# megapose6d/megapose6d

Measured on AMD Instinct MI355X. Metric: pose-hypotheses/sec (render+coarse+refine), 640×480, megapose-1.0-RGB, higher is better.
Workload: dtype f32 (results of fp32 arithmetic; the convolutions' multiplications run on the bf16 MFMA as EXACT piece products of the fp32 operands, fp32 accumulate)

## Files before the change

### include/mp_engine.h

```cpp
#ifndef MP_ENGINE_H
#define MP_ENGINE_H

#include <stddef.h>
#include <stdint.h>

#ifdef __cplusplus
extern "C" {
#endif

typedef void* mp_stream;

#define MP_OK 0
#define MP_ERR_INVALID (-22)
#define MP_ERR_NOMEM (-12)
#define MP_ERR_HIP (-5)

int mp_version(void);
const char* mp_last_error(void);
int mp_profile_begin(void);
int mp_profile_end(void);
int mp_profile_active(void);
int mp_profile_query_ex(int idx, char* name, int name_len, int64_t* launches, double* total_ms, double* total_flops,
                        double* total_bytes, double* total_executed_flops, double* peak_tflops);



int mp_device_info(int* n_cus, int* lds_bytes, char* arch_name, int arch_name_len);

typedef struct mp_mesh_db mp_mesh_db;

typedef struct {
  const float* h_vertices;
  const float* h_normals;
  const float* h_colors;
  const int32_t* h_faces;
  int32_t n_vertices;
  int32_t n_faces;
} mp_mesh_desc;

int mp_mesh_db_create(const mp_mesh_desc* h_meshes, int n_meshes, mp_mesh_db** out);
#define MP_TEX_MAX_LEVELS 15
int mp_mesh_db_set_texture(mp_mesh_db* db, int mesh_id, const float* h_uvs, const uint32_t* h_texels, int tex_w, int tex_h,
                           int n_levels);
int mp_mesh_db_destroy(mp_mesh_db* db);
int mp_mesh_db_max_vertices(const mp_mesh_db* db);
float mp_mesh_db_radius(const mp_mesh_db* db, int mesh_id);

#define MP_RASTER_NORMALS 1u
#define MP_RASTER_DEPTH 2u
#define MP_RASTER_NORMALS_GL 4u
#define MP_RASTER_MSAA4 16u

#define MP_RASTER_F16 32u

#define MP_RASTER_XREC 64u

typedef struct {
  float ambient[3];
  int32_t n_point;
  float point_dir[8][3];
  float point_color[8][3];
  float point_offset[8][3];
} mp_lights;

size_t mp_raster_workspace_bytes(const mp_mesh_db* db, int n_views, int h, int w);

int mp_raster_render(const mp_mesh_db* db, const int32_t* d_mesh_ids, const float* d_TCO ,
                     const float* d_K , int n_views, int h, int w, uint32_t flags,
                     const mp_lights* h_lights, float* d_out, int64_t stride_v, int views_per_item,
                     int64_t stride_view, int64_t stride_y, int64_t stride_x, int c_rgb, int c_normals,
                     int c_depth, void* d_workspace, size_t workspace_bytes, mp_stream stream);

int mp_raster_render_crop(const mp_mesh_db* db, const int32_t* d_mesh_ids, const float* d_TCO, const float* d_K, int n_views,
                          int h, int w, uint32_t flags, const mp_lights* lights, float* d_out, int64_t stride_v,
                          int views_per_item, int64_t stride_view, int64_t stride_y, int64_t stride_x, int c_rgb,
                          int c_normals, int c_depth, void* d_workspace, size_t workspace_bytes,
                          const float* d_images , int images_nhwc4, int n_im,
                          int C, int H, int W, const int32_t* d_im_ids, const float* d_boxes, int c0_crop, mp_stream stream);
int mp_raster_render_xrec(const mp_mesh_db* db, const int32_t* d_mesh_ids, const float* d_TCO, const float* d_K, int n_views,
                          int h, int w, uint32_t flags, const mp_lights* lights, void* d_out_records, int64_t stride_v,
                          int views_per_item, int64_t stride_view, int64_t stride_y, int64_t stride_x, int c_rgb,
                          int c_normals, int c_depth, void* d_workspace, size_t workspace_bytes,
                          const float* d_images, int images_nhwc4, int n_im, int C, int H, int W, const int32_t* d_im_ids,
                          const float* d_boxes, uint32_t f32_mask, const float* d_tCR, int depth_mode, mp_stream stream);
const unsigned char* mp_raster_job_flags(const mp_mesh_db* db, const void* d_workspace, int n_views, int h, int w);
int mp_pack_observation_nhwc4(const float* d_images, int n_im, int C, int H, int W, float* d_out, mp_stream stream);

size_t mp_raster_scene_workspace_bytes(const mp_mesh_db* db, int n_objects, int h, int w);

int mp_raster_render_scene(const mp_mesh_db* db, int n_cams, const int32_t* h_obj_off, const int32_t* d_obj_off,
                           const int32_t* d_mesh_ids, const float* d_TCO, const float* d_K, const float* d_radius,
                           const mp_lights* d_lights, int h, int w, uint32_t flags, float* d_out, int64_t stride_v, int64_t stride_y,
                           int64_t stride_x, int c_rgb, int c_normals, int c_depth, int32_t* d_instance, void* d_workspace,
                           size_t workspace_bytes, mp_stream stream);

int mp_crop_roi_align(const float* d_images , int n_im, int C, int H, int W,
                      const int32_t* d_im_ids , const float* d_boxes , int b,
                      int out_h, int out_w, float* d_out, int64_t stride_b, int64_t stride_y,
                      int64_t stride_x, int c0, mp_stream stream);

int mp_normalize_depth(float* d_x, int b, int h, int w, int border, int C, const int32_t* h_channels,
                       int n_ch, const float* d_tCR , int mode, mp_stream stream);
int mp_normalize_depth_f16(void* d_x_half, int b, int h, int w, int border, int C, const int32_t* h_channels,
                           int n_ch, const float* d_tCR , int mode, mp_stream stream);

size_t mp_conv_packed_floats(int Cin_p, int Cout, int KH, int KW);
int mp_conv_pack_weights(const float* h_w_oihw, int Cout, int Cin, int KH, int KW, int Cin_p,
                         const float* h_scale , float* h_packed);

typedef struct {
  const float* d_x;
  int32_t N, H, W, C;
  int32_t in_border;
  const float* d_w;
  const float* d_bias;
  int32_t Cout, KH, KW, stride, pad;
  float* d_y;
  int32_t out_border;
  const float* d_residual;
  int32_t relu;
  float* d_y_act;
  const float* d_act_scale;
  const float* d_act_shift;
  int32_t c_real;
  float* d_splitk_ws;
  int64_t splitk_ws_floats;
  int32_t x_f16;
} mp_conv_desc;

int mp_conv2d_nhwc(const mp_conv_desc* desc, mp_stream stream);
int mp_conv2d_plan(const mp_conv_desc* desc, int n_cu, int32_t* out5);

const char* mp_conv2d_kernel_name(const mp_conv_desc* desc);

size_t mp_conv_bf16x9_packed_bytes(int Cin_p, int Cout, int KH, int KW);
int mp_conv_bf16x9_pack_weights(const float* h_w_oihw, int Cout, int Cin, int KH, int KW, int Cin_p, const float* h_scale ,
                                void* h_packed);
int mp_conv2d_bf16x9_nhwc(const mp_conv_desc* desc, const void* d_w_pieces, mp_stream stream);

size_t mp_conv_wino_packed_floats(int Cin_p, int Cout);
int mp_conv_wino_pack_weights(const float* h_w_oi33, int Cout, int Cin, int Cin_p, const float* h_scale , float* h_packed);
int mp_conv_wino_eligible(const mp_conv_desc* desc, int n_cu);
int mp_conv3x3_wino_nhwc(const mp_conv_desc* desc, const float* d_u, mp_stream stream);

size_t mp_conv_wino_bf16_packed_bytes(int Cin_p, int Cout);
int mp_conv_wino_bf16_pack_weights(const float* h_w_oi33, int Cout, int Cin, int Cin_p, const float* h_scale , void* h_packed);
int mp_conv3x3_wino_bf16_nhwc(const mp_conv_desc* desc, const void* d_u_pieces, mp_stream stream);

int mp_xrec_elements(int n_f32, int n_u8);
int mp_conv_stem_supported(int KS, int n_f32, int n_u8);
size_t mp_conv_stem_packed_bytes(int KS, int n_f32, int n_u8, int Cout);
int mp_conv_stem_pack_weights_mask(const float* h_w_oihw, int Cout, int Cin, int KS, uint32_t f32_mask,
                                   const float* h_scale , void* h_packed);
int mp_conv_stem_xrec(const mp_conv_desc* desc, const void* d_packed, int n_f32, mp_stream stream);
int mp_conv_stem_xrec_pool(const mp_conv_desc* desc, const void* d_packed, int n_f32, float* d_ypool, int pool_border, mp_stream stream);

int mp_conv_stem_sparse_chunks(int KS, int n_f32, int n_u8);
size_t mp_conv_stem_sparse_packed_bytes(int KS, int n_f32, int n_u8, int Cout);
int mp_conv_stem_pack_weights_sparse(const float* h_w_oihw, int Cout, int Cin, int KS, int n_f32, const float* h_scale, void* h_packed);
int mp_conv_stem_xrec_sparse(const mp_conv_desc* desc, const void* d_packed, const void* d_packed_sparse, int n_f32,
                             const unsigned char* d_tile_flags, float* d_ypool, int pool_border, mp_stream stream);

int mp_maxpool3x3s2(const float* d_x, int N, int H, int W, int C, int in_border, float* d_y,
                    int out_border, float* d_y_act, const float* d_act_scale, const float* d_act_shift,
                    mp_stream stream);

int mp_bn_relu_nhwc(const float* d_x, int N, int H, int W, int C, int border, float* d_y_act, const float* d_act_scale,
                    const float* d_act_shift, mp_stream stream);

int mp_pool_fc_heads(const float* d_x, int N, int H, int W, int C, int in_border, const float* d_fc_w,
                     const float* d_fc_b, int n_feat, const float* d_head_w, const float* d_head_b,
                     int n_out, float* d_feat , float* d_out ,
                     float* d_sigmoid , mp_stream stream);

typedef struct mp_backbone mp_backbone;
#define MP_BACKBONE_VANILLA_RESNET34 0
#define MP_BACKBONE_WIDE_RESNET34 1
#define MP_BACKBONE_WIDE_RESNET18 2

typedef struct {
  const char* name;
  const float* h_data;
  int64_t numel;
} mp_named_tensor;

int mp_backbone_create_wide(int kind, int width, int c_in, int head_kind, int n_head_out, const mp_named_tensor* state, int n_tensors,
                            mp_backbone** out);
int mp_backbone_destroy(mp_backbone* bb);
int mp_backbone_input_channels_padded(const mp_backbone* bb);
int mp_backbone_input_border(const mp_backbone* bb);
size_t mp_backbone_workspace_bytes(const mp_backbone* bb, int batch, int h, int w);
int mp_backbone_workspace_reset(mp_backbone* bb, const void* d_workspace);
int mp_backbone_forward(mp_backbone* bb, const float* d_x, int batch, int h, int w, float* d_out,
                        float* d_sigmoid, float* d_feat, void* d_workspace, size_t workspace_bytes,
                        mp_stream stream);
int mp_backbone_forward_f16(mp_backbone* bb, const void* d_x_half, int batch, int h, int w, float* d_out,
                            float* d_sigmoid, float* d_feat, void* d_workspace, size_t workspace_bytes,
                            mp_stream stream);
int mp_backbone_xrec_prepare(mp_backbone* bb, uint32_t f32_mask);
int mp_backbone_forward_xrec_mask(mp_backbone* bb, const void* d_xrec, uint32_t f32_mask, int batch, int h, int w, float* d_out,
                                  float* d_sigmoid, float* d_feat, void* d_workspace, size_t workspace_bytes,
                                  mp_stream stream);
int mp_backbone_forward_xrec_sparse(mp_backbone* bb, const void* d_xrec, uint32_t f32_mask, const unsigned char* d_tile_flags, int batch,
                                    int h, int w, float* d_out, float* d_sigmoid, float* d_feat, void* d_workspace,
                                    size_t workspace_bytes, mp_stream stream);
double mp_backbone_flops(const mp_backbone* bb, int batch, int h, int w);

int mp_normalize_T(const float* d_T, int b, float* d_T_out, mp_stream stream);

int mp_init_extents(const float* d_points , int n_mesh, int n_pts,
                    const float* d_R , int n_rot, float* d_ext, mp_stream stream);
int mp_init_poses_from_boxes(const float* d_boxes , const float* d_K ,
                             const int32_t* d_mesh_ids, const int32_t* d_rot_ids, const float* d_R,
                             int n_rot, const float* d_ext, int b, float* d_TCO ,
                             mp_stream stream);

#define MP_MV_REMOVE_TCO 256
#define MP_MV_INPLANE 512
int mp_pose_multiview_n_views(int multiview);
int mp_pose_prepare_ex(const float* d_TCO_in , const float* d_K ,
                       const int32_t* d_mesh_ids, const float* d_points ,
                       int n_pts_stride, int n_pts_main, int n_pts_views, int b, int V, int multiview,
                       int im_h, int im_w, int out_h, int out_w, float lamb,
                       float* d_TCO_n , float* d_tCR , float* d_TCV_O ,
                       float* d_KV_crop , float* d_boxes_rend ,
                       float* d_boxes_crop , float* d_K_main , mp_stream stream);

int mp_pose_update(const float* d_TCO , const float* d_K_crop ,
                   int k_stride_floats, const float* d_out9 , const float* d_tCR , int b,
                   float* d_TCO_out, mp_stream stream);

#define MP_POSE_ERROR_MEAN 0
#define MP_POSE_ERROR_MAX 1
size_t mp_pose_error_workspace_bytes(int b, int n_pts, int S_max);
int mp_pose_error_sym(const float* d_T_pred , const float* d_T_gt, const float* d_symmetries, const int32_t* d_n_sym, int S_max,
                      const float* d_points, int n_pts_stride, const int32_t* d_mesh_ids , const int32_t* d_n_points, int n_pts,
                      int b, int reduce, int split, float* d_err , float* d_err_alt, int32_t* d_idx , float* d_T_gt_sym,
                      float* d_errs, float* d_diffs, void* d_workspace, size_t workspace_bytes, mp_stream stream);
int mp_pose_error_nn(const float* d_T_pred , const float* d_T_gt , const float* d_points, int n_pts_stride,
                     const int32_t* d_mesh_ids, const int32_t* d_n_points, int n_pts, int b, int split, float* d_diffs, int32_t* d_assign,
                     float* d_mean , float* d_max , void* d_workspace, size_t workspace_bytes, mp_stream stream);
int mp_pose_error_rigid(const float* d_T_a , const float* d_T_b , int b, const float* d_K, const float* d_points,
                        int n_pts_stride, const int32_t* d_mesh_ids, const int32_t* d_n_points, int n_pts, float* d_trans_err ,
                        float* d_rot_err_deg , float* d_proj_err, mp_stream stream);

int mp_pose_error_mspd(const float* d_T_pred , const float* d_T_gt, const float* d_symmetries, const int32_t* d_n_sym, int S_max,
                       const float* d_points, int n_pts_stride, const int32_t* d_mesh_ids , const int32_t* d_n_points, int n_pts,
                       int b, int reduce, int split, const float* d_K , float* d_err , float* d_err_alt,
                       int32_t* d_idx , float* d_T_gt_sym, float* d_errs, void* d_workspace, size_t workspace_bytes, mp_stream stream);

size_t mp_vsd_workspace_bytes(int b, int n_tau);
int mp_vsd(const float* d_depth_est , const int32_t* d_est_ids ,
           const float* d_depth_gt , const int32_t* d_gt_ids, const float* d_depth_test ,
           const int32_t* d_im_ids, int n_est, int n_gt, int n_im, const float* d_K , const float* d_diameter ,
           int b, int h, int w, float delta, const float* h_taus, int n_tau , int normalized, int split,
           float* d_errs , int32_t* d_counts ,
           void* d_workspace, size_t workspace_bytes, mp_stream stream);

size_t mp_gt_info_workspace_bytes(int b);
int mp_gt_info(const float* d_depth_gt , const int32_t* d_gt_ids ,
               const float* d_depth_test , const int32_t* d_im_ids, int n_gt, int n_im, const float* d_K ,
               int b, int h, int w, int canvas , float delta, int split,
               int32_t* d_counts , int32_t* d_boxes ,
               float* d_visib_fract , uint8_t* d_mask , uint8_t* d_mask_visib ,
               void* d_workspace, size_t workspace_bytes, mp_stream stream);

int mp_bop_match_limits(int* max_errors, int* max_thetas, int* mask_bits, int* stage_floats);
size_t mp_bop_match_workspace_bytes(int n_taken_words, int E, int n_theta);
int mp_bop_match(const float* d_errs , const int32_t* d_cand_gt , const int32_t* d_cand_lgt ,
                 const int32_t* d_est_row , const int32_t* d_est_off ,
                 const int32_t* d_group_est_off , const int32_t* d_group_n_gt ,
                 const int32_t* d_group_taken_off , const int32_t* d_n_top ,
                 const double* d_thr , int P, int C, int n_est, int n_groups, int n_taken_words, int E,
                 int n_theta, int32_t* d_match , void* d_workspace, size_t workspace_bytes, mp_stream stream);

int mp_mask_pair_counts(const uint8_t* d_pred_masks , const uint8_t* d_gt_masks ,
                        const int32_t* d_cand_pred , const int32_t* d_cand_gt , int P, int G, int C, int H, int W, int split,
                        int32_t* d_counts , mp_stream stream);
size_t mp_det_match_workspace_bytes(int n_taken_words, int n_theta);
int mp_det_match(const double* d_iou , const int32_t* d_cand_gt , const int32_t* d_cand_lgt ,
                 const int32_t* d_est_row , const int32_t* d_est_off ,
                 const int32_t* d_group_est_off , const int32_t* d_group_n_gt ,
                 const int32_t* d_group_taken_off , const int32_t* d_n_top ,
                 const uint8_t* d_gt_ignore , const double* d_thr , int P, int C, int n_est, int n_groups,
                 int n_taken_words, int n_theta, int32_t* d_match , void* d_workspace, size_t workspace_bytes,
                 mp_stream stream);

size_t mp_model_info_scratch_bytes(int n_obj, const int32_t* h_n_points, int tile);
int mp_model_info(const float* d_points , int stride, const int32_t* d_n_points ,
                  const int32_t* h_n_points , int n_obj, int tile, void* d_scratch, float* d_d2 ,
                  int32_t* d_pair , float* d_bounds , mp_stream stream);

size_t mp_surface_sample_scratch_bytes(int n_obj, const int32_t* h_face_off, int count, int block);
int mp_surface_sample(const float* d_vertices , const int32_t* d_faces , const int32_t* d_vert_off ,
                      const int32_t* d_face_off , const int32_t* h_vert_off , const int32_t* h_face_off ,
                      int n_obj, const float* d_u , int count, int block, void* d_workspace,
                      float* d_points , int32_t* d_face , mp_stream stream);

int mp_overlay(const uint8_t* d_images , const uint8_t* d_render , const int32_t* d_labels ,
               const uint8_t* d_colors , int n_colors, int n, int h, int w, int dilate_iterations,
               uint8_t* d_contour , uint8_t* d_canny , uint8_t* d_mask ,
               uint8_t* d_mesh , mp_stream stream);
int mp_draw_boxes(const uint8_t* d_images , const float* d_boxes , const int32_t* d_image_ids ,
                  int n_boxes, const uint8_t* d_colors , int n_colors, int n, int h, int w, int thickness,
                  uint8_t* d_out , mp_stream stream);

size_t mp_icp_workspace_bytes(int n_images, int n_rows, int H, int W);
int mp_icp_refine(const float* d_depth_meas, int n_images, const int32_t* d_im_ids, const float* d_depth_rend,
                  const float* d_K_images, const float* d_K_rows, const float* d_TCO, int n_rows, int H, int W,
                  int n_iterations, int n_levels, float tolerance, int n_min_points, int user_masks, float* d_TCO_out,
                  int32_t* d_retval, float* d_residual, void* d_workspace, size_t workspace_bytes, mp_stream stream);

int mp_icp_nn_max_points(void);
size_t mp_icp_nn_workspace_bytes(int n_images, int n_rows, int H, int W);
int mp_icp_refine_nn(const float* d_depth_meas, int n_images, const int32_t* d_im_ids, const float* d_depth_rend, const float* d_K_images,
                     const float* d_K_rows, const float* d_TCO, int n_rows, int H, int W, int n_iterations, int n_levels, float tolerance,
                     int n_min_points, const unsigned char* d_masks, float* d_TCO_out, int32_t* d_retval, float* d_residual, int32_t* d_iters,
                     void* d_ws, size_t ws_bytes, mp_stream stream);

size_t mp_fps_workspace_bytes(int n_rows, int stride);
int mp_fps(const float* d_points, const int32_t* d_counts, int n_rows, int stride, int n_points, int use_fps, int32_t* d_idx, int32_t* d_m,
           void* d_workspace, size_t workspace_bytes, mp_stream stream);
size_t mp_teaser_workspace_bytes(int n_rows, int H, int W);
int mp_teaser_solve(const float* d_src, const float* d_dst, const int32_t* d_counts, int n_rows, int stride, float noise_bound,
                    int inlier_selection, int tim_graph, int min_num_inliers, double* d_Rt, int32_t* d_retval, int32_t* d_degree,
                    int32_t* d_core, int32_t* d_selected, int32_t* d_info, void* d_workspace, size_t workspace_bytes, mp_stream stream);
int mp_teaser_refine(const float* d_depth_meas, int n_images, const int32_t* d_im_ids, const float* d_depth_rend, const float* d_K_rows,
                     const float* d_TCO, int n_rows, int H, int W, int mask_type, float depth_delta_thresh, int n_min_points, int n_points,
                     float noise_bound, int min_num_inliers, int use_fps, int inlier_selection, int tim_graph, float* d_TCO_out,
                     int32_t* d_retval, double* d_Rt, int32_t* d_sample_idx, int32_t* d_degree, int32_t* d_core, int32_t* d_selected,
                     int32_t* d_info, void* d_workspace, size_t workspace_bytes, mp_stream stream);
int mp_max_clique_default_steps(void);
size_t mp_max_clique_workspace_bytes(int n_rows, int stride);
int mp_max_clique(const uint8_t* d_adjacency, const int32_t* d_counts, int n_rows, int stride, int max_steps, int32_t* d_members, int32_t* d_info,
                  void* d_workspace, size_t workspace_bytes, mp_stream stream);
size_t mp_teaser_workspace_bytes_ex(int n_rows, int H, int W, int stride, int inlier_selection);
int mp_teaser_solve_ex(const float* d_src, const float* d_dst, const int32_t* d_counts, int n_rows, int stride, float noise_bound,
                       int inlier_selection, int tim_graph, int min_num_inliers, double* d_Rt, int32_t* d_retval, int32_t* d_degree,
                       int32_t* d_core, int32_t* d_selected, int32_t* d_info, int max_clique_steps, int32_t* d_clique_info, void* d_workspace,
                       size_t workspace_bytes, mp_stream stream);
int mp_teaser_refine_ex(const float* d_depth_meas, int n_images, const int32_t* d_im_ids, const float* d_depth_rend, const float* d_K_rows,
                        const float* d_TCO, int n_rows, int H, int W, int mask_type, float depth_delta_thresh, int n_min_points, int n_points,
                        float noise_bound, int min_num_inliers, int use_fps, int inlier_selection, int tim_graph, float* d_TCO_out,
                        int32_t* d_retval, double* d_Rt, int32_t* d_sample_idx, int32_t* d_degree, int32_t* d_core, int32_t* d_selected,
                        int32_t* d_info, int max_clique_steps, int32_t* d_clique_info, void* d_workspace, size_t workspace_bytes, mp_stream stream);

typedef struct mp_detector mp_detector;

typedef struct {
  int32_t n_classes;
  int32_t min_size, max_size;
  float image_mean[3], image_std[3];
  int32_t anchor_sizes[5];
  float aspect_ratios[3];
  int32_t rpn_pre_nms_top_n, rpn_post_nms_top_n;
  float rpn_nms_thresh, rpn_score_thresh, rpn_min_size;
  float box_score_thresh, box_nms_thresh, box_min_size;
  int32_t box_detections_per_img;
} mp_detector_config;

int mp_detector_default_config(mp_detector_config* cfg, int n_classes, int min_size, int max_size);
int mp_detector_state_spec(int n_classes, int idx, char* name, int name_len, int64_t* shape4, int32_t* n_dims);
int mp_detector_create(const mp_detector_config* cfg, const mp_named_tensor* h_state, int n_tensors, mp_detector** out);
int mp_detector_destroy(mp_detector* det);
size_t mp_detector_workspace_bytes(const mp_detector* det, int n_images, int H, int W);
int mp_detector_forward(mp_detector* det, const float* d_images, int n_images, int H, int W, float* d_boxes, float* d_scores,
                        int32_t* d_labels, int32_t* d_counts, float* d_masks, void* d_workspace, size_t workspace_bytes,
                        mp_stream stream);
int mp_detector_debug_tensor(const mp_detector* det, const char* what, const void** d_ptr, int64_t* shape4, int32_t* border,
                             int64_t* row_stride, int64_t* n_elements );

#ifdef __cplusplus
}
#endif
#endif
```

### megapose6d_amd/_lib.py

```python
from __future__ import annotations

import ctypes as C
import os
from pathlib import Path

_HERE = Path(__file__).resolve().parent
LIB_PATH = _HERE / "libmp_engine.so"


class EngineError(RuntimeError):
    pass


class MeshDesc(C.Structure):
    _fields_ = [
        ("h_vertices", C.c_void_p),
        ("h_normals", C.c_void_p),
        ("h_colors", C.c_void_p),
        ("h_faces", C.c_void_p),
        ("n_vertices", C.c_int32),
        ("n_faces", C.c_int32),
    ]


class Lights(C.Structure):
    _fields_ = [
        ("ambient", C.c_float * 3),
        ("n_point", C.c_int32),
        ("point_dir", (C.c_float * 3) * 8),
        ("point_color", (C.c_float * 3) * 8),
        ("point_offset", (C.c_float * 3) * 8),
    ]


class ConvDesc(C.Structure):
    _fields_ = [
        ("d_x", C.c_void_p),
        ("N", C.c_int32), ("H", C.c_int32), ("W", C.c_int32), ("C", C.c_int32),
        ("in_border", C.c_int32),
        ("d_w", C.c_void_p),
        ("d_bias", C.c_void_p),
        ("Cout", C.c_int32), ("KH", C.c_int32), ("KW", C.c_int32), ("stride", C.c_int32), ("pad", C.c_int32),
        ("d_y", C.c_void_p),
        ("out_border", C.c_int32),
        ("d_residual", C.c_void_p),
        ("relu", C.c_int32),
        ("d_y_act", C.c_void_p),
        ("d_act_scale", C.c_void_p),
        ("d_act_shift", C.c_void_p),
        ("c_real", C.c_int32),
        ("d_splitk_ws", C.c_void_p),
        ("splitk_ws_floats", C.c_int64),
        ("x_f16", C.c_int32),
    ]


class DetectorConfig(C.Structure):
    _fields_ = [
        ("n_classes", C.c_int32),
        ("min_size", C.c_int32), ("max_size", C.c_int32),
        ("image_mean", C.c_float * 3), ("image_std", C.c_float * 3),
        ("anchor_sizes", C.c_int32 * 5),
        ("aspect_ratios", C.c_float * 3),
        ("rpn_pre_nms_top_n", C.c_int32), ("rpn_post_nms_top_n", C.c_int32),
        ("rpn_nms_thresh", C.c_float), ("rpn_score_thresh", C.c_float), ("rpn_min_size", C.c_float),
        ("box_score_thresh", C.c_float), ("box_nms_thresh", C.c_float), ("box_min_size", C.c_float),
        ("box_detections_per_img", C.c_int32),
    ]


class NamedTensor(C.Structure):
    _fields_ = [("name", C.c_char_p), ("h_data", C.c_void_p), ("numel", C.c_int64)]


_vp, _i, _i64, _f, _sz, _u32 = C.c_void_p, C.c_int, C.c_int64, C.c_float, C.c_size_t, C.c_uint32

SIGNATURES = {
    "mp_version": (_i, []),
    "mp_last_error": (C.c_char_p, []),
    "mp_conv_clock_read": (_i, [C.POINTER(C.c_double), _i]),
    "mp_clock_probe": (_i, [C.c_double, C.POINTER(C.c_double), C.POINTER(C.c_double), _vp]),
    "mp_profile_begin": (_i, []),
    "mp_profile_end": (_i, []),
    "mp_profile_active": (_i, []),
    "mp_profile_query_ex": (_i, [_i, C.c_char_p, _i, C.POINTER(_i64), C.POINTER(C.c_double), C.POINTER(C.c_double), C.POINTER(C.c_double),
                                 C.POINTER(C.c_double), C.POINTER(C.c_double)]),
    "mp_device_info": (_i, [C.POINTER(_i), C.POINTER(_i), C.c_char_p, _i]),
    "mp_mesh_db_create": (_i, [C.POINTER(MeshDesc), _i, C.POINTER(_vp)]),
    "mp_mesh_db_set_texture": (_i, [_vp, _i, _vp, _vp, _i, _i, _i]),
    "mp_mesh_db_destroy": (_i, [_vp]),
    "mp_mesh_db_max_vertices": (_i, [_vp]),
    "mp_mesh_db_radius": (_f, [_vp, _i]),
    "mp_raster_workspace_bytes": (_sz, [_vp, _i, _i, _i]),
    "mp_raster_render": (_i, [_vp, _vp, _vp, _vp, _i, _i, _i, _u32, C.POINTER(Lights), _vp, _i64, _i, _i64, _i64, _i64, _i, _i, _i,
                              _vp, _sz, _vp]),
    "mp_raster_render_crop": (_i, [_vp, _vp, _vp, _vp, _i, _i, _i, _u32, C.POINTER(Lights), _vp, _i64, _i, _i64, _i64, _i64, _i, _i, _i,
                                   _vp, _sz, _vp, _i, _i, _i, _i, _i, _vp, _vp, _i, _vp]),
    "mp_raster_render_xrec": (_i, [_vp, _vp, _vp, _vp, _i, _i, _i, _u32, C.POINTER(Lights), _vp, _i64, _i, _i64, _i64, _i64, _i, _i, _i,
                                   _vp, _sz, _vp, _i, _i, _i, _i, _i, _vp, _vp, _u32, _vp, _i, _vp]),
    "mp_raster_job_flags": (_vp, [_vp, _vp, _i, _i, _i]),
    "mp_pack_observation_nhwc4": (_i, [_vp, _i, _i, _i, _i, _vp, _vp]),
    "mp_raster_scene_workspace_bytes": (_sz, [_vp, _i, _i, _i]),
    "mp_raster_render_scene": (_i, [_vp, _i, C.POINTER(C.c_int32), _vp, _vp, _vp, _vp, _vp, _vp, _i, _i, _u32, _vp, _i64, _i64, _i64, _i, _i,
                                    _i, _vp, _vp, _sz, _vp]),
    "mp_crop_roi_align": (_i, [_vp, _i, _i, _i, _i, _vp, _vp, _i, _i, _i, _vp, _i64, _i64, _i64, _i, _vp]),
    "mp_normalize_depth": (_i, [_vp, _i, _i, _i, _i, _i, C.POINTER(C.c_int32), _i, _vp, _i, _vp]),
    "mp_normalize_depth_f16": (_i, [_vp, _i, _i, _i, _i, _i, C.POINTER(C.c_int32), _i, _vp, _i, _vp]),
    "mp_conv_packed_floats": (_sz, [_i, _i, _i, _i]),
    "mp_conv_pack_weights": (_i, [_vp, _i, _i, _i, _i, _i, _vp, _vp]),
    "mp_conv2d_nhwc": (_i, [C.POINTER(ConvDesc), _vp]),
    "mp_conv2d_plan": (_i, [C.POINTER(ConvDesc), _i, C.POINTER(C.c_int32)]),
    "mp_conv_bf16x9_packed_bytes": (_sz, [_i, _i, _i, _i]),
    "mp_conv_bf16x9_pack_weights": (_i, [_vp, _i, _i, _i, _i, _i, _vp, _vp]),
    "mp_conv2d_bf16x9_nhwc": (_i, [C.POINTER(ConvDesc), _vp, _vp]),
    "mp_conv2d_kernel_name": (C.c_char_p, [C.POINTER(ConvDesc)]),
    "mp_conv_wino_packed_floats": (_sz, [_i, _i]),
    "mp_conv_wino_pack_weights": (_i, [_vp, _i, _i, _i, _vp, _vp]),
    "mp_conv_wino_eligible": (_i, [C.POINTER(ConvDesc), _i]),
    "mp_conv3x3_wino_nhwc": (_i, [C.POINTER(ConvDesc), _vp, _vp]),
    "mp_conv_wino_stats": (_i, [C.POINTER(C.c_double), C.POINTER(C.c_double), _i]),
    "mp_conv_wino_bf16_packed_bytes": (_sz, [_i, _i]),
    "mp_conv_wino_bf16_pack_weights": (_i, [_vp, _i, _i, _i, _vp, _vp]),
    "mp_conv3x3_wino_bf16_nhwc": (_i, [C.POINTER(ConvDesc), _vp, _vp]),
    "mp_conv_wino_bf16_stats": (_i, [C.POINTER(C.c_double), C.POINTER(C.c_double), _i]),
    "mp_conv_wino_bf16_clock": (_i, [C.POINTER(C.c_double), C.POINTER(C.c_double), _i]),
    "mp_conv_wino_bf16_phases": (_i, [C.POINTER(C.c_double), C.POINTER(C.c_double)]),
    "mp_conv_wino_bf16_telemetry": (_i, [_i]),
    "mp_xrec_elements": (_i, [_i, _i]),
    "mp_conv_stem_supported": (_i, [_i, _i, _i]),
    "mp_conv_stem_packed_bytes": (_sz, [_i, _i, _i, _i]),
    "mp_conv_stem_pack_weights_mask": (_i, [_vp, _i, _i, _i, _u32, _vp, _vp]),
    "mp_conv_stem_sparse_chunks": (_i, [_i, _i, _i]),
    "mp_conv_stem_sparse_packed_bytes": (_sz, [_i, _i, _i, _i]),
    "mp_conv_stem_pack_weights_sparse": (_i, [_vp, _i, _i, _i, _i, _vp, _vp]),
    "mp_conv_stem_xrec_sparse": (_i, [C.POINTER(ConvDesc), _vp, _vp, _i, _vp, _vp, _i, _vp]),
    "mp_conv_stem_bg_stats": (_i, [C.POINTER(C.c_double), C.POINTER(C.c_double), _i]),
    "mp_conv_stem_xrec": (_i, [C.POINTER(ConvDesc), _vp, _i, _vp]),
    "mp_conv_stem_xrec_pool": (_i, [C.POINTER(ConvDesc), _vp, _i, _vp, _i, _vp]),
    "mp_maxpool3x3s2": (_i, [_vp, _i, _i, _i, _i, _i, _vp, _i, _vp, _vp, _vp, _vp]),
    "mp_bn_relu_nhwc": (_i, [_vp, _i, _i, _i, _i, _i, _vp, _vp, _vp, _vp]),
    "mp_pool_fc_heads": (_i, [_vp, _i, _i, _i, _i, _i, _vp, _vp, _i, _vp, _vp, _i, _vp, _vp, _vp, _vp]),
    "mp_backbone_create_wide": (_i, [_i, _i, _i, _i, _i, C.POINTER(NamedTensor), _i, C.POINTER(_vp)]),
    "mp_backbone_destroy": (_i, [_vp]),
    "mp_backbone_input_channels_padded": (_i, [_vp]),
    "mp_backbone_input_border": (_i, [_vp]),
    "mp_backbone_workspace_bytes": (_sz, [_vp, _i, _i, _i]),
    "mp_backbone_workspace_reset": (_i, [_vp, _vp]),
    "mp_backbone_forward": (_i, [_vp, _vp, _i, _i, _i, _vp, _vp, _vp, _vp, _sz, _vp]),
    "mp_backbone_forward_f16": (_i, [_vp, _vp, _i, _i, _i, _vp, _vp, _vp, _vp, _sz, _vp]),
    "mp_backbone_xrec_prepare": (_i, [_vp, _u32]),
    "mp_backbone_forward_xrec_mask": (_i, [_vp, _vp, _u32, _i, _i, _i, _vp, _vp, _vp, _vp, _sz, _vp]),
    "mp_backbone_forward_xrec_sparse": (_i, [_vp, _vp, _u32, _vp, _i, _i, _i, _vp, _vp, _vp, _vp, _sz, _vp]),
    "mp_backbone_flops": (C.c_double, [_vp, _i, _i, _i]),
    "mp_normalize_T": (_i, [_vp, _i, _vp, _vp]),
    "mp_init_extents": (_i, [_vp, _i, _i, _vp, _i, _vp, _vp]),
    "mp_init_poses_from_boxes": (_i, [_vp, _vp, _vp, _vp, _vp, _i, _vp, _i, _vp, _vp]),
    "mp_pose_multiview_n_views": (_i, [_i]),
    "mp_pose_prepare_ex": (_i, [_vp, _vp, _vp, _vp, _i, _i, _i, _i, _i, _i, _i, _i, _i, _i, _f, _vp, _vp, _vp, _vp, _vp, _vp, _vp, _vp]),
    "mp_pose_error_workspace_bytes": (_sz, [_i, _i, _i]),
    "mp_pose_error_sym": (_i, [_vp, _vp, _vp, _vp, _i, _vp, _i, _vp, _vp, _i, _i, _i, _i, _vp, _vp, _vp, _vp, _vp, _vp, _vp, _sz, _vp]),
    "mp_pose_error_nn": (_i, [_vp, _vp, _vp, _i, _vp, _vp, _i, _i, _i, _vp, _vp, _vp, _vp, _vp, _sz, _vp]),
    "mp_pose_error_rigid": (_i, [_vp, _vp, _i, _vp, _vp, _i, _vp, _vp, _i, _vp, _vp, _vp, _vp]),
    "mp_pose_error_mspd": (_i, [_vp, _vp, _vp, _vp, _i, _vp, _i, _vp, _vp, _i, _i, _i, _i, _vp, _vp, _vp, _vp, _vp, _vp, _vp, _sz, _vp]),
    "mp_vsd_workspace_bytes": (_sz, [_i, _i]),
    "mp_vsd": (_i, [_vp, _vp, _vp, _vp, _vp, _vp, _i, _i, _i, _vp, _vp, _i, _i, _i, _f, _vp, _i, _i, _i, _vp, _vp, _vp, _sz, _vp]),
    "mp_gt_info_workspace_bytes": (_sz, [_i]),
    "mp_gt_info": (_i, [_vp, _vp, _vp, _vp, _i, _i, _vp, _i, _i, _i, _i, _f, _i, _vp, _vp, _vp, _vp, _vp, _vp, _sz, _vp]),
    "mp_bop_match_limits": (_i, [C.POINTER(_i), C.POINTER(_i), C.POINTER(_i), C.POINTER(_i)]),
    "mp_bop_match_workspace_bytes": (_sz, [_i, _i, _i]),
    "mp_bop_match": (_i, [_vp, _vp, _vp, _vp, _vp, _vp, _vp, _vp, _vp, _vp, _i, _i, _i, _i, _i, _i, _i, _vp, _vp, _sz, _vp]),
    "mp_mask_pair_counts": (_i, [_vp, _vp, _vp, _vp, _i, _i, _i, _i, _i, _i, _vp, _vp]),
    "mp_det_match_workspace_bytes": (_sz, [_i, _i]),
    "mp_det_match": (_i, [_vp, _vp, _vp, _vp, _vp, _vp, _vp, _vp, _vp, _vp, _vp, _i, _i, _i, _i, _i, _i, _vp, _vp, _sz, _vp]),
    "mp_model_info_scratch_bytes": (_sz, [_i, _vp, _i]),
    "mp_model_info": (_i, [_vp, _i, _vp, _vp, _i, _i, _vp, _vp, _vp, _vp, _vp]),
    "mp_overlay": (_i, [_vp, _vp, _vp, _vp, _i, _i, _i, _i, _i, _vp, _vp, _vp, _vp, _vp]),
    "mp_draw_boxes": (_i, [_vp, _vp, _vp, _i, _vp, _i, _i, _i, _i, _i, _vp, _vp]),
    "mp_surface_sample_scratch_bytes": (_sz, [_i, _vp, _i, _i]),
    "mp_surface_sample": (_i, [_vp, _vp, _vp, _vp, _vp, _vp, _i, _vp, _i, _i, _vp, _vp, _vp, _vp]),
    "mp_fps_workspace_bytes": (_sz, [_i, _i]),
    "mp_fps": (_i, [_vp, _vp, _i, _i, _i, _i, _vp, _vp, _vp, _sz, _vp]),
    "mp_teaser_workspace_bytes": (_sz, [_i, _i, _i]),
    "mp_teaser_solve": (_i, [_vp, _vp, _vp, _i, _i, _f, _i, _i, _i, _vp, _vp, _vp, _vp, _vp, _vp, _vp, _sz, _vp]),
    "mp_teaser_refine": (_i, [_vp, _i, _vp, _vp, _vp, _vp, _i, _i, _i, _i, _f, _i, _i, _f, _i, _i, _i, _i, _vp, _vp, _vp, _vp, _vp, _vp, _vp, _vp,
                              _vp, _sz, _vp]),
    "mp_max_clique_default_steps": (_i, []),
    "mp_max_clique_workspace_bytes": (_sz, [_i, _i]),
    "mp_max_clique": (_i, [_vp, _vp, _i, _i, _i, _vp, _vp, _vp, _sz, _vp]),
    "mp_teaser_workspace_bytes_ex": (_sz, [_i, _i, _i, _i, _i]),
    "mp_teaser_solve_ex": (_i, [_vp, _vp, _vp, _i, _i, _f, _i, _i, _i, _vp, _vp, _vp, _vp, _vp, _vp, _i, _vp, _vp, _sz, _vp]),
    "mp_teaser_refine_ex": (_i, [_vp, _i, _vp, _vp, _vp, _vp, _i, _i, _i, _i, _f, _i, _i, _f, _i, _i, _i, _i, _vp, _vp, _vp, _vp, _vp, _vp, _vp, _vp,
                                 _i, _vp, _vp, _sz, _vp]),
    "mp_icp_workspace_bytes": (_sz, [_i, _i, _i, _i]),
    "mp_icp_refine": (_i, [_vp, _i, _vp, _vp, _vp, _vp, _vp, _i, _i, _i, _i, _i, _f, _i, _i, _vp, _vp, _vp, _vp, _sz, _vp]),
    "mp_icp_nn_max_points": (_i, []),
    "mp_icp_nn_workspace_bytes": (_sz, [_i, _i, _i, _i]),
    "mp_icp_refine_nn": (_i, [_vp, _i, _vp, _vp, _vp, _vp, _vp, _i, _i, _i, _i, _i, _f, _i, _vp, _vp, _vp, _vp, _vp, _vp, _sz, _vp]),
    "mp_pose_update": (_i, [_vp, _vp, _i, _vp, _vp, _i, _vp, _vp]),
    "mp_detector_default_config": (_i, [C.POINTER(DetectorConfig), _i, _i, _i]),
    "mp_detector_state_spec": (_i, [_i, _i, C.c_char_p, _i, C.POINTER(_i64), C.POINTER(C.c_int32)]),
    "mp_detector_create": (_i, [C.POINTER(DetectorConfig), C.POINTER(NamedTensor), _i, C.POINTER(_vp)]),
    "mp_detector_destroy": (_i, [_vp]),
    "mp_detector_workspace_bytes": (_sz, [_vp, _i, _i, _i]),
    "mp_detector_forward": (_i, [_vp, _vp, _i, _i, _i, _vp, _vp, _vp, _vp, _vp, _vp, _sz, _vp]),
    "mp_detector_debug_tensor": (_i, [_vp, C.c_char_p, C.POINTER(_vp), C.POINTER(_i64), C.POINTER(C.c_int32), C.POINTER(_i64), C.POINTER(_i64)]),
}

_lib = None


def load() -> C.CDLL:
    global _lib
    if _lib is not None:
        return _lib
    path = Path(os.environ.get("MP_ENGINE_LIB", LIB_PATH))
    if not path.is_file():
        raise EngineError(
            f"{path} not found: the HIP engine is not built. Run `python __graft_entry__.py` "
            "(hipcc --offload-arch=gfx950). There is no CPU/PyTorch fallback."
        )
    try:
        lib = C.CDLL(str(path))
    except OSError as e:
        raise EngineError(f"cannot load {path}: {e}") from e
    for name, (res, args) in SIGNATURES.items():
        try:
            fn = getattr(lib, name)
        except AttributeError as e:
            raise EngineError(f"{path} does not export {name}") from e
        fn.restype = res
        fn.argtypes = args
    _lib = lib
    return lib


def check(rc: int) -> None:
    if rc != 0:
        msg = load().mp_last_error().decode("utf-8", "replace")
        raise EngineError(f"mp_engine error {rc}: {msg}")
```

### megapose6d_amd/csrc/backbone.hip

```cpp
#include <cmath>
#include <cstdlib>
#include <map>
#include <mutex>
#include <string>
#include <vector>

#include "conv_layer.h"

namespace mp {

struct BnAct {
  float* d_scale = nullptr;
  float* d_shift = nullptr;
};

struct Block {
  ConvLayer conv1, conv2, down;
  bool has_down = false;
  BnAct pre;
};

}

using namespace mp;

struct mp_backbone {
  int kind, c_in, c_in_p, in_border, head_kind, n_out, n_feat;
  int width = 1;
  int stageC[4] = {64, 128, 256, 512};
  bool wide;
  bool direct_bf16 = true;
  ConvLayer stem;
  std::vector<Block> blocks;
  std::vector<int> stage_of_block;
  float *d_fc_w = nullptr, *d_fc_b = nullptr, *d_head_w = nullptr, *d_head_b = nullptr;
  std::vector<void*> allocs;
  std::vector<float> stem_w_host, stem_scale_host;
  std::mutex blob_mu;
  std::map<uint32_t, void*> stem_blobs;
  std::map<uint32_t, void*> stem_blobs_sparse;
  struct WsKey { void* ptr; int batch, h, w; };
  std::vector<WsKey> ws_known;
};

namespace {

const char* const WHO = "mp_backbone_create";

int make_conv(mp_backbone* bb, const StateMap& sm, const std::string& wkey, const std::string& bnkey , int Cin,
              int Cin_p, int Cout, int K, int stride, int pad, ConvLayer* L) {
  const float* w = find(sm, wkey, (int64_t)Cout * Cin * K * K, WHO);
  if (!w) return MP_ERR_INVALID;
  static const int wino_mode = getenv("MP_CONV_WINO") ? atoi(getenv("MP_CONV_WINO")) : 2;
  unsigned forms = wino_mode == 0 ? 0u : wino_mode == 1 ? CONV_FORM_WINO_F32 : CONV_FORM_WINO_BF16;
  if (L == &bb->stem) {
    bb->stem_w_host.assign(w, w + (size_t)Cout * Cin * K * K);
    std::vector<float> shift;
    if (!bnkey.empty() && bn_affine(sm, bnkey, Cout, WHO, bb->stem_scale_host, shift)) return MP_ERR_INVALID;
  } else if (bb->direct_bf16) {
    forms |= CONV_FORM_DIRECT_BF16;
  }
  return make_conv_layer(bb->allocs, sm, WHO, w, bnkey, nullptr, 0, Cin, Cin_p, Cout, K, stride, pad, forms, L);
}

int make_bnact(mp_backbone* bb, const StateMap& sm, const std::string& bnkey, int C, BnAct* a) {
  std::vector<float> scale, shift;
  int rc = bn_affine(sm, bnkey, C, WHO, scale, shift);
  if (rc) return rc;
  rc = upload(bb->allocs, scale, &a->d_scale);
  if (rc) return rc;
  return upload(bb->allocs, shift, &a->d_shift);
}

constexpr size_t SPLITK_WS_FLOATS = 12u << 20;

inline size_t align_up(size_t v, size_t a) { return (v + a - 1) / a * a; }
inline size_t buf_floats(int N, int H, int W, int C) { return (size_t)N * (H + 2) * (W + 2) * C + (size_t)(W + 3) * C + 64; }

struct Geometry {
  int h1, w1;
  int hs[4], ws[4];
};

Geometry geometry(const mp_backbone* bb, int h, int w) {
  Geometry g;
  g.h1 = (h + 2 * bb->stem.pad - bb->stem.K) / 2 + 1;
  g.w1 = (w + 2 * bb->stem.pad - bb->stem.K) / 2 + 1;
  g.hs[0] = (g.h1 + 2 - 3) / 2 + 1;
  g.ws[0] = (g.w1 + 2 - 3) / 2 + 1;
  for (int s = 1; s < 4; ++s) {
    g.hs[s] = (g.hs[s - 1] + 2 - 3) / 2 + 1;
    g.ws[s] = (g.ws[s - 1] + 2 - 3) / 2 + 1;
  }
  return g;
}


}

extern "C" int mp_backbone_create_wide(int kind, int width, int c_in, int head_kind, int n_head_out, const mp_named_tensor* st, int n_tensors,
                                       mp_backbone** out) {
  MP_REQUIRE(out && st && n_tensors > 0, "mp_backbone_create: bad arguments");
  MP_REQUIRE(kind >= 0 && kind <= 2, "mp_backbone_create: unknown backbone kind %d", kind);
  MP_REQUIRE(width >= 1 && width <= 8 && (width == 1 || kind != MP_BACKBONE_VANILLA_RESNET34),
             "mp_backbone_create: width multiplier %d (1..8, WideResNets only: training/pose_models_cfg.py:114-116)", width);
  MP_REQUIRE(c_in >= 1 && c_in <= 512, "mp_backbone_create: bad c_in %d", c_in);
  StateMap sm;
  for (int i = 0; i < n_tensors; ++i) sm[st[i].name] = std::make_pair(st[i].h_data, st[i].numel);
  mp_backbone* bb = new mp_backbone();
  bb->kind = kind;
  bb->wide = kind != MP_BACKBONE_VANILLA_RESNET34;
  bb->direct_bf16 = !(getenv("MP_CONV_DIRECT_BF16") && atoi(getenv("MP_CONV_DIRECT_BF16")) == 0);
  bb->c_in = c_in;
  bb->c_in_p = (c_in + 3) / 4 * 4;
  bb->head_kind = head_kind;
  bb->n_out = n_head_out;
  bb->width = width;
  for (int k = 0; k < 4; ++k) bb->stageC[k] = bb->stageC[k] * width;
  const int C0 = bb->stageC[0], NF = bb->stageC[3];
  bb->n_feat = NF;
  int rc;
#define MP_TRY(e) do { rc = (e); if (rc) { mp_backbone_destroy(bb); return rc; } } while (0)
  const std::string B = "backbone.";
  if (!bb->wide) {
    bb->in_border = 3;
    MP_TRY(make_conv(bb, sm, B + "conv1.weight", B + "bn1", c_in, bb->c_in_p, C0, 7, 2, 3, &bb->stem));
  } else {
    bb->in_border = 2;
    MP_TRY(make_conv(bb, sm, B + "conv1.weight", B + "bn1", c_in, bb->c_in_p, C0, 5, 2, 2, &bb->stem));
  }
  static const int n34[4] = {3, 4, 6, 3}, n18[4] = {2, 2, 2, 2};
  const int* nblocks = (kind == MP_BACKBONE_WIDE_RESNET18) ? n18 : n34;
  int inplanes = C0;
  for (int s = 0; s < 4; ++s) {
    const int planes = bb->stageC[s];
    for (int i = 0; i < nblocks[s]; ++i) {
      Block blk;
      const int stride = (i == 0 && s > 0) ? 2 : 1;
      const std::string P = B + "layer" + std::to_string(s + 1) + "." + std::to_string(i) + ".";
      blk.has_down = (i == 0) && (stride != 1 || inplanes != planes);
      if (!bb->wide) {
        MP_TRY(make_conv(bb, sm, P + "conv1.weight", P + "bn1", inplanes, inplanes, planes, 3, stride, 1, &blk.conv1));
        MP_TRY(make_conv(bb, sm, P + "conv2.weight", P + "bn2", planes, planes, planes, 3, 1, 1, &blk.conv2));
        if (blk.has_down)
          MP_TRY(make_conv(bb, sm, P + "downsample.0.weight", P + "downsample.1", inplanes, inplanes, planes, 1, stride, 0, &blk.down));
      } else {
        MP_TRY(make_bnact(bb, sm, P + "bn1", inplanes, &blk.pre));
        MP_TRY(make_conv(bb, sm, P + "conv1.weight", P + "bn2", inplanes, inplanes, planes, 3, stride, 1, &blk.conv1));
        MP_TRY(make_conv(bb, sm, P + "conv2.weight", "", planes, planes, planes, 3, 1, 1, &blk.conv2));
        if (blk.has_down) MP_TRY(make_conv(bb, sm, P + "downsample.weight", "", inplanes, inplanes, planes, 1, stride, 0, &blk.down));
      }
      bb->blocks.push_back(blk);
      bb->stage_of_block.push_back(s);
      inplanes = planes;
    }
  }
  if (!bb->wide) {
    const float* fw = find(sm, B + "fc.weight", 512 * 512, WHO);
    const float* fb = find(sm, B + "fc.bias", 512, WHO);
    if (!fw || !fb) { mp_backbone_destroy(bb); return MP_ERR_INVALID; }
    MP_TRY(upload(bb->allocs, std::vector<float>(fw, fw + 512 * 512), &bb->d_fc_w));
    MP_TRY(upload(bb->allocs, std::vector<float>(fb, fb + 512), &bb->d_fc_b));
  }
  const std::string H = head_kind == 0 ? "pose_fc" : "views_logits_head";
  const float* hw = find(sm, H + ".weight", (int64_t)n_head_out * NF, WHO);
  const float* hb = find(sm, H + ".bias", n_head_out, WHO);
  if (!hw || !hb) { mp_backbone_destroy(bb); return MP_ERR_INVALID; }
  MP_TRY(upload(bb->allocs, std::vector<float>(hw, hw + (size_t)n_head_out * NF), &bb->d_head_w));
  MP_TRY(upload(bb->allocs, std::vector<float>(hb, hb + n_head_out), &bb->d_head_b));
#undef MP_TRY
  *out = bb;
  return MP_OK;
}

extern "C" int mp_backbone_destroy(mp_backbone* bb) {
  if (!bb) return MP_OK;
  for (void* p : bb->allocs) (void)hipFree(p);
  delete bb;
  return MP_OK;
}

extern "C" int mp_backbone_input_channels_padded(const mp_backbone* bb) { return bb ? bb->c_in_p : 0; }
extern "C" int mp_backbone_input_border(const mp_backbone* bb) { return bb ? bb->in_border : 0; }

extern "C" size_t mp_backbone_workspace_bytes(const mp_backbone* bb, int batch, int h, int w) {
  if (!bb || batch <= 0) return 0;
  const Geometry g = geometry(bb, h, w);
  size_t fl = align_up(buf_floats(batch, g.h1, g.w1, bb->stageC[0]), 64);
  const int per_stage = bb->wide ? 4 : 3;
  for (int s = 0; s < 4; ++s) fl += per_stage * align_up(buf_floats(batch, g.hs[s], g.ws[s], bb->stageC[s]), 64);
  fl += SPLITK_WS_FLOATS;
  return fl * sizeof(float);
}

extern "C" int mp_backbone_workspace_reset(mp_backbone* bb, const void* d_ws) {
  MP_REQUIRE(bb, "mp_backbone_workspace_reset: null handle");
  for (size_t i = 0; i < bb->ws_known.size();)
    if (bb->ws_known[i].ptr == d_ws) bb->ws_known.erase(bb->ws_known.begin() + i); else ++i;
  return MP_OK;
}

extern "C" int mp_backbone_xrec_prepare(mp_backbone* bb, uint32_t f32_mask) {
  if (!bb || bb->stem_w_host.empty() || bb->c_in > 32) return 0;
  if (bb->c_in < 32 && (f32_mask >> bb->c_in) != 0u) return 0;
  const int n_f32 = __builtin_popcount(f32_mask), n_u8 = bb->c_in - n_f32;
  if (!mp_conv_stem_supported(bb->stem.K, n_f32, n_u8) || bb->stem.Cout % 64 != 0) return 0;
  std::lock_guard<std::mutex> blob_lock(bb->blob_mu);
  if (!bb->stem_blobs.count(f32_mask)) {
    std::vector<unsigned char> blob(mp_conv_stem_packed_bytes(bb->stem.K, n_f32, n_u8, bb->stem.Cout));
    if (mp_conv_stem_pack_weights_mask(bb->stem_w_host.data(), bb->stem.Cout, bb->c_in, bb->stem.K, f32_mask,
                                       bb->stem_scale_host.empty() ? nullptr : bb->stem_scale_host.data(), blob.data()) != MP_OK)
      return 0;
    void* d = nullptr;
    if (hipMalloc(&d, blob.size()) != hipSuccess) return 0;
    if (hipMemcpy(d, blob.data(), blob.size(), hipMemcpyHostToDevice) != hipSuccess) { (void)hipFree(d); return 0; }
    bb->allocs.push_back(d);
    bb->stem_blobs[f32_mask] = d;
    if (f32_mask == (n_f32 >= 32 ? 0xFFFFFFFFu : (1u << n_f32) - 1u) && mp_conv_stem_sparse_chunks(bb->stem.K, n_f32, n_u8) > 0) {
      std::vector<unsigned char> sb(mp_conv_stem_sparse_packed_bytes(bb->stem.K, n_f32, n_u8, bb->stem.Cout));
      void* ds = nullptr;
      if (mp_conv_stem_pack_weights_sparse(bb->stem_w_host.data(), bb->stem.Cout, bb->c_in, bb->stem.K, n_f32,
                                           bb->stem_scale_host.empty() ? nullptr : bb->stem_scale_host.data(), sb.data()) == MP_OK &&
          hipMalloc(&ds, sb.size()) == hipSuccess) {
        if (hipMemcpy(ds, sb.data(), sb.size(), hipMemcpyHostToDevice) == hipSuccess) {
          bb->allocs.push_back(ds);
          bb->stem_blobs_sparse[f32_mask] = ds;
        } else {
          (void)hipFree(ds);
        }
      }
    }
  }
  return mp_xrec_elements(n_f32, n_u8);
}

static int backbone_forward_impl(mp_backbone* bb, const float* d_x, int x_mode, uint32_t f32_mask, int batch, int h, int w, float* d_out, float* d_sigmoid,
                                 float* d_feat, void* d_ws, size_t ws_bytes, mp_stream stream, const unsigned char* d_tile_flags = nullptr) {
  const bool x_f16 = x_mode == 1;
  MP_REQUIRE(bb && d_x && d_out && d_ws, "mp_backbone_forward: null pointer");
  if (batch == 0) return MP_OK;
  const size_t need = mp_backbone_workspace_bytes(bb, batch, h, w);
  MP_REQUIRE(ws_bytes >= need, "mp_backbone_forward: workspace %zu < %zu bytes", ws_bytes, need);
  hipStream_t s = (hipStream_t)stream;
  const Geometry g = geometry(bb, h, w);
  bool known = false;
  for (const auto& k : bb->ws_known) known = known || (k.ptr == d_ws && k.batch == batch && k.h == h && k.w == w);
  if (!known) {
    MP_CHECK_HIP(hipMemsetAsync(d_ws, 0, need, s));
    for (size_t i = 0; i < bb->ws_known.size();)
      if (bb->ws_known[i].ptr == d_ws) bb->ws_known.erase(bb->ws_known.begin() + i); else ++i;
    if (bb->ws_known.size() >= 8) bb->ws_known.erase(bb->ws_known.begin());
    bb->ws_known.push_back({d_ws, batch, h, w});
  }
  float* p = (float*)d_ws;
  float* S = p; p += align_up(buf_floats(batch, g.h1, g.w1, bb->stageC[0]), 64);
  float *A[4], *Aact[4], *Bf[4], *Cf[4];
  for (int st = 0; st < 4; ++st) {
    const size_t n = align_up(buf_floats(batch, g.hs[st], g.ws[st], bb->stageC[st]), 64);
    A[st] = p; p += n;
    Aact[st] = nullptr;
    if (bb->wide) { Aact[st] = p; p += n; }
    Bf[st] = p; p += n;
    Cf[st] = p; p += n;
  }
  float* SK = p;
  int rc;
  bool stem_pooled = false;
  if (x_mode == 2) {
    const void* d_stem_pieces = nullptr;
    const void* d_sparse_blob = nullptr;
    {
      std::lock_guard<std::mutex> blob_lock(bb->blob_mu);
      const auto blob_it = bb->stem_blobs.find(f32_mask);
      if (blob_it != bb->stem_blobs.end()) d_stem_pieces = blob_it->second;
      const auto sp_it = bb->stem_blobs_sparse.find(f32_mask);
      if (sp_it != bb->stem_blobs_sparse.end()) d_sparse_blob = sp_it->second;
    }
    MP_REQUIRE(d_stem_pieces != nullptr, "mp_backbone_forward_xrec: no piece blob for the fp32-kind channel mask 0x%x of this %d-channel stem: "
               "call mp_backbone_xrec_prepare first (it returns 0 if the stem has no exact-piece form)", f32_mask, bb->c_in);
    const int n_f32 = __builtin_popcount(f32_mask);
    mp_conv_desc d;
    memset(&d, 0, sizeof(d));
    d.d_x = d_x; d.N = batch; d.H = h; d.W = w; d.C = bb->stem.Cin_p; d.c_real = bb->c_in; d.in_border = bb->in_border;
    d.d_bias = bb->stem.d_b; d.Cout = bb->stem.Cout; d.KH = bb->stem.K; d.KW = bb->stem.K; d.stride = 2; d.pad = bb->stem.pad;
    d.d_y = S; d.out_border = 1; d.relu = 1;
    static const bool fuse_pool = !(getenv("MP_STEM_POOL") && atoi(getenv("MP_STEM_POOL")) == 0);
    const void* d_sparse = d_tile_flags ? d_sparse_blob : nullptr;
    if (fuse_pool) {
      d.d_y = nullptr;
      rc = d_sparse ? mp_conv_stem_xrec_sparse(&d, d_stem_pieces, d_sparse, n_f32, d_tile_flags, A[0], 1, s)
                    : mp_conv_stem_xrec_pool(&d, d_stem_pieces, n_f32, A[0], 1, s);
      if (!rc && bb->wide) rc = mp_bn_relu_nhwc(A[0], batch, g.hs[0], g.ws[0], bb->stageC[0], 1, Aact[0], bb->blocks[0].pre.d_scale, bb->blocks[0].pre.d_shift, s);
      stem_pooled = true;
    } else {
      rc = d_sparse ? mp_conv_stem_xrec_sparse(&d, d_stem_pieces, d_sparse, n_f32, d_tile_flags, nullptr, 0, s)
                    : mp_conv_stem_xrec(&d, d_stem_pieces, n_f32, s);
    }
  } else {
    rc = run_conv_layer(bb->stem, d_x, batch, h, w, bb->in_border, S, 1, nullptr, 1, s, SK, SPLITK_WS_FLOATS, nullptr, nullptr, nullptr, x_f16);
  }
  if (rc) return rc;
  const Block& b0 = bb->blocks[0];
  if (!stem_pooled) {
    rc = mp_maxpool3x3s2(S, batch, g.h1, g.w1, bb->stageC[0], 1, A[0], 1, bb->wide ? Aact[0] : nullptr, bb->wide ? b0.pre.d_scale : nullptr,
                         bb->wide ? b0.pre.d_shift : nullptr, s);
    if (rc) return rc;
  }
  const int nb = (int)bb->blocks.size();
  for (int i = 0; i < nb; ++i) {
    const Block& blk = bb->blocks[i];
    const int so = bb->stage_of_block[i];
    const int si = (blk.has_down && so > 0) ? so - 1 : so;
    const int Hi = g.hs[si], Wi = g.ws[si];
    const bool last = (i + 1 == nb);
    if (!bb->wide) {
      rc = run_conv_layer(blk.conv1, A[si], batch, Hi, Wi, 1, Bf[so], 1, nullptr, 1, s, SK, SPLITK_WS_FLOATS);
      if (rc) return rc;
      const float* idn = A[si];
      if (blk.has_down) {
        rc = run_conv_layer(blk.down, A[si], batch, Hi, Wi, 1, Cf[so], 1, nullptr, 0, s, SK, SPLITK_WS_FLOATS);
        if (rc) return rc;
        idn = Cf[so];
      }
      rc = run_conv_layer(blk.conv2, Bf[so], batch, g.hs[so], g.ws[so], 1, A[so], 1, idn, 1, s, SK, SPLITK_WS_FLOATS);
      if (rc) return rc;
    } else {
      rc = run_conv_layer(blk.conv1, Aact[si], batch, Hi, Wi, 1, Bf[so], 1, nullptr, 1, s, SK, SPLITK_WS_FLOATS);
      if (rc) return rc;
      const float* idn = A[si];
      if (blk.has_down) {
        rc = run_conv_layer(blk.down, Aact[si], batch, Hi, Wi, 1, Cf[so], 1, nullptr, 0, s, SK, SPLITK_WS_FLOATS);
        if (rc) return rc;
        idn = Cf[so];
      }
      const BnAct next_pre = last ? BnAct() : bb->blocks[i + 1].pre;
      rc = run_conv_layer(blk.conv2, Bf[so], batch, g.hs[so], g.ws[so], 1, A[so], 1, idn, 0, s, SK, SPLITK_WS_FLOATS, last ? nullptr : Aact[so],
                          next_pre.d_scale, next_pre.d_shift);
      if (rc) return rc;
    }
  }
  return mp_pool_fc_heads(A[3], batch, g.hs[3], g.ws[3], bb->stageC[3], 1, bb->d_fc_w, bb->d_fc_b, bb->n_feat, bb->d_head_w, bb->d_head_b, bb->n_out,
                          d_feat, d_out, d_sigmoid, s);
}

extern "C" int mp_backbone_forward(mp_backbone* bb, const float* d_x, int batch, int h, int w, float* d_out, float* d_sigmoid,
                                   float* d_feat, void* d_ws, size_t ws_bytes, mp_stream stream) {
  return backbone_forward_impl(bb, d_x, 0, 0, batch, h, w, d_out, d_sigmoid, d_feat, d_ws, ws_bytes, stream);
}

extern "C" int mp_backbone_forward_xrec_mask(mp_backbone* bb, const void* d_xrec, uint32_t f32_mask, int batch, int h, int w, float* d_out,
                                             float* d_sigmoid, float* d_feat, void* d_ws, size_t ws_bytes, mp_stream stream) {
  return backbone_forward_impl(bb, (const float*)d_xrec, 2, f32_mask, batch, h, w, d_out, d_sigmoid, d_feat, d_ws, ws_bytes, stream);
}

extern "C" int mp_backbone_forward_xrec_sparse(mp_backbone* bb, const void* d_xrec, uint32_t f32_mask, const unsigned char* d_tile_flags, int batch,
                                               int h, int w, float* d_out, float* d_sigmoid, float* d_feat, void* d_ws, size_t ws_bytes,
                                               mp_stream stream) {
  return backbone_forward_impl(bb, (const float*)d_xrec, 2, f32_mask, batch, h, w, d_out, d_sigmoid, d_feat, d_ws, ws_bytes, stream, d_tile_flags);
}

extern "C" int mp_backbone_forward_f16(mp_backbone* bb, const void* d_x_half, int batch, int h, int w, float* d_out, float* d_sigmoid,
                                       float* d_feat, void* d_ws, size_t ws_bytes, mp_stream stream) {
  return backbone_forward_impl(bb, (const float*)d_x_half, 1, 0, batch, h, w, d_out, d_sigmoid, d_feat, d_ws, ws_bytes, stream);
}

extern "C" double mp_backbone_flops(const mp_backbone* bb, int batch, int h, int w) {
  if (!bb) return 0.0;
  const Geometry g = geometry(bb, h, w);
  auto conv_flops = [](const ConvLayer& L, int Ho, int Wo) { return 2.0 * L.Cout * L.Cin * L.K * L.K * (double)Ho * Wo; };
  double f = conv_flops(bb->stem, g.h1, g.w1);
  for (size_t i = 0; i < bb->blocks.size(); ++i) {
    const Block& blk = bb->blocks[i];
    const int so = bb->stage_of_block[i];
    f += conv_flops(blk.conv1, g.hs[so], g.ws[so]) + conv_flops(blk.conv2, g.hs[so], g.ws[so]);
    if (blk.has_down) f += conv_flops(blk.down, g.hs[so], g.ws[so]);
  }
  if (!bb->wide) f += 2.0 * 512 * 512;
  f += 2.0 * bb->n_feat * bb->n_out;
  return f * batch;
}
```

### megapose6d_amd/csrc/conv_stem.hip

```cpp
#include <cstdlib>
#include <vector>

#include "bf16x9_split.h"
#include "common.h"

namespace mp {
namespace stem {

typedef float f32x4 __attribute__((ext_vector_type(4)));
typedef __bf16 bf16x8 __attribute__((ext_vector_type(8)));
typedef unsigned u32x4 __attribute__((ext_vector_type(4)));

constexpr int TH = 8, TW = 16;
constexpr int NCO = 64;

struct Params {
  const unsigned char* __restrict__ x;
  const unsigned char* __restrict__ w;
  const float* __restrict__ bias;
  float* __restrict__ y;
  int N, Ho, Wo;
  int Hp, Wp;
  int in_off;
  int Cout, Hop, Wop, out_border;
  int tiles_x, tiles_y, n_cb;
  int n_steps;
  int relu;
  unsigned img_bytes;
  unsigned out_bytes;
  float* __restrict__ ypool;
  int Hq, Wq, pool_border;
  const unsigned char* __restrict__ tile_flags;
  const unsigned char* __restrict__ w_sparse;
  int fl_tx, fl_ty, q_use, n_steps_sparse;
  int H, W, pad;
  int count_bg;
};

__device__ unsigned long long g_stem_bg[2];

constexpr size_t LDS_PER_WG = 80 * 1024;

template <int KS, int Q>
struct Geo {
  static constexpr int PH = 2 * (TH - 1) + KS, PW = 2 * (TW - 1) + KS;
  static constexpr int QP = (Q % 2 == 0 && (size_t)(PH + 1) * ((PW * (Q + 1)) | 1) * 16 <= LDS_PER_WG) ? Q + 1 : Q;
  static constexpr int ROW16 = PW * QP;
  static constexpr int PITCH16 = ROW16 | 1;
  static constexpr int PITCH = PITCH16 * 16;
  static constexpr int KWQ = KS * Q;
  static constexpr int S = KS * KWQ;
  static constexpr int T = ((S + 3) / 4 + 1) / 2 * 2;
  static constexpr size_t PATCH = (size_t)(PH + 1) * PITCH;
  static constexpr size_t OUT_TILE = (size_t)TH * TW * NCO * 4;
  static constexpr size_t LDS = PATCH > OUT_TILE ? PATCH : OUT_TILE;
  static_assert(4 * T + 4 - S <= KWQ, "padding slices (and the look-ahead read past the last step) must stay inside the extra row");
  static_assert(LDS <= LDS_PER_WG, "the patch must leave room for a second workgroup on the CU");
};

template <int KS, int Q, bool POOL, bool SP = false>
__global__ __launch_bounds__(256) __attribute__((amdgpu_waves_per_eu(2, 2))) void conv_stem_bf16x3(Params p) {
  using G = Geo<KS, Q>;
  extern __shared__ __attribute__((aligned(16))) unsigned char lds[];
  const int tid = threadIdx.x, lane = tid & 63;
  const int wave = __builtin_amdgcn_readfirstlane(tid >> 6);
  int wg = xcd_remap(blockIdx.x, gridDim.x);
  const int cb = wg % p.n_cb; wg /= p.n_cb;
  const int tx = wg % p.tiles_x; wg /= p.tiles_x;
  const int ty = wg % p.tiles_y;
  const int n = wg / p.tiles_y;
  bool sparse = false;
  if constexpr (SP) {
    const int r0 = max(2 * ty * TH - p.pad, 0) >> 3, r1 = min(2 * ty * TH - p.pad + G::PH - 1, p.H - 1) >> 3;
    const int c0 = max(2 * tx * TW - p.pad, 0) >> 3, c1 = min(2 * tx * TW - p.pad + G::PW - 1, p.W - 1) >> 3;
    const int nc = c1 - c0 + 1, cnt = (r1 - r0 + 1) * nc;
    unsigned char f = 0;
    if (lane < cnt) f = p.tile_flags[((size_t)n * p.fl_ty + r0 + lane / nc) * p.fl_tx + c0 + lane % nc];
    sparse = cnt <= 64 && __ballot(f != 0) == 0ull;
  }
  if constexpr (SP) {
    if (p.count_bg && tid == 0) {
      if (sparse) atomicAdd(&g_stem_bg[0], 1ull);
      if (blockIdx.x == 0) atomicAdd(&g_stem_bg[1], (unsigned long long)gridDim.x);
    }
  }
  const int QU = SP && sparse ? p.q_use : Q;
  const int n_steps = SP && sparse ? p.n_steps_sparse : p.n_steps;

  {
    const unsigned char* img = p.x + (size_t)n * p.img_bytes;
    const __amdgpu_buffer_rsrc_t r_x = __builtin_amdgcn_make_buffer_rsrc((void*)img, 0, p.img_bytes, 0x00020000);
    const int row_bytes = p.Wp * (16 * Q);
    const int org = (2 * ty * TH + p.in_off) * row_bytes + (2 * tx * TW + p.in_off) * (16 * Q);
    constexpr int SRC16 = G::PW * Q;
    constexpr int N_CH = G::PH * SRC16, PER = (N_CH + 255) / 256;
    constexpr int HALF = (PER + 1) / 2;
    u32x4 v[HALF];
#pragma unroll
    for (int h = 0; h < 2; ++h) {
#pragma unroll
      for (int k = 0; k < HALF; ++k) {
        const int c = tid + 256 * (h * HALF + k);
        const int row = c / SRC16, col = c - row * SRC16;
        const bool want = c < N_CH && (!SP || col % Q < QU);
        v[k] = want ? __builtin_amdgcn_raw_buffer_load_b128(r_x, org + row * row_bytes + col * 16, 0, 0) : u32x4{0, 0, 0, 0};
      }
#pragma unroll
      for (int k = 0; k < HALF; ++k) {
        const int c = tid + 256 * (h * HALF + k);
        const int row = c / SRC16, col = c - row * SRC16;
        const int lcol = G::QP == Q ? col : col + (col / Q) * (G::QP - Q);
        if (c < N_CH && (!SP || col % Q < QU)) *reinterpret_cast<u32x4*>(lds + row * G::PITCH + lcol * 16) = v[k];
      }
    }
    for (int c = tid; c < G::PITCH16; c += 256) *reinterpret_cast<u32x4*>(lds + G::PH * G::PITCH + c * 16) = u32x4{0, 0, 0, 0};
  }

  const size_t w_wave = ((size_t)cb * 4 + wave) * n_steps * 3072;
  const __amdgpu_buffer_rsrc_t r_w = __builtin_amdgcn_make_buffer_rsrc((void*)((SP && sparse ? p.w_sparse : p.w) + w_wave), 0, (unsigned)n_steps * 3072u, 0x00020000);
  const int w_voff = lane * 16;
  u32x4 b0[3], b1[3];
#pragma unroll
  for (int q = 0; q < 3; ++q) {
    b0[q] = __builtin_amdgcn_raw_buffer_load_b128(r_w, w_voff, q * 1024, 0);
    b1[q] = __builtin_amdgcn_raw_buffer_load_b128(r_w, w_voff, 3072 + q * 1024, 0);
  }

  const int i = lane & 15, g = lane >> 4;
  int s_r = g;
  int a_row = (2 * i) * (16 * G::QP);
  const int kwq = SP ? KS * QU : G::KWQ;
  const int qu_m = 1024 / QU + 1;
  auto slice_off = [&](int sr) {
    if constexpr (SP) {
      const int kw = (sr * qu_m) >> 10;
      return (kw * G::QP + (sr - kw * QU)) * 16;
    } else {
      return G::QP == Q ? sr * 16 : (sr + (sr / Q) * (G::QP - Q)) * 16;
    }
  };
  int a_off = a_row + slice_off(s_r);
  auto advance = [&]() {
    s_r += 4;
    if (s_r >= kwq) { s_r -= kwq; a_row += G::PITCH; }
    a_off = a_row + slice_off(s_r);
  };
  f32x4 acc[TH];
#pragma unroll
  for (int j = 0; j < TH; ++j) acc[j] = f32x4{0.f, 0.f, 0.f, 0.f};
  u32x4 a0[TH], a1[TH];

  __syncthreads();
#pragma unroll
  for (int j = 0; j < TH; ++j) a0[j] = *reinterpret_cast<const u32x4*>(lds + a_off + j * 2 * G::PITCH);
  advance();

  const int n_pairs = n_steps >> 1;
  for (int tp = 0; tp < n_pairs; ++tp) {
    const int w_next = (2 * tp + 2) * 3072;
#pragma unroll
    for (int j = 0; j < TH; ++j) a1[j] = *reinterpret_cast<const u32x4*>(lds + a_off + j * 2 * G::PITCH);
    advance();
#pragma unroll
    for (int q = 0; q < 3; ++q) {
      const bf16x8 bq = __builtin_bit_cast(bf16x8, b0[q]);
#pragma unroll
      for (int j = 0; j < TH; ++j) acc[j] = __builtin_amdgcn_mfma_f32_16x16x32_bf16(__builtin_bit_cast(bf16x8, a0[j]), bq, acc[j], 0, 0, 0);
    }
#pragma unroll
    for (int q = 0; q < 3; ++q) b0[q] = __builtin_amdgcn_raw_buffer_load_b128(r_w, w_voff, w_next + q * 1024, 0);
#pragma unroll
    for (int j = 0; j < TH; ++j) a0[j] = *reinterpret_cast<const u32x4*>(lds + a_off + j * 2 * G::PITCH);
    advance();
#pragma unroll
    for (int q = 0; q < 3; ++q) {
      const bf16x8 bq = __builtin_bit_cast(bf16x8, b1[q]);
#pragma unroll
      for (int j = 0; j < TH; ++j) acc[j] = __builtin_amdgcn_mfma_f32_16x16x32_bf16(__builtin_bit_cast(bf16x8, a1[j]), bq, acc[j], 0, 0, 0);
    }
#pragma unroll
    for (int q = 0; q < 3; ++q) b1[q] = __builtin_amdgcn_raw_buffer_load_b128(r_w, w_voff, w_next + 3072 + q * 1024, 0);
  }

  __syncthreads();
  {
    const int co = cb * NCO + wave * 16 + i;
    const float bias = p.bias ? p.bias[co] : 0.f;
    float* tile = reinterpret_cast<float*>(lds);
#pragma unroll
    for (int j = 0; j < TH; ++j)
#pragma unroll
      for (int r = 0; r < 4; ++r) {
        float v = acc[j][r] + bias;
        if (p.relu) v = fmaxf(v, 0.f);
        tile[(j * TW + 4 * g + r) * NCO + wave * 16 + i] = v;
      }
  }
  __syncthreads();
  if constexpr (POOL) {
    const int oy0 = ty * TH, ox0 = tx * TW;
    const int Hqp = p.Hq + 2 * p.pool_border, Wqp = p.Wq + 2 * p.pool_border;
    const float4* tile4 = reinterpret_cast<const float4*>(lds);
    for (int item = tid; item < (TH / 2 + 1) * (TW / 2 + 1) * 16; item += 256) {
      const int part = item & 15, pp = item >> 4;
      const int ppy = pp / (TW / 2 + 1), ppx = pp - ppy * (TW / 2 + 1);
      const int PY = ty * (TH / 2) + ppy, PX = tx * (TW / 2) + ppx;
      if (PY >= p.Hq || PX >= p.Wq) continue;
      const int wr0 = max(2 * PY - 1, 0), wr1 = min(2 * PY + 1, p.Ho - 1), wc0 = max(2 * PX - 1, 0), wc1 = min(2 * PX + 1, p.Wo - 1);
      const int r0 = max(wr0, oy0), r1 = min(wr1, oy0 + TH - 1), c0 = max(wc0, ox0), c1 = min(wc1, ox0 + TW - 1);
      if (r0 > r1 || c0 > c1) continue;
      float4 m = make_float4(0.f, 0.f, 0.f, 0.f);
      for (int r = r0; r <= r1; ++r)
        for (int c = c0; c <= c1; ++c) {
          const float4 v = tile4[((r - oy0) * TW + (c - ox0)) * 16 + part];
          m.x = fmaxf(m.x, v.x); m.y = fmaxf(m.y, v.y); m.z = fmaxf(m.z, v.z); m.w = fmaxf(m.w, v.w);
        }
      float* dst = p.ypool + ((((size_t)n * Hqp + PY + p.pool_border) * Wqp + PX + p.pool_border) * p.Cout + cb * NCO + part * 4);
      if (r0 == wr0 && r1 == wr1 && c0 == wc0 && c1 == wc1) {
        *reinterpret_cast<float4*>(dst) = m;
      } else {
        unsigned* du = reinterpret_cast<unsigned*>(dst);
        atomicMax(du, __float_as_uint(m.x) & 0x7FFFFFFFu); atomicMax(du + 1, __float_as_uint(m.y) & 0x7FFFFFFFu);
        atomicMax(du + 2, __float_as_uint(m.z) & 0x7FFFFFFFu); atomicMax(du + 3, __float_as_uint(m.w) & 0x7FFFFFFFu);
      }
    }
  }
  if (!POOL || p.y != nullptr) {
    const __amdgpu_buffer_rsrc_t r_y = __builtin_amdgcn_make_buffer_rsrc((void*)(p.y + (size_t)n * (p.out_bytes / 4)), 0, p.out_bytes, 0x00020000);
    const int oy0 = ty * TH, ox0 = tx * TW;
#pragma unroll
    for (int k = 0; k < (TH * TW * NCO / 4) / 256; ++k) {
      const int c = tid + 256 * k;
      const int pix = c >> 4, part = c & 15;
      const int oy = oy0 + (pix >> 4), ox = ox0 + (pix & 15);
      const u32x4 v = *reinterpret_cast<const u32x4*>(lds + c * 16);
      const int off = ((oy + p.out_border) * p.Wop + ox + p.out_border) * p.Cout + cb * NCO + part * 4;
      const unsigned voff = (oy < p.Ho && ox < p.Wo) ? (unsigned)off * 4u : 0xFFFFFFF0u;
      __builtin_amdgcn_raw_buffer_store_b128(v, r_y, (int)voff, 0, 0);
    }
  }
}

__host__ __device__ inline int pool_zero_positions(int Hq, int Wq) {
  const int rows4 = (Hq + TH / 2 - 1) / (TH / 2), cols8 = (Wq + TW / 2 - 1) / (TW / 2);
  return rows4 * Wq + (Hq - rows4) * cols8;
}
__global__ __launch_bounds__(256) void pool_zero_kernel(float* __restrict__ y, int N, int Hq, int Wq, int C, int border) {
  const int c4n = C / 4;
  const int P = pool_zero_positions(Hq, Wq);
  const long idx = (long)blockIdx.x * blockDim.x + threadIdx.x;
  if (idx >= (long)N * P * c4n) return;
  const int c4 = (int)(idx % c4n);
  long t = idx / c4n;
  const int pos = (int)(t % P), n = (int)(t / P);
  const int rows4 = (Hq + TH / 2 - 1) / (TH / 2), cols8 = (Wq + TW / 2 - 1) / (TW / 2);
  int py, px;
  if (pos < rows4 * Wq) {
    py = (pos / Wq) * (TH / 2);
    px = pos % Wq;
  } else {
    const int q = pos - rows4 * Wq, k = q / cols8;
    py = k + k / (TH / 2 - 1) + 1;
    px = (q % cols8) * (TW / 2);
  }
  *reinterpret_cast<float4*>(y + ((((size_t)n * (Hq + 2 * border) + py + border) * (Wq + 2 * border) + px + border) * C + c4 * 4)) =
      make_float4(0.f, 0.f, 0.f, 0.f);
}

template <int KS, int Q, bool POOL = false, bool SP = false>
int launch(const Params& p, hipStream_t s, double flops, double bytes, const char* name) {
  const double executed = 2.0 * (double)p.N * p.tiles_y * p.tiles_x * (TH * TW) * p.Cout * (double)p.n_steps * 32.0 * 3.0;
  using G = Geo<KS, Q>;
  static int attr_dev = -1;
  int dev = 0;
  MP_CHECK_HIP(hipGetDevice(&dev));
  if (attr_dev != dev) {
    MP_CHECK_HIP(hipFuncSetAttribute((const void*)conv_stem_bf16x3<KS, Q, POOL, SP>, hipFuncAttributeMaxDynamicSharedMemorySize, (int)G::LDS));
    attr_dev = dev;
  }
  if (POOL) {
    ProfScope prof0("pool_zero", 0.0, 16.0 * p.N * (p.Hq / 4 + 1) * p.Wq * p.Cout, s);
    const long total = (long)p.N * pool_zero_positions(p.Hq, p.Wq) * (p.Cout / 4);
    hipLaunchKernelGGL(pool_zero_kernel, dim3((unsigned)((total + 255) / 256)), dim3(256), 0, s, p.ypool, p.N, p.Hq, p.Wq, p.Cout, p.pool_border);
  }
  ProfScope prof(name, flops, bytes, s, executed, 2500.0);
  hipLaunchKernelGGL((conv_stem_bf16x3<KS, Q, POOL, SP>), dim3((unsigned)((long)p.N * p.tiles_y * p.tiles_x * p.n_cb)), dim3(256), G::LDS, s, p);
  MP_CHECK_HIP(hipGetLastError());
  return MP_OK;
}

inline int n_steps(int KS, int Q) { return ((KS * KS * Q + 3) / 4 + 1) / 2 * 2; }

}
}

using namespace mp;

extern "C" int mp_xrec_elements(int n_f32, int n_u8) {
  if (n_f32 < 0 || n_u8 < 0 || n_f32 + n_u8 <= 0) return 0;
  return (3 * n_f32 + n_u8 + 7) / 8 * 8;
}

extern "C" int mp_conv_stem_supported(int KS, int n_f32, int n_u8) {
  const int R = mp_xrec_elements(n_f32, n_u8);
  return (KS == 7 || KS == 5) && R >= 16 && R <= 48 ? 1 : 0;
}

extern "C" size_t mp_conv_stem_packed_bytes(int KS, int n_f32, int n_u8, int Cout) {
  const int Q = mp_xrec_elements(n_f32, n_u8) / 8;
  return (size_t)(Cout / stem::NCO) * 4 * stem::n_steps(KS, Q) * 3072;
}

static int pack_weights_walk(const float* w, int Cout, int Cin, int KS, uint32_t f32_mask, const float* scale, void* packed, int q_walk);

extern "C" int mp_conv_stem_pack_weights_mask(const float* w, int Cout, int Cin, int KS, uint32_t f32_mask, const float* scale, void* packed) {
  return pack_weights_walk(w, Cout, Cin, KS, f32_mask, scale, packed, 0);
}

extern "C" int mp_conv_stem_sparse_chunks(int KS, int n_f32, int n_u8) {
  if (!mp_conv_stem_supported(KS, n_f32, n_u8) || n_f32 <= 0) return 0;
  const int Q = mp_xrec_elements(n_f32, n_u8) / 8, q_use = (3 * n_f32 + 7) / 8;
  if (q_use >= Q) return 0;
  const int pad = 4 * stem::n_steps(KS, q_use) + 4 - KS * KS * q_use;
  return pad <= KS * q_use ? q_use : 0;
}
extern "C" size_t mp_conv_stem_sparse_packed_bytes(int KS, int n_f32, int n_u8, int Cout) {
  const int q_use = mp_conv_stem_sparse_chunks(KS, n_f32, n_u8);
  return q_use ? (size_t)(Cout / stem::NCO) * 4 * stem::n_steps(KS, q_use) * 3072 : 0;
}
extern "C" int mp_conv_stem_pack_weights_sparse(const float* w, int Cout, int Cin, int KS, int n_f32, const float* scale, void* packed) {
  const int q_use = mp_conv_stem_sparse_chunks(KS, n_f32, Cin - n_f32);
  MP_REQUIRE(q_use > 0, "mp_conv_stem_pack_weights_sparse: this record has no background-tile form");
  return pack_weights_walk(w, Cout, Cin, KS, n_f32 >= 32 ? 0xFFFFFFFFu : (1u << n_f32) - 1u, scale, packed, q_use);
}

static int pack_weights_walk(const float* w, int Cout, int Cin, int KS, uint32_t f32_mask, const float* scale, void* packed, int q_walk) {
  MP_REQUIRE(Cin >= 1 && Cin <= 32 && (Cin == 32 || (f32_mask >> Cin) == 0u), "mp_conv_stem_pack_weights_mask: mask names channels >= Cin (<= 32 input channels)");
  const int n_f32 = __builtin_popcount(f32_mask), n_u8 = Cin - n_f32;
  MP_REQUIRE(w && packed && n_u8 >= 0 && Cout % stem::NCO == 0 && mp_conv_stem_supported(KS, n_f32, n_u8),
             "mp_conv_stem_pack_weights: bad arguments (Cout %% 64, KS 5 | 7, 16 <= record <= 48 elements)");
  int ch_of_f32[32], ch_of_u8[32];
  for (int c = 0, a = 0, b = 0; c < Cin; ++c) {
    if ((f32_mask >> c) & 1u) ch_of_f32[a++] = c; else ch_of_u8[b++] = c;
  }
  const int Q = q_walk > 0 ? q_walk : mp_xrec_elements(n_f32, n_u8) / 8;
  const int T = stem::n_steps(KS, Q), S = KS * KS * Q;
  unsigned short* out = (unsigned short*)packed;
  memset(out, 0, (size_t)(Cout / stem::NCO) * 4 * T * 3072);
  for (int co = 0; co < Cout; ++co) {
    const int cb = co / stem::NCO, wave = (co % stem::NCO) / 16, i = co % 16;
    const double sc = scale ? (double)scale[co] : 1.0;
    for (int s = 0; s < S; ++s) {
      const int t = s / 4, g = s % 4;
      const int kh = s / (KS * Q), rr = s % (KS * Q), kw = rr / Q, q = rr % Q;
      for (int e = 0; e < 8; ++e) {
        const int slot = 8 * q + e;
        int ch;
        double f;
        if (slot < 3 * n_f32) { ch = ch_of_f32[slot / 3]; f = sc; }
        else if (slot < 3 * n_f32 + n_u8) { ch = ch_of_u8[slot - 3 * n_f32]; f = sc / 255.0; }
        else continue;
        const float v = (float)((double)w[(((size_t)co * Cin + ch) * KS + kh) * KS + kw] * f);
        unsigned short pc[3];
        bf16x9_split3(v, pc);
        for (int piece = 0; piece < 3; ++piece)
          out[((((size_t)(cb * 4 + wave) * T + t) * 3 + piece) * 64 + (g * 16 + i)) * 8 + e] = pc[piece];
      }
    }
  }
  return MP_OK;
}

static int stem_xrec_impl(const mp_conv_desc* d, const void* d_packed, int n_f32, float* d_ypool, int pool_border, mp_stream stream,
                          const void* d_packed_sparse = nullptr, const unsigned char* d_tile_flags = nullptr) {
  MP_REQUIRE(d && d->d_x && d_packed && (d->d_y || d_ypool), "mp_conv_stem_xrec: null pointer");
  MP_REQUIRE(!d_ypool || (d->relu && pool_border >= 0), "mp_conv_stem_xrec_pool: the fused max pool needs the ReLU (its atomicMax orders non-negative floats)");
  const int n_u8 = d->c_real - n_f32;
  MP_REQUIRE(d->KH == d->KW && d->stride == 2 && d->Cout % stem::NCO == 0 && !d->d_residual && !d->d_y_act && d->in_border >= d->pad &&
                 mp_conv_stem_supported(d->KH, n_f32, n_u8),
             "mp_conv_stem_xrec: unsupported layer (square 5x5 / 7x7, stride 2, Cout %% 64, c_real = real channels, 16 <= record <= 48 elements)");
  const int R = mp_xrec_elements(n_f32, n_u8), Q = R / 8;
  stem::Params p;
  p.x = (const unsigned char*)d->d_x; p.w = (const unsigned char*)d_packed; p.bias = d->d_bias; p.y = d->d_y;
  p.N = d->N;
  p.Ho = (d->H + 2 * d->pad - d->KH) / 2 + 1; p.Wo = (d->W + 2 * d->pad - d->KW) / 2 + 1;
  p.Hp = d->H + 2 * d->in_border; p.Wp = d->W + 2 * d->in_border; p.in_off = d->in_border - d->pad;
  p.Cout = d->Cout; p.Hop = p.Ho + 2 * d->out_border; p.Wop = p.Wo + 2 * d->out_border; p.out_border = d->out_border;
  p.tiles_x = ceil_div(p.Wo, stem::TW); p.tiles_y = ceil_div(p.Ho, stem::TH); p.n_cb = d->Cout / stem::NCO;
  p.n_steps = stem::n_steps(d->KH, Q);
  p.relu = d->relu;
  const long img = (long)p.Hp * p.Wp * 16 * Q, outb = (long)p.Hop * p.Wop * d->Cout * 4;
  MP_REQUIRE(img < (1L << 31) && outb < (1L << 31) && (long)d->N * p.tiles_y * p.tiles_x * p.n_cb < (1L << 31), "mp_conv_stem_xrec: image too large for 32-bit offsets");
  p.img_bytes = (unsigned)img; p.out_bytes = (unsigned)outb;
  p.ypool = d_ypool; p.pool_border = pool_border;
  p.Hq = (p.Ho + 2 - 3) / 2 + 1; p.Wq = (p.Wo + 2 - 3) / 2 + 1;
  p.H = d->H; p.W = d->W; p.pad = d->pad;
  p.tile_flags = nullptr; p.w_sparse = nullptr; p.fl_tx = p.fl_ty = 0; p.q_use = Q; p.n_steps_sparse = p.n_steps;
  const int q_use = mp_conv_stem_sparse_chunks(d->KH, n_f32, n_u8);
  const bool sp = d_packed_sparse && d_tile_flags && q_use > 0;
  p.count_bg = 0;
  if (sp) {
    p.count_bg = mp_profile_active();
    p.tile_flags = d_tile_flags; p.w_sparse = (const unsigned char*)d_packed_sparse;
    p.fl_tx = ceil_div(d->W, 8); p.fl_ty = ceil_div(d->H, 8); p.q_use = q_use; p.n_steps_sparse = stem::n_steps(d->KH, q_use);
  }
  const double M = (double)d->N * p.Ho * p.Wo;
  const double flops = 2.0 * M * d->Cout * d->KH * d->KW * d->c_real;
  const double bytes = (double)d->N * img + (d->d_y ? 4.0 * M * d->Cout : 0.0) + (d_ypool ? 4.0 * (double)d->N * p.Hq * p.Wq * d->Cout : 0.0) +
                       (double)mp_conv_stem_packed_bytes(d->KH, n_f32, n_u8, d->Cout);
  hipStream_t s = (hipStream_t)stream;
#define MP_STEM_GO(KSV, QV)                                                                                                          \
  if (d->KH == KSV && Q == QV) {                                                                                                   \
    if (sp)                                                                                                                        \
      return d_ypool ? stem::launch<KSV, QV, true, true>(p, s, flops, bytes, "conv_stem_bf16x3+maxpool<" #KSV "x" #KSV ",Q" #QV ">")   \
                     : stem::launch<KSV, QV, false, true>(p, s, flops, bytes, "conv_stem_bf16x3<" #KSV "x" #KSV ",Q" #QV ">");       \
    return d_ypool ? stem::launch<KSV, QV, true>(p, s, flops, bytes, "conv_stem_bf16x3+maxpool<" #KSV "x" #KSV ",Q" #QV ">")         \
                   : stem::launch<KSV, QV, false>(p, s, flops, bytes, "conv_stem_bf16x3<" #KSV "x" #KSV ",Q" #QV ">");               \
  }
  MP_STEM_GO(7, 2) MP_STEM_GO(7, 3) MP_STEM_GO(7, 4) MP_STEM_GO(7, 5) MP_STEM_GO(7, 6)
  MP_STEM_GO(5, 2) MP_STEM_GO(5, 3) MP_STEM_GO(5, 4) MP_STEM_GO(5, 5) MP_STEM_GO(5, 6)
#undef MP_STEM_GO
  set_error("mp_conv_stem_xrec: no instance for %dx%d, record of %d elements", d->KH, d->KW, R);
  return MP_ERR_INVALID;
}

extern "C" int mp_conv_stem_xrec(const mp_conv_desc* d, const void* d_packed, int n_f32, mp_stream stream) {
  MP_REQUIRE(d && d->d_y, "mp_conv_stem_xrec: null output");
  return stem_xrec_impl(d, d_packed, n_f32, nullptr, 0, stream);
}

extern "C" int mp_conv_stem_xrec_pool(const mp_conv_desc* d, const void* d_packed, int n_f32, float* d_ypool, int pool_border, mp_stream stream) {
  MP_REQUIRE(d_ypool, "mp_conv_stem_xrec_pool: null pooled output");
  return stem_xrec_impl(d, d_packed, n_f32, d_ypool, pool_border, stream);
}

extern "C" int mp_conv_stem_xrec_sparse(const mp_conv_desc* d, const void* d_packed, const void* d_packed_sparse, int n_f32,
                                        const unsigned char* d_tile_flags, float* d_ypool, int pool_border, mp_stream stream) {
  MP_REQUIRE(d && (d->d_y || d_ypool), "mp_conv_stem_xrec_sparse: null output");
  return stem_xrec_impl(d, d_packed, n_f32, d_ypool, pool_border, stream, d_packed_sparse, d_tile_flags);
}

extern "C" int mp_conv_stem_bg_stats(double* background_wgs, double* total_wgs, int reset) {
  unsigned long long h[2] = {0, 0};
  MP_CHECK_HIP(hipDeviceSynchronize());
  MP_CHECK_HIP(hipMemcpyFromSymbol(h, HIP_SYMBOL(stem::g_stem_bg), sizeof(h)));
  if (background_wgs) *background_wgs = (double)h[0];
  if (total_wgs) *total_wgs = (double)h[1];
  if (reset) {
    const unsigned long long z[2] = {0, 0};
    MP_CHECK_HIP(hipMemcpyToSymbol(HIP_SYMBOL(stem::g_stem_bg), z, sizeof(z)));
  }
  return MP_OK;
}
```

### megapose6d_amd/engine.py

```python
from __future__ import annotations

import ctypes as C
from typing import Dict, List, Optional, Sequence, Tuple

import numpy as np
import torch

from . import _lib
from ._lib import ConvDesc, EngineError, Lights, MeshDesc, NamedTensor, check

RASTER_NORMALS = 1
RASTER_DEPTH = 2
RASTER_NORMALS_GL = 4
RASTER_MSAA4 = 16
RASTER_F16 = 32
RASTER_XREC = 64

BACKBONE_KINDS = {"vanilla_resnet34": 0, "resnet34": 1, "resnet18": 2}


def _stream() -> int:
    return torch.cuda.current_stream().cuda_stream


def _ptr(t: Optional[torch.Tensor]) -> Optional[int]:
    return None if t is None else t.data_ptr()


def _dev(t: torch.Tensor, dtype: torch.dtype) -> torch.Tensor:
    if not t.is_cuda:
        raise EngineError("engine tensors must live on the GPU")
    if t.dtype != dtype or not t.is_contiguous():
        t = t.to(dtype).contiguous()
    return t


def _dev_f32(t: torch.Tensor) -> torch.Tensor:
    return _dev(t, torch.float32)


def _dev_i32(t: torch.Tensor) -> torch.Tensor:
    return _dev(t, torch.int32)


def _workspace(n_bytes: int, device) -> torch.Tensor:
    return torch.empty(max(int(n_bytes), 256), dtype=torch.uint8, device=device)


class _Handle:
    _destroy = ""
    handle = None

    def close(self):
        if self.handle:
            getattr(_lib.load(), self._destroy)(self.handle)
            self.handle = None

    def __del__(self):
        try:
            self.close()
        except Exception:
            pass


def _named_tensors(state_dict: Dict[str, torch.Tensor]):
    items = [(k.encode(), np.ascontiguousarray(v.detach().cpu().numpy(), dtype=np.float32)) for k, v in state_dict.items()
             if torch.is_tensor(v) and v.dtype.is_floating_point]
    arr = (NamedTensor * len(items))()
    for i, (k, a) in enumerate(items):
        arr[i] = NamedTensor(k, a.ctypes.data, a.size)
    return arr, items


def clock_probe(ms_target: float = 20.0) -> Dict[str, float]:
    mhz, tf = C.c_double(0), C.c_double(0)
    check(_lib.load().mp_clock_probe(float(ms_target), C.byref(mhz), C.byref(tf), _stream()))
    return {"shader_mhz": mhz.value, "mfma_tflops": tf.value}


def conv_clock(reset: bool = True) -> float:
    mhz = C.c_double(0)
    check(_lib.load().mp_conv_clock_read(C.byref(mhz), 1 if reset else 0))
    return mhz.value


def conv_wino_stats(reset: bool = True) -> Tuple[float, float]:
    a, b = C.c_double(0), C.c_double(0)
    check(_lib.load().mp_conv_wino_stats(C.byref(a), C.byref(b), 1 if reset else 0))
    return a.value, b.value


_PROFILING = False


def profiling() -> bool:
    return _PROFILING


def profile_begin() -> None:
    global _PROFILING
    check(_lib.load().mp_profile_begin())
    _PROFILING = True


def profile_end() -> Dict[str, Dict[str, float]]:
    global _PROFILING
    lib = _lib.load()
    check(lib.mp_profile_end())
    _PROFILING = False
    out: Dict[str, Dict[str, float]] = {}
    i = 0
    while True:
        name = C.create_string_buffer(128)
        n, ms, fl, by, ex, pk = C.c_int64(0), C.c_double(0), C.c_double(0), C.c_double(0), C.c_double(0), C.c_double(0)
        rc = lib.mp_profile_query_ex(i, name, 128, C.byref(n), C.byref(ms), C.byref(fl), C.byref(by), C.byref(ex), C.byref(pk))
        if rc == 1:
            break
        check(rc)
        out[name.value.decode()] = {"launches": n.value, "ms": ms.value, "flops": fl.value, "bytes": by.value, "executed": ex.value,
                                    "peak_tflops": pk.value}
        i += 1
    return out


def device_info() -> Tuple[int, int, str]:
    lib = _lib.load()
    n_cu, lds = C.c_int(0), C.c_int(0)
    name = C.create_string_buffer(64)
    check(lib.mp_device_info(C.byref(n_cu), C.byref(lds), name, 64))
    return n_cu.value, lds.value, name.value.decode()


class MeshDB(_Handle):
    _destroy = "mp_mesh_db_destroy"

    def __init__(self, meshes: Sequence[Dict[str, np.ndarray]]):
        lib = _lib.load()
        self._keep = []
        descs = (MeshDesc * len(meshes))()
        for i, m in enumerate(meshes):
            v = np.ascontiguousarray(m["vertices"], dtype=np.float32)
            n = np.ascontiguousarray(m["normals"], dtype=np.float32)
            c = np.ascontiguousarray(m["colors"], dtype=np.float32)
            f = np.ascontiguousarray(m["faces"], dtype=np.int32)
            assert v.shape == n.shape == c.shape and v.shape[1] == 3 and f.shape[1] == 3
            self._keep += [v, n, c, f]
            descs[i] = MeshDesc(v.ctypes.data, n.ctypes.data, c.ctypes.data, f.ctypes.data, v.shape[0], f.shape[0])
        h = C.c_void_p()
        check(lib.mp_mesh_db_create(descs, len(meshes), C.byref(h)))
        self.handle = h
        self.n = len(meshes)
        self.max_vertices = lib.mp_mesh_db_max_vertices(h)
        for i, m in enumerate(meshes):
            if m.get("uvs") is not None and m.get("texture_mips") is not None:
                uv = np.ascontiguousarray(m["uvs"], dtype=np.float32)
                mips = m["texture_mips"]
                assert uv.shape == (np.asarray(m["faces"]).shape[0], 3, 2)
                th, tw = mips[0].shape[:2]
                flat = np.ascontiguousarray(np.concatenate([lv.reshape(-1) for lv in mips]).astype(np.uint32))
                check(lib.mp_mesh_db_set_texture(h, i, uv.ctypes.data, flat.ctypes.data, tw, th, len(mips)))
        self._keep = []
        self._ws: Dict[int, torch.Tensor] = {}

    def radius(self, i: int) -> float:
        return _lib.load().mp_mesh_db_radius(self.handle, i)

    def workspace(self, n_views: int, h: int, w: int, device, slot: int = 0) -> torch.Tensor:
        need = _lib.load().mp_raster_workspace_bytes(self.handle, n_views, h, w)
        ws = self._ws.get(slot)
        if ws is None or ws.numel() < need or ws.device != torch.device(device):
            self._ws[slot] = ws = torch.empty(max(need, 1), dtype=torch.uint8, device=device)
        return ws


def make_lights(ambient=(1.0, 1.0, 1.0), point_dirs=(), point_colors=(), point_offsets=None) -> Lights:
    L = Lights()
    L.ambient[:] = ambient
    L.n_point = len(point_dirs)
    for i, (d, c) in enumerate(zip(point_dirs, point_colors)):
        L.point_dir[i][:] = d
        L.point_color[i][:] = c
        L.point_offset[i][:] = point_offsets[i] if point_offsets is not None else (0.0, 0.0, 0.0)
    return L


class PackedObservation:

    def __init__(self, images: torch.Tensor):
        images = _dev_f32(images)
        self.n_im, self.C, self.H, self.W = (int(v) for v in images.shape)
        self.data = torch.empty(self.n_im, self.H, self.W, 4, dtype=torch.float32, device=images.device)
        check(_lib.load().mp_pack_observation_nhwc4(images.data_ptr(), self.n_im, self.C, self.H, self.W, self.data.data_ptr(), _stream()))


def raster_render(db: MeshDB, mesh_ids: torch.Tensor, TCO: torch.Tensor, K: torch.Tensor, h: int, w: int, flags: int,
                  lights: Lights, out: torch.Tensor, stride_v: int, stride_y: int, stride_x: int, c_rgb: int, c_normals: int,
                  c_depth: int, out_offset_floats: int = 0, views_per_item: int = 1, stride_view: int = 0, slot: int = 0,
                  crop=None, xrec=None) -> None:
    lib = _lib.load()
    n = int(TCO.shape[0])
    mesh_ids = _dev_i32(mesh_ids)
    TCO = _dev_f32(TCO)
    K = _dev_f32(K)
    assert out.dtype in (torch.float32, torch.float16, torch.bfloat16) and out.is_cuda
    es = out.element_size()
    flags = (flags | RASTER_F16) if out.dtype == torch.float16 else (flags & ~RASTER_F16)
    flags = (flags | RASTER_XREC) if out.dtype == torch.bfloat16 else (flags & ~RASTER_XREC)
    ws = db.workspace(n, h, w, out.device, slot)
    args = [db.handle, mesh_ids.data_ptr(), TCO.data_ptr(), K.data_ptr(), n, h, w, flags, C.byref(lights),
            out.data_ptr() + es * out_offset_floats, stride_v, views_per_item, stride_view, stride_y, stride_x, c_rgb, c_normals, c_depth,
            ws.data_ptr(), ws.numel()]
    if crop is not None:
        images, im_ids, boxes, c0 = crop
        if isinstance(images, PackedObservation):
            nhwc4, n_im, Cc, H, W, images = 1, images.n_im, images.C, images.H, images.W, images.data
        else:
            images = _dev_f32(images)
            nhwc4 = 0
            n_im, Cc, H, W = images.shape
        im_ids, boxes = _dev_i32(im_ids), _dev_f32(boxes)
        assert boxes.shape[0] * views_per_item == n and im_ids.shape[0] == boxes.shape[0]
        args += [images.data_ptr(), nhwc4, n_im, Cc, H, W, im_ids.data_ptr(), boxes.data_ptr()]
        if xrec is not None:
            assert out.dtype == torch.bfloat16 and c0 == 0
            f32_mask, tCR, depth_mode = xrec
            tCR = _dev_f32(tCR) if tCR is not None else None
            args[7] = flags & ~RASTER_XREC
            check(lib.mp_raster_render_xrec(*args, int(f32_mask) & 0xFFFFFFFF, _ptr(tCR), int(depth_mode), _stream()))
            return
        check(lib.mp_raster_render_crop(*args, c0, _stream()))
        return
    check(lib.mp_raster_render(*args, _stream()))


def lights_array(rigs: Sequence[Lights], device) -> torch.Tensor:
    arr = (Lights * max(len(rigs), 1))(*rigs)
    return torch.frombuffer(bytearray(arr), dtype=torch.uint8).to(device)


def raster_render_scene(db: MeshDB, obj_off: Sequence[int], mesh_ids: torch.Tensor, TCO: torch.Tensor, K: torch.Tensor, radius: torch.Tensor,
                        lights: torch.Tensor, h: int, w: int, flags: int, out: Optional[torch.Tensor], stride_v: int, stride_y: int,
                        stride_x: int, c_rgb: int, c_normals: int, c_depth: int, instance: Optional[torch.Tensor] = None) -> None:
    lib = _lib.load()
    n_cams = len(obj_off) - 1
    off = (C.c_int32 * len(obj_off))(*[int(v) for v in obj_off])
    dev = K.device
    d_off = torch.tensor([int(v) for v in obj_off], dtype=torch.int32, device=dev)
    mesh_ids, TCO, K, radius = _dev_i32(mesh_ids), _dev_f32(TCO), _dev_f32(K), _dev_f32(radius)
    assert out is None or (out.dtype == torch.float32 and out.is_cuda)
    assert instance is None or (instance.dtype == torch.int32 and instance.is_cuda and instance.is_contiguous() and instance.numel() >= n_cams * h * w)
    n_obj = int(obj_off[-1])
    need = lib.mp_raster_scene_workspace_bytes(db.handle, n_obj, h, w)
    ws = torch.empty(max(need, 1), dtype=torch.uint8, device=dev)
    check(lib.mp_raster_render_scene(db.handle, n_cams, off, d_off.data_ptr(), mesh_ids.data_ptr(), TCO.data_ptr(), K.data_ptr(),
                                     radius.data_ptr(), lights.data_ptr(), h, w, flags, _ptr(out), stride_v, stride_y, stride_x, c_rgb,
                                     c_normals, c_depth, _ptr(instance), ws.data_ptr(), ws.numel(), _stream()))


def raster_job_flags(db: MeshDB, n_views: int, h: int, w: int, device, slot: int = 0) -> int:
    ws = db.workspace(n_views, h, w, device, slot)
    return int(_lib.load().mp_raster_job_flags(db.handle, ws.data_ptr(), n_views, h, w) or 0)


def crop_roi_align(images: torch.Tensor, im_ids: torch.Tensor, boxes: torch.Tensor, out_h: int, out_w: int, out: torch.Tensor,
                   stride_b: int, stride_y: int, stride_x: int, c0: int, out_offset_floats: int = 0) -> None:
    lib = _lib.load()
    images = _dev_f32(images)
    n_im, Cc, H, W = images.shape
    check(lib.mp_crop_roi_align(images.data_ptr(), n_im, Cc, H, W, _dev_i32(im_ids).data_ptr(), _dev_f32(boxes).data_ptr(),
                                int(boxes.shape[0]), out_h, out_w, out.data_ptr() + 4 * out_offset_floats, stride_b, stride_y,
                                stride_x, c0, _stream()))


def normalize_depth(x: torch.Tensor, b: int, h: int, w: int, border: int, Cp: int, channels: Sequence[int], tCR: torch.Tensor,
                    mode: int) -> None:
    lib = _lib.load()
    ch = (C.c_int32 * len(channels))(*channels)
    fn = lib.mp_normalize_depth_f16 if x.dtype == torch.float16 else lib.mp_normalize_depth
    check(fn(x.data_ptr(), b, h, w, border, Cp, ch, len(channels), _dev_f32(tCR).data_ptr(), mode, _stream()))


DEPTH_NORM_MODES = {None: 0, "none": 0, "tCR_scale": 1, "tCR_scale_clamp_center": 2, "tCR_center_clamp": 3}


def padded_nhwc(n: int, h: int, w: int, c: int, border: int, device, slack: Optional[int] = None,
                dtype: torch.dtype = torch.float32) -> torch.Tensor:
    if slack is None:
        slack = (w + 2 * border) * c + 64
    return torch.zeros(n * (h + 2 * border) * (w + 2 * border) * c + slack, dtype=dtype, device=device)


def padded_view(buf: torch.Tensor, n: int, h: int, w: int, c: int, border: int) -> torch.Tensor:
    full = buf[: n * (h + 2 * border) * (w + 2 * border) * c].view(n, h + 2 * border, w + 2 * border, c)
    return full[:, border : border + h, border : border + w, :]


def _pack_weights(entry, w_oihw: np.ndarray, scale: Optional[np.ndarray], n_out: int, dtype, *dims) -> np.ndarray:
    w = np.ascontiguousarray(w_oihw, dtype=np.float32)
    sc = None if scale is None else np.ascontiguousarray(scale, dtype=np.float32)
    out = np.empty(n_out, dtype=dtype)
    check(entry(w.ctypes.data, *dims, None if sc is None else sc.ctypes.data, out.ctypes.data))
    return out


def _conv_desc(x: Optional[int], N: int, H: int, W: int, Cp: int, in_border: int, Cout: int, K: int, stride: int, pad: int,
               y: Optional[int] = None, out_border: int = 0, bias=None, residual=None, relu: bool = False, y_act=None, act_scale=None,
               act_shift=None) -> ConvDesc:
    d = ConvDesc()
    d.d_x, d.N, d.H, d.W, d.C, d.in_border = x, N, H, W, Cp, in_border
    d.d_bias = _ptr(bias)
    d.Cout, d.KH, d.KW, d.stride, d.pad = Cout, K, K, stride, pad
    d.d_y, d.out_border, d.d_residual, d.relu = y, out_border, _ptr(residual), int(relu)
    d.d_y_act, d.d_act_scale, d.d_act_shift = _ptr(y_act), _ptr(act_scale), _ptr(act_shift)
    return d


def conv_pack_weights(w_oihw: np.ndarray, cin_p: int, scale: Optional[np.ndarray] = None) -> np.ndarray:
    lib = _lib.load()
    Cout, Cin, KH, KW = np.shape(w_oihw)
    return _pack_weights(lib.mp_conv_pack_weights, w_oihw, scale, lib.mp_conv_packed_floats(cin_p, Cout, KH, KW), np.float32,
                         Cout, Cin, KH, KW, cin_p)


def conv2d_nhwc(x: torch.Tensor, N: int, H: int, W: int, Cp: int, in_border: int, w_packed: torch.Tensor,
                bias: Optional[torch.Tensor], Cout: int, K: int, stride: int, pad: int, y: Optional[torch.Tensor], out_border: int,
                residual: Optional[torch.Tensor] = None, relu: bool = False, y_act: Optional[torch.Tensor] = None,
                act_scale: Optional[torch.Tensor] = None, act_shift: Optional[torch.Tensor] = None,
                splitk_ws: Optional[torch.Tensor] = None) -> None:
    assert x.dtype in (torch.float32, torch.float16)
    d = _conv_desc(x.data_ptr(), N, H, W, Cp, in_border, Cout, K, stride, pad, _ptr(y), out_border, bias, residual, relu, y_act, act_scale,
                   act_shift)
    d.d_w, d.x_f16 = w_packed.data_ptr(), int(x.dtype == torch.float16)
    if splitk_ws is not None:
        d.d_splitk_ws, d.splitk_ws_floats = splitk_ws.data_ptr(), splitk_ws.numel()
    check(_lib.load().mp_conv2d_nhwc(C.byref(d), _stream()))


def conv_bf16x9_pack_weights(w_oihw: np.ndarray, cin_p: int, scale: Optional[np.ndarray] = None) -> np.ndarray:
    lib = _lib.load()
    Cout, Cin, KH, KW = np.shape(w_oihw)
    return _pack_weights(lib.mp_conv_bf16x9_pack_weights, w_oihw, scale, lib.mp_conv_bf16x9_packed_bytes(cin_p, Cout, KH, KW), np.uint8,
                         Cout, Cin, KH, KW, cin_p)


def conv2d_bf16x9_nhwc(x: torch.Tensor, N: int, H: int, W: int, Cp: int, in_border: int, w_pieces: torch.Tensor,
                       bias: Optional[torch.Tensor], Cout: int, K: int, stride: int, pad: int, y: Optional[torch.Tensor], out_border: int,
                       residual: Optional[torch.Tensor] = None, relu: bool = False, y_act: Optional[torch.Tensor] = None,
                       act_scale: Optional[torch.Tensor] = None, act_shift: Optional[torch.Tensor] = None) -> None:
    d = _conv_desc(x.data_ptr(), N, H, W, Cp, in_border, Cout, K, stride, pad, _ptr(y), out_border, bias, residual, relu, y_act, act_scale,
                   act_shift)
    d.d_w = w_pieces.data_ptr()
    check(_lib.load().mp_conv2d_bf16x9_nhwc(C.byref(d), w_pieces.data_ptr(), _stream()))


def conv_wino_pack_weights(w_oihw: np.ndarray, cin_p: int, scale: Optional[np.ndarray] = None) -> np.ndarray:
    lib = _lib.load()
    Cout, Cin, KH, KW = np.shape(w_oihw)
    assert KH == 3 and KW == 3
    return _pack_weights(lib.mp_conv_wino_pack_weights, w_oihw, scale, lib.mp_conv_wino_packed_floats(cin_p, Cout), np.float32,
                         Cout, Cin, cin_p)


def conv3x3_wino_nhwc(x: torch.Tensor, N: int, H: int, W: int, Cp: int, in_border: int, u_packed: torch.Tensor,
                      bias: Optional[torch.Tensor], Cout: int, y: Optional[torch.Tensor], out_border: int,
                      residual: Optional[torch.Tensor] = None, relu: bool = False, y_act: Optional[torch.Tensor] = None,
                      act_scale: Optional[torch.Tensor] = None, act_shift: Optional[torch.Tensor] = None) -> None:
    d = _conv_desc(x.data_ptr(), N, H, W, Cp, in_border, Cout, 3, 1, 1, _ptr(y), out_border, bias, residual, relu, y_act, act_scale,
                   act_shift)
    if u_packed.dtype == torch.uint8:
        check(_lib.load().mp_conv3x3_wino_bf16_nhwc(C.byref(d), u_packed.data_ptr(), _stream()))
        return
    check(_lib.load().mp_conv3x3_wino_nhwc(C.byref(d), u_packed.data_ptr(), _stream()))


def conv_wino_eligible(N: int, H: int, W: int, Cp: int, in_border: int, Cout: int, out_border: int, n_cu: int) -> bool:
    d = _conv_desc(None, N, H, W, Cp, in_border, Cout, 3, 1, 1, None, out_border)
    return bool(_lib.load().mp_conv_wino_eligible(C.byref(d), n_cu))


def conv_wino_bf16_pack_weights(w_oihw: np.ndarray, cin_p: int, scale: Optional[np.ndarray] = None) -> np.ndarray:
    lib = _lib.load()
    Cout, Cin, KH, KW = np.shape(w_oihw)
    assert KH == 3 and KW == 3
    return _pack_weights(lib.mp_conv_wino_bf16_pack_weights, w_oihw, scale, lib.mp_conv_wino_bf16_packed_bytes(cin_p, Cout), np.uint8,
                         Cout, Cin, cin_p)


def conv_wino_bf16_telemetry(on: bool) -> bool:
    return bool(_lib.load().mp_conv_wino_bf16_telemetry(int(bool(on))))


def conv_wino_bf16_stats(reset: bool = True) -> Tuple[float, float]:
    a, b = C.c_double(0), C.c_double(0)
    check(_lib.load().mp_conv_wino_bf16_stats(C.byref(a), C.byref(b), 1 if reset else 0))
    return a.value, b.value


def conv_wino_bf16_clock(reset: bool = True) -> Tuple[float, float]:
    a, b = C.c_double(0), C.c_double(0)
    check(_lib.load().mp_conv_wino_bf16_clock(C.byref(a), C.byref(b), 1 if reset else 0))
    return a.value, b.value


def leading_mask(n_f32: int) -> int:
    return (1 << int(n_f32)) - 1


def conv_stem_pack_weights(w_oihw: np.ndarray, n_f32: int, scale: Optional[np.ndarray] = None, f32_mask: Optional[int] = None) -> np.ndarray:
    lib = _lib.load()
    Cout, Cin, KH, KW = np.shape(w_oihw)
    assert KH == KW
    mask = leading_mask(n_f32) if f32_mask is None else int(f32_mask)
    nf = bin(mask).count("1")
    return _pack_weights(lib.mp_conv_stem_pack_weights_mask, w_oihw, scale, lib.mp_conv_stem_packed_bytes(KH, nf, Cin - nf, Cout), np.uint8,
                         Cout, Cin, KH, mask)


def xrec_elements(n_f32: int, n_u8: int) -> int:
    return int(_lib.load().mp_xrec_elements(n_f32, n_u8))


def conv_stem_pack_weights_sparse(w_oihw: np.ndarray, n_f32: int, scale: Optional[np.ndarray] = None) -> Optional[np.ndarray]:
    lib = _lib.load()
    Cout, Cin, KH, KW = np.shape(w_oihw)
    n = lib.mp_conv_stem_sparse_packed_bytes(KH, n_f32, Cin - n_f32, Cout)
    if n == 0:
        return None
    return _pack_weights(lib.mp_conv_stem_pack_weights_sparse, w_oihw, scale, n, np.uint8, Cout, Cin, KH, n_f32)


def conv_stem_bg_stats(reset: bool = True) -> Tuple[float, float]:
    a, b = C.c_double(), C.c_double()
    check(_lib.load().mp_conv_stem_bg_stats(C.byref(a), C.byref(b), int(reset)))
    return a.value, b.value


def conv_stem_xrec(xrec: torch.Tensor, N: int, H: int, W: int, c_real: int, n_f32: int, in_border: int, w_pieces: torch.Tensor,
                   bias: Optional[torch.Tensor], Cout: int, K: int, pad: int, y: Optional[torch.Tensor], out_border: int, relu: bool = False,
                   y_pool: Optional[torch.Tensor] = None, pool_border: int = 1, w_sparse: Optional[torch.Tensor] = None,
                   tile_flags: Optional[torch.Tensor] = None) -> None:
    assert xrec.dtype == torch.bfloat16 and w_pieces.dtype == torch.uint8
    d = _conv_desc(xrec.data_ptr(), N, H, W, (c_real + 3) // 4 * 4, in_border, Cout, K, 2, pad, _ptr(y), out_border, bias, relu=relu)
    d.c_real = c_real
    if w_sparse is not None and tile_flags is not None:
        assert tile_flags.dtype == torch.uint8 and tile_flags.is_cuda and w_sparse.dtype == torch.uint8
        check(_lib.load().mp_conv_stem_xrec_sparse(C.byref(d), w_pieces.data_ptr(), w_sparse.data_ptr(), n_f32, tile_flags.data_ptr(),
                                                   _ptr(y_pool), pool_border, _stream()))
        return
    if y_pool is not None:
        check(_lib.load().mp_conv_stem_xrec_pool(C.byref(d), w_pieces.data_ptr(), n_f32, y_pool.data_ptr(), pool_border, _stream()))
        return
    check(_lib.load().mp_conv_stem_xrec(C.byref(d), w_pieces.data_ptr(), n_f32, _stream()))


def conv2d_plan(N: int, H: int, W: int, Cp: int, in_border: int, Cout: int, K: int, stride: int, pad: int, n_cu: int,
                ws_floats: int = 0, x_f16: bool = False) -> Dict[str, int]:
    dummy = 0x1000
    d = _conv_desc(dummy, N, H, W, Cp, in_border, Cout, K, stride, pad, dummy, 1)
    d.d_w, d.x_f16 = dummy, int(x_f16)
    if ws_floats:
        d.d_splitk_ws, d.splitk_ws_floats = dummy, ws_floats
    out = (C.c_int32 * 5)()
    check(_lib.load().mp_conv2d_plan(C.byref(d), n_cu, out))
    return dict(zip(("mode", "k_split", "chunks_per_split", "n_main", "m_begin"), out))


def maxpool3x3s2(x, N, H, W, Cc, in_border, y, out_border, y_act=None, sc=None, sh=None) -> None:
    check(_lib.load().mp_maxpool3x3s2(x.data_ptr(), N, H, W, Cc, in_border, _ptr(y), out_border, _ptr(y_act), _ptr(sc), _ptr(sh),
                                      _stream()))


def bn_relu_nhwc(x, N, H, W, Cc, border, y_act, sc, sh) -> None:
    check(_lib.load().mp_bn_relu_nhwc(x.data_ptr(), N, H, W, Cc, border, y_act.data_ptr(), sc.data_ptr(), sh.data_ptr(), _stream()))


def pool_fc_heads(x, N, H, W, Cc, in_border, fc_w, fc_b, n_feat, head_w, head_b, n_out, feat, out, sigmoid) -> None:
    check(_lib.load().mp_pool_fc_heads(x.data_ptr(), N, H, W, Cc, in_border, _ptr(fc_w), _ptr(fc_b), n_feat, head_w.data_ptr(),
                                       head_b.data_ptr(), n_out, _ptr(feat), out.data_ptr(), _ptr(sigmoid), _stream()))


class Backbone(_Handle):
    _destroy = "mp_backbone_destroy"

    def __init__(self, kind: str, c_in: int, head: str, n_out: int, state_dict: Dict[str, torch.Tensor]):
        lib = _lib.load()
        width = 1
        if kind.startswith("resnet34_width="):
            width, kind = int(kind.split("resnet34_width=")[1]), "resnet34"
        if kind not in BACKBONE_KINDS:
            raise EngineError(f"unknown backbone '{kind}' (pose_models_cfg.py:106-118 supports {list(BACKBONE_KINDS)} and resnet34_width=N)")
        self.width = width
        arr, items = _named_tensors(state_dict)
        h = C.c_void_p()
        check(lib.mp_backbone_create_wide(BACKBONE_KINDS[kind], width, c_in, 0 if head == "pose" else 1, n_out, arr, len(items), C.byref(h)))
        self.handle = h
        self.kind, self.c_in, self.n_out = kind, c_in, n_out
        self.c_in_p = lib.mp_backbone_input_channels_padded(h)
        self.in_border = lib.mp_backbone_input_border(h)
        self._ws: Dict[int, torch.Tensor] = {}
        self._xrec_len: Dict[int, int] = {}

    def workspace(self, batch: int, h: int, w: int, device, slot: int = 0) -> torch.Tensor:
        need = _lib.load().mp_backbone_workspace_bytes(self.handle, batch, h, w)
        ws = self._ws.get(slot)
        if ws is None or ws.numel() < need or ws.device != torch.device(device):
            self._ws.pop(slot, None)
            self._ws[slot] = ws = torch.empty(need, dtype=torch.uint8, device=device)
            check(_lib.load().mp_backbone_workspace_reset(self.handle, ws.data_ptr()))
        return ws

    def flops(self, batch: int, h: int, w: int) -> float:
        return _lib.load().mp_backbone_flops(self.handle, batch, h, w)

    def xrec_elements(self, n_f32: int = 3, f32_mask: Optional[int] = None) -> int:
        mask = leading_mask(n_f32) if f32_mask is None else int(f32_mask)
        if mask >> 32 or (self.c_in < 32 and mask >> self.c_in):
            return 0
        hit = self._xrec_len.get(mask)
        if hit is None:
            hit = self._xrec_len[mask] = int(_lib.load().mp_backbone_xrec_prepare(self.handle, mask))
        return hit

    def forward(self, x: torch.Tensor, batch: int, h: int, w: int, out: torch.Tensor, sigmoid: Optional[torch.Tensor] = None,
                feat: Optional[torch.Tensor] = None, slot: int = 0, n_f32: int = 3, f32_mask: Optional[int] = None,
                tile_flags: int = 0) -> None:
        ws = self.workspace(batch, h, w, x.device, slot)
        assert x.dtype in (torch.float32, torch.float16, torch.bfloat16)
        lib = _lib.load()
        if x.dtype == torch.bfloat16:
            mask = leading_mask(n_f32) if f32_mask is None else int(f32_mask)
            self.xrec_elements(f32_mask=mask)
            if tile_flags:
                check(lib.mp_backbone_forward_xrec_sparse(self.handle, x.data_ptr(), mask & 0xFFFFFFFF, tile_flags, batch, h, w, out.data_ptr(),
                                                          _ptr(sigmoid), _ptr(feat), ws.data_ptr(), ws.numel(), _stream()))
                return
            check(lib.mp_backbone_forward_xrec_mask(self.handle, x.data_ptr(), mask & 0xFFFFFFFF, batch, h, w, out.data_ptr(), _ptr(sigmoid),
                                                    _ptr(feat), ws.data_ptr(), ws.numel(), _stream()))
            return
        fn = lib.mp_backbone_forward_f16 if x.dtype == torch.float16 else lib.mp_backbone_forward
        check(fn(self.handle, x.data_ptr(), batch, h, w, out.data_ptr(), _ptr(sigmoid), _ptr(feat), ws.data_ptr(), ws.numel(), _stream()))


def normalize_T(T: torch.Tensor) -> torch.Tensor:
    T = _dev_f32(T)
    out = torch.empty_like(T)
    check(_lib.load().mp_normalize_T(T.data_ptr(), T.shape[0], out.data_ptr(), _stream()))
    return out


def init_extents(points: torch.Tensor, R: torch.Tensor) -> torch.Tensor:
    points, R = _dev_f32(points), _dev_f32(R)
    n_mesh, n_pts, _ = points.shape
    ext = torch.empty(n_mesh, R.shape[0], 2, dtype=torch.float32, device=points.device)
    check(_lib.load().mp_init_extents(points.data_ptr(), n_mesh, n_pts, R.data_ptr(), R.shape[0], ext.data_ptr(), _stream()))
    return ext


def init_poses_from_boxes(boxes, K, mesh_ids, rot_ids, R, ext) -> torch.Tensor:
    boxes, K, R, ext = _dev_f32(boxes), _dev_f32(K), _dev_f32(R), _dev_f32(ext)
    b = boxes.shape[0]
    TCO = torch.empty(b, 4, 4, dtype=torch.float32, device=boxes.device)
    check(_lib.load().mp_init_poses_from_boxes(boxes.data_ptr(), K.data_ptr(), _dev_i32(mesh_ids).data_ptr(),
                                               _dev_i32(rot_ids).data_ptr(), R.data_ptr(), R.shape[0], ext.data_ptr(), b,
                                               TCO.data_ptr(), _stream()))
    return TCO


MV_MODES = {"TCO": 0, "1view_TCO": 0, "TCO+front_3views": 1, "TCO+front_1view": 2, "sphere_26views": 3}
MV_REMOVE_TCO, MV_INPLANE = 256, 512


def multiview_n_views(multiview: int) -> int:
    return int(_lib.load().mp_pose_multiview_n_views(int(multiview)))


def pose_prepare(TCO_in, K, mesh_ids, points, n_pts_main: int, n_pts_views: int, V: int, multiview: int, im_hw, out_hw,
                 lamb: float = 1.4, with_K_main: bool = False):
    TCO_in, K, points = _dev_f32(TCO_in), _dev_f32(K), _dev_f32(points)
    b = TCO_in.shape[0]
    dev = TCO_in.device
    f = dict(dtype=torch.float32, device=dev)
    TCO_n = torch.empty(b, 4, 4, **f)
    tCR = torch.empty(b, 3, **f)
    TCV_O = torch.empty(b, V, 4, 4, **f)
    KV = torch.empty(b, V, 3, 3, **f)
    boxes_rend = torch.empty(b, 4, **f)
    boxes_crop = torch.empty(b, 4, **f)
    K_main = torch.empty(b, 3, 3, **f) if with_K_main else None
    check(_lib.load().mp_pose_prepare_ex(TCO_in.data_ptr(), K.data_ptr(), _dev_i32(mesh_ids).data_ptr(), points.data_ptr(),
                                         points.shape[1], n_pts_main, n_pts_views, b, V, multiview, im_hw[0], im_hw[1], out_hw[0],
                                         out_hw[1], lamb, TCO_n.data_ptr(), tCR.data_ptr(), TCV_O.data_ptr(), KV.data_ptr(),
                                         boxes_rend.data_ptr(), boxes_crop.data_ptr(), _ptr(K_main), _stream()))
    if with_K_main:
        return TCO_n, tCR, TCV_O, KV, boxes_rend, boxes_crop, K_main
    return TCO_n, tCR, TCV_O, KV, boxes_rend, boxes_crop


def pose_update(TCO, K_crop, out9, tCR, k_stride_floats: int = 9) -> torch.Tensor:
    TCO, out9, tCR = _dev_f32(TCO), _dev_f32(out9), _dev_f32(tCR)
    assert K_crop.dtype == torch.float32 and K_crop.is_cuda
    out = torch.empty_like(TCO)
    check(_lib.load().mp_pose_update(TCO.data_ptr(), K_crop.data_ptr(), k_stride_floats, out9.data_ptr(), tCR.data_ptr(),
                                     TCO.shape[0], out.data_ptr(), _stream()))
    return out


POSE_ERROR_MEAN, POSE_ERROR_MAX = 0, 1


def _pose_error_points(points: torch.Tensor, mesh_ids, n_points, b: int):
    points = _dev_f32(points)
    if points.dim() != 3 or points.shape[-1] != 3 or points.shape[1] < 1:
        raise EngineError(f"points must be [n_mesh, n_pts >= 1, 3], got {tuple(points.shape)}")
    if mesh_ids is None:
        if points.shape[0] != b:
            raise EngineError("without mesh ids the points are per row: [b, n_pts, 3]")
        mesh_ids = torch.arange(b, dtype=torch.int32, device=points.device)
    return points, _dev_i32(mesh_ids), (None if n_points is None else _dev_i32(n_points))


def pose_error_workspace(b: int, n_pts: int, S_max: int, device) -> torch.Tensor:
    return _workspace(_lib.load().mp_pose_error_workspace_bytes(b, n_pts, S_max), device)


def _pose_error_sym_set(entry, T_pred, T_gt, symmetries, n_sym, points, mesh_ids, n_points, reduce, split, with_errs, with_alt,
                        K=None, with_diffs=None) -> Dict[str, torch.Tensor]:
    T_pred, T_gt = _dev_f32(T_pred), _dev_f32(T_gt)
    b = T_pred.shape[0]
    if K is not None:
        K = _dev_f32(K)
        if K.shape != (b, 3, 3):
            raise EngineError(f"K must be [b,3,3], got {tuple(K.shape)}")
    points, mesh_ids, n_points = _pose_error_points(points, mesh_ids, n_points, b)
    if symmetries is not None:
        symmetries = _dev_f32(symmetries)
        S = symmetries.shape[1]
        if T_gt.shape != (b, 4, 4):
            raise EngineError(f"T_gt must be [b,4,4], got {tuple(T_gt.shape)}")
    else:
        if T_gt.dim() != 4 or T_gt.shape[0] != b:
            raise EngineError(f"candidate poses must be [b,S,4,4], got {tuple(T_gt.shape)}")
        S = T_gt.shape[1]
    n_sym = None if symmetries is None or n_sym is None else _dev_i32(n_sym)
    n_pts = points.shape[1]
    dev = T_pred.device
    f = dict(dtype=torch.float32, device=dev)
    out = dict(err=torch.empty(b, **f), idx=torch.empty(b, dtype=torch.int32, device=dev), T_gt_sym=torch.empty(b, 4, 4, **f))
    if with_errs:
        out["errs"] = torch.empty(b, S, **f)
    if with_diffs:
        out["diffs"] = torch.empty(b, n_pts, 3, **f)
    if with_alt:
        out["err_alt"] = torch.empty(b, **f)
    ws = pose_error_workspace(b, n_pts, S, dev)
    check(entry(T_pred.data_ptr(), T_gt.data_ptr(), _ptr(symmetries), _ptr(n_sym), S, points.data_ptr(), n_pts, mesh_ids.data_ptr(),
                _ptr(n_points), n_pts, b, int(reduce), int(split), *([] if K is None else [K.data_ptr()]), out["err"].data_ptr(),
                _ptr(out.get("err_alt")), out["idx"].data_ptr(), out["T_gt_sym"].data_ptr(), _ptr(out.get("errs")),
                *([] if with_diffs is None else [_ptr(out.get("diffs"))]), ws.data_ptr(), ws.numel(), _stream()))
    return out


def pose_error_sym(T_pred: torch.Tensor, T_gt: torch.Tensor, symmetries: Optional[torch.Tensor], n_sym: Optional[torch.Tensor],
                   points: torch.Tensor, mesh_ids: Optional[torch.Tensor] = None, n_points: Optional[torch.Tensor] = None,
                   reduce: int = POSE_ERROR_MEAN, split: int = 0, with_errs: bool = True, with_diffs: bool = False,
                   with_alt: bool = False) -> Dict[str, torch.Tensor]:
    return _pose_error_sym_set(_lib.load().mp_pose_error_sym, T_pred, T_gt, symmetries, n_sym, points, mesh_ids, n_points, reduce, split,
                               with_errs, with_alt, with_diffs=bool(with_diffs))


def pose_error_nn(T_pred: torch.Tensor, T_gt: torch.Tensor, points: torch.Tensor, mesh_ids: Optional[torch.Tensor] = None,
                  n_points: Optional[torch.Tensor] = None, split: int = 0, with_diffs: bool = True,
                  with_assign: bool = True) -> Dict[str, torch.Tensor]:
    T_pred, T_gt = _dev_f32(T_pred), _dev_f32(T_gt)
    b = T_pred.shape[0]
    points, mesh_ids, n_points = _pose_error_points(points, mesh_ids, n_points, b)
    n_pts = points.shape[1]
    dev = T_pred.device
    f = dict(dtype=torch.float32, device=dev)
    out = dict(mean=torch.empty(b, **f), max=torch.empty(b, **f))
    if with_diffs:
        out["diffs"] = torch.empty(b, n_pts, 3, **f)
    if with_assign:
        out["assign"] = torch.empty(b, n_pts, dtype=torch.int32, device=dev)
    ws = pose_error_workspace(b, n_pts, 1, dev)
    check(_lib.load().mp_pose_error_nn(T_pred.data_ptr(), T_gt.data_ptr(), points.data_ptr(), n_pts, mesh_ids.data_ptr(), _ptr(n_points),
                                       n_pts, b, int(split), _ptr(out.get("diffs")), _ptr(out.get("assign")), out["mean"].data_ptr(),
                                       out["max"].data_ptr(), ws.data_ptr(), ws.numel(), _stream()))
    return out


def pose_error_rigid(T_a: torch.Tensor, T_b: torch.Tensor, K: Optional[torch.Tensor] = None, points: Optional[torch.Tensor] = None,
                     mesh_ids: Optional[torch.Tensor] = None, n_points: Optional[torch.Tensor] = None) -> Dict[str, torch.Tensor]:
    T_a, T_b = _dev_f32(T_a), _dev_f32(T_b)
    b = T_a.shape[0]
    f = dict(dtype=torch.float32, device=T_a.device)
    out = dict(trans_err=torch.empty(b, **f), rot_err_deg=torch.empty(b, **f))
    n_pts = 0
    if K is not None:
        K = _dev_f32(K)
        points, mesh_ids, n_points = _pose_error_points(points, mesh_ids, n_points, b)
        n_pts = points.shape[1]
        out["proj_error"] = torch.empty(b, **f)
    check(_lib.load().mp_pose_error_rigid(T_a.data_ptr(), T_b.data_ptr(), b, _ptr(K), _ptr(points) if K is not None else None,
                                          n_pts, _ptr(mesh_ids) if K is not None else None, _ptr(n_points) if K is not None else None, n_pts,
                                          out["trans_err"].data_ptr(), out["rot_err_deg"].data_ptr(), _ptr(out.get("proj_error")), _stream()))
    return out


def pose_error_mspd(T_pred: torch.Tensor, T_gt: torch.Tensor, symmetries: Optional[torch.Tensor], n_sym: Optional[torch.Tensor],
                    points: torch.Tensor, K: torch.Tensor, mesh_ids: Optional[torch.Tensor] = None, n_points: Optional[torch.Tensor] = None,
                    reduce: int = POSE_ERROR_MAX, split: int = 0, with_errs: bool = True, with_alt: bool = False) -> Dict[str, torch.Tensor]:
    return _pose_error_sym_set(_lib.load().mp_pose_error_mspd, T_pred, T_gt, symmetries, n_sym, points, mesh_ids, n_points, reduce, split,
                               with_errs, with_alt, K=K)


def _row_ids(name: str, ids: Optional[torch.Tensor], maps: torch.Tensor, b: int) -> Optional[torch.Tensor]:
    if ids is None:
        if maps.shape[0] < b:
            raise EngineError(f"without {name} the maps are per row: need {b}, got {maps.shape[0]}")
        return None
    ids = _dev_i32(ids)
    if ids.shape != (b,):
        raise EngineError(f"{name} must be [b], got {tuple(ids.shape)}")
    return ids


VSD_TAUS = tuple(0.05 * k for k in range(1, 11))


def vsd(depth_est: torch.Tensor, depth_gt: torch.Tensor, depth_test: torch.Tensor, K: torch.Tensor, diameter: torch.Tensor,
        delta: float = 0.015, taus=None, normalized_by_diameter: bool = True, est_ids: Optional[torch.Tensor] = None,
        gt_ids: Optional[torch.Tensor] = None, im_ids: Optional[torch.Tensor] = None, split: int = 0,
        with_counts: bool = True) -> Dict[str, torch.Tensor]:
    depth_est, depth_gt, depth_test = _dev_f32(depth_est), _dev_f32(depth_gt), _dev_f32(depth_test)
    K, diameter = _dev_f32(K), _dev_f32(diameter)
    if depth_est.dim() != 3 or depth_gt.dim() != 3 or depth_test.dim() != 3 or depth_gt.shape[1:] != depth_est.shape[1:] \
            or depth_test.shape[1:] != depth_est.shape[1:]:
        raise EngineError(f"depth maps must be [n,h,w] of one size, got {tuple(depth_est.shape)}, {tuple(depth_gt.shape)}, {tuple(depth_test.shape)}")
    b = K.shape[0]
    if K.shape != (b, 3, 3) or diameter.shape != (b,):
        raise EngineError(f"K must be [b,3,3] and diameter [b], got {tuple(K.shape)}, {tuple(diameter.shape)}")
    h, w = depth_est.shape[1:]
    ids = [_row_ids("est_ids", est_ids, depth_est, b), _row_ids("gt_ids", gt_ids, depth_gt, b), _row_ids("im_ids", im_ids, depth_test, b)]
    taus = [float(t) for t in (VSD_TAUS if taus is None else taus)]
    n_tau = len(taus)
    h_taus = (C.c_float * max(n_tau, 1))(*taus)
    dev = K.device
    out = dict(errs=torch.empty(b, n_tau, dtype=torch.float32, device=dev))
    if with_counts:
        out["counts"] = torch.empty(b, 2 + n_tau, dtype=torch.int32, device=dev)
    lib = _lib.load()
    ws = _workspace(lib.mp_vsd_workspace_bytes(b, n_tau), dev)
    check(lib.mp_vsd(depth_est.data_ptr(), _ptr(ids[0]), depth_gt.data_ptr(), _ptr(ids[1]), depth_test.data_ptr(), _ptr(ids[2]),
                     depth_est.shape[0], depth_gt.shape[0], depth_test.shape[0], K.data_ptr(), diameter.data_ptr(), b, h, w, float(delta),
                     C.cast(h_taus, C.c_void_p), n_tau, int(bool(normalized_by_diameter)), int(split), out["errs"].data_ptr(),
                     _ptr(out.get("counts")), ws.data_ptr(), ws.numel(), _stream()))
    return out


def gt_info(depth_gt: torch.Tensor, depth_test: torch.Tensor, K: torch.Tensor, canvas: int = 3, delta: float = 0.015,
            gt_ids: Optional[torch.Tensor] = None, im_ids: Optional[torch.Tensor] = None, with_masks: bool = False,
            split: int = 0) -> Dict[str, torch.Tensor]:
    depth_gt, depth_test, K = _dev_f32(depth_gt), _dev_f32(depth_test), _dev_f32(K)
    if depth_gt.dim() == 3 and canvas == 1:
        depth_gt = depth_gt.unsqueeze(1)
    if depth_gt.dim() != 4 or depth_test.dim() != 3 or depth_gt.shape[1] != canvas * canvas or depth_gt.shape[2:] != depth_test.shape[1:]:
        raise EngineError(f"depth_gt must be [n_gt,{canvas * canvas},h,w] and depth_test [n_im,h,w], got {tuple(depth_gt.shape)}, {tuple(depth_test.shape)}")
    b = K.shape[0]
    if K.shape != (b, 3, 3):
        raise EngineError(f"K must be [b,3,3], got {tuple(K.shape)}")
    h, w = depth_test.shape[1:]
    ids = [_row_ids("gt_ids", gt_ids, depth_gt, b), _row_ids("im_ids", im_ids, depth_test, b)]
    dev = K.device
    out = dict(counts=torch.empty(b, 4, dtype=torch.int32, device=dev), boxes=torch.empty(b, 8, dtype=torch.int32, device=dev),
               visib_fract=torch.empty(b, dtype=torch.float32, device=dev))
    if with_masks:
        out["mask"] = torch.empty(b, h, w, dtype=torch.uint8, device=dev)
        out["mask_visib"] = torch.empty(b, h, w, dtype=torch.uint8, device=dev)
    lib = _lib.load()
    ws = _workspace(lib.mp_gt_info_workspace_bytes(b), dev)
    check(lib.mp_gt_info(depth_gt.data_ptr(), _ptr(ids[0]), depth_test.data_ptr(), _ptr(ids[1]), depth_gt.shape[0], depth_test.shape[0],
                         K.data_ptr(), b, h, w, int(canvas), float(delta), int(split), out["counts"].data_ptr(), out["boxes"].data_ptr(),
                         out["visib_fract"].data_ptr(), _ptr(out.get("mask")), _ptr(out.get("mask_visib")), ws.data_ptr(), ws.numel(),
                         _stream()))
    return out


BOP_MATCH_MAX_ERRORS = 16
BOP_MATCH_MAX_THETAS = 16
BOP_MATCH_MASK_BITS = 64
BOP_MATCH_STAGE_FLOATS = 4096
BOP_MATCH_INDEX = ("cand_gt", "cand_lgt", "est_row", "est_off", "group_est_off", "group_n_gt", "group_taken_off")


def bop_match_limits() -> Dict[str, int]:
    v = [C.c_int(0) for _ in range(4)]
    check(_lib.load().mp_bop_match_limits(*[C.byref(x) for x in v]))
    return dict(zip(("max_errors", "max_thetas", "mask_bits", "stage_floats"), (int(x.value) for x in v)))


def _match_index(index: Dict[str, torch.Tensor], c: int, n_groups: Optional[int], checked: Sequence[str], misfit: str,
                 n_top: Optional[torch.Tensor]):
    ix = {k: _dev_i32(index[k]) for k in BOP_MATCH_INDEX}
    n_est = ix["est_row"].shape[0]
    if n_groups is None:
        n_groups = ix["group_n_gt"].shape[0]
    shape = dict(cand_gt=(c,), cand_lgt=(c,), est_off=(n_est + 1,), group_est_off=(n_groups + 1,), group_n_gt=(n_groups,),
                 group_taken_off=(n_groups + 1,))
    if any(ix[k].shape != shape[k] for k in checked):
        raise EngineError(misfit)
    if n_top is not None:
        n_top = _dev_i32(n_top)
        if n_top.shape != (n_groups,):
            raise EngineError(f"n_top must be [n_groups], got {tuple(n_top.shape)}")
    n_words = int(index["n_taken_words"])
    return ix, [ix[k].data_ptr() for k in BOP_MATCH_INDEX], n_top, n_est, n_groups, n_words


def bop_match(errs: torch.Tensor, index: Dict[str, torch.Tensor], thr: torch.Tensor, n_pred: int,
              n_top: Optional[torch.Tensor] = None) -> torch.Tensor:
    errs = _dev_f32(errs)
    if errs.dim() != 2:
        raise EngineError(f"errs must be [C,E], got {tuple(errs.shape)}")
    dev = errs.device
    c, e = errs.shape
    thr = thr.to(device=dev, dtype=torch.float64).contiguous()
    if thr.dim() != 3 or thr.shape[1] != e:
        raise EngineError(f"thr must be [n_groups,{e},n_theta], got {tuple(thr.shape)}")
    n_groups, _, n_theta = thr.shape
    ix, ix_ptrs, n_top, n_est, n_groups, n_words = _match_index(
        index, c, n_groups, BOP_MATCH_INDEX[:2] + BOP_MATCH_INDEX[3:], "the index does not fit errs [C,E] and thr [n_groups,E,n_theta]", n_top)
    match = torch.empty(int(n_pred), e, n_theta, dtype=torch.int32, device=dev)
    lib = _lib.load()
    ws = _workspace(lib.mp_bop_match_workspace_bytes(n_words, e, n_theta), dev)
    check(lib.mp_bop_match(errs.data_ptr(), *ix_ptrs, _ptr(n_top), thr.data_ptr(), int(n_pred), c, n_est, n_groups, n_words, e, n_theta,
                           match.data_ptr(), ws.data_ptr(), ws.numel(), _stream()))
    return match


DET_MATCH_MAX_THETAS = 16
MASK_PAIR_MAX_PAIRS = 1 << 23


def _dev_bytes(name: str, t: torch.Tensor) -> torch.Tensor:
    t = _dev(t, t.dtype)
    if t.dtype == torch.bool:
        t = t.view(torch.uint8)
    if t.dtype != torch.uint8:
        raise EngineError(f"{name} must be uint8 or bool, got {t.dtype}")
    return t


def mask_pair_counts(pred_masks: torch.Tensor, gt_masks: torch.Tensor, cand_pred: torch.Tensor, cand_gt: torch.Tensor,
                     split: int = 0) -> torch.Tensor:
    pred_masks, gt_masks = _dev_bytes("pred_masks", pred_masks), _dev_bytes("gt_masks", gt_masks)
    if pred_masks.dim() != 3 or gt_masks.dim() != 3 or pred_masks.shape[1:] != gt_masks.shape[1:]:
        raise EngineError(f"masks must be [P,H,W] and [G,H,W], got {tuple(pred_masks.shape)}, {tuple(gt_masks.shape)}")
    cand_pred, cand_gt = _dev_i32(cand_pred), _dev_i32(cand_gt)
    if cand_pred.dim() != 1 or cand_pred.shape != cand_gt.shape:
        raise EngineError(f"cand_pred and cand_gt must be [C], got {tuple(cand_pred.shape)}, {tuple(cand_gt.shape)}")
    c = cand_pred.shape[0]
    h, w = pred_masks.shape[1:]
    counts = torch.empty(c, 3, dtype=torch.int32, device=pred_masks.device)
    lib = _lib.load()
    for c0 in range(0, max(c, 1), MASK_PAIR_MAX_PAIRS):
        n = min(c, c0 + MASK_PAIR_MAX_PAIRS) - c0
        check(lib.mp_mask_pair_counts(pred_masks.data_ptr(), gt_masks.data_ptr(), cand_pred[c0:].data_ptr(), cand_gt[c0:].data_ptr(),
                                      pred_masks.shape[0], gt_masks.shape[0], n, h, w, int(split), counts[c0:].data_ptr(), _stream()))
    return counts


def det_match(iou: torch.Tensor, index: Dict[str, torch.Tensor], gt_ignore: torch.Tensor, thr: torch.Tensor, n_pred: int,
              n_top: Optional[torch.Tensor] = None) -> torch.Tensor:
    iou = _dev(iou, torch.float64)
    dev = iou.device
    thr = thr.to(device=dev, dtype=torch.float64).contiguous()
    if iou.dim() != 1 or thr.dim() != 1:
        raise EngineError(f"iou must be [C] and thr [n_theta], got {tuple(iou.shape)}, {tuple(thr.shape)}")
    c, n_theta = iou.shape[0], thr.shape[0]
    gt_ignore = _dev_bytes("gt_ignore", gt_ignore)
    misfit = "the index does not fit iou [C]"
    if gt_ignore.dim() != 1:
        raise EngineError(misfit)
    ix, ix_ptrs, n_top, n_est, n_groups, n_words = _match_index(
        index, c, None, ("cand_gt", "cand_lgt", "est_off", "group_est_off", "group_taken_off"), misfit, n_top)
    match = torch.empty(int(n_pred), n_theta, dtype=torch.int32, device=dev)
    lib = _lib.load()
    ws = _workspace(lib.mp_det_match_workspace_bytes(n_words, n_theta), dev)
    check(lib.mp_det_match(iou.data_ptr(), *ix_ptrs, _ptr(n_top), gt_ignore.data_ptr(), thr.data_ptr(), int(n_pred), c, n_est, n_groups,
                           n_words, n_theta, match.data_ptr(), ws.data_ptr(), ws.numel(), _stream()))
    return match


MODEL_INFO_TILE_STEP = 64
MODEL_INFO_MAX_TILE = 1024


def model_info(points: torch.Tensor, n_points, tile: int = 0) -> Tuple[torch.Tensor, torch.Tensor, torch.Tensor]:
    points = _dev_f32(points)
    if points.dim() != 3 or points.shape[2] != 3:
        raise EngineError(f"points must be [n_obj,stride,3], got {tuple(points.shape)}")
    n_obj, stride = int(points.shape[0]), int(points.shape[1])
    h_n = np.ascontiguousarray(n_points.cpu().numpy() if isinstance(n_points, torch.Tensor) else n_points).astype(np.int32)
    if h_n.shape != (n_obj,) or n_obj < 1 or h_n.min() < 1 or h_n.max() > stride:
        raise EngineError(f"n_points must be [n_obj] with every count in 1 .. {stride}")
    dev = points.device
    d_n = torch.from_numpy(h_n).to(dev)
    lib = _lib.load()
    n_bytes = lib.mp_model_info_scratch_bytes(n_obj, h_n.ctypes.data, int(tile))
    if n_bytes == 0:
        raise EngineError(f"model_info: tile {tile} is not 0 or a multiple of {MODEL_INFO_TILE_STEP} up to {MODEL_INFO_MAX_TILE}, or too many jobs")
    ws = _workspace(n_bytes, dev)
    d2 = torch.empty(n_obj, dtype=torch.float32, device=dev)
    pair = torch.empty(n_obj, 2, dtype=torch.int32, device=dev)
    bounds = torch.empty(n_obj, 6, dtype=torch.float32, device=dev)
    check(lib.mp_model_info(points.data_ptr(), stride, d_n.data_ptr(), h_n.ctypes.data, n_obj, int(tile), ws.data_ptr(), d2.data_ptr(),
                            pair.data_ptr(), bounds.data_ptr(), _stream()))
    return d2, pair, bounds


OVERLAY_OUTPUTS = ("contour", "mesh", "canny", "mask")
OVERLAY_MAX_DILATE = 8
OVERLAY_MAX_THICKNESS = 8
OVERLAY_MAX_SIDE = 8192


def _overlay_images(name: str, t: torch.Tensor, like: Optional[torch.Tensor] = None) -> torch.Tensor:
    t = _dev_bytes(name, t)
    if t.dim() != 4 or t.shape[3] != 3 or (like is not None and t.shape != like.shape):
        raise EngineError(f"{name} must be uint8 [n,h,w,3]" + ("" if like is None else f" like images {tuple(like.shape)}") + f", got {tuple(t.shape)}")
    n, h, w = (int(v) for v in t.shape[:3])
    if not (1 <= h <= OVERLAY_MAX_SIDE and 1 <= w <= OVERLAY_MAX_SIDE) or n * h * w * 3 >= 2 ** 31:
        raise EngineError(f"{name}: h and w must be in 1 .. {OVERLAY_MAX_SIDE} and n * h * w * 3 below 2^31, got {tuple(t.shape)}")
    return t


def _overlay_colors(colors, device) -> torch.Tensor:
    colors = torch.as_tensor(colors, dtype=torch.uint8).to(device).contiguous()
    if colors.dim() != 2 or colors.shape[0] < 1 or colors.shape[1] != 3:
        raise EngineError(f"colors must be uint8 [n_colors,3] with n_colors >= 1, got {tuple(colors.shape)}")
    return colors


def overlay(images: torch.Tensor, render: Optional[torch.Tensor] = None, labels: Optional[torch.Tensor] = None, colors=((0, 255, 0),),
            dilate_iterations: int = 1, outputs: Sequence[str] = ("contour", "mesh", "canny", "mask")) -> Dict[str, torch.Tensor]:
    images = _overlay_images("images", images)
    dev = images.device
    n, h, w = (int(v) for v in images.shape[:3])
    outputs = tuple(outputs)
    if any(o not in OVERLAY_OUTPUTS for o in outputs) or len(set(outputs)) != len(outputs):
        raise EngineError(f"outputs must be distinct names of {OVERLAY_OUTPUTS}, got {outputs}")
    if render is None and labels is None:
        raise EngineError("overlay needs a render or a label map")
    if render is None and "mesh" in outputs:
        raise EngineError("the mesh blend needs a render")
    if render is not None:
        render = _overlay_images("render", render, images)
    if labels is not None:
        labels = _dev_i32(labels)
        if labels.shape != images.shape[:3]:
            raise EngineError(f"labels must be int32 [n,h,w] like images {tuple(images.shape)}, got {tuple(labels.shape)}")
    colors = _overlay_colors(colors, dev)
    k = int(dilate_iterations)
    if not 0 <= k <= OVERLAY_MAX_DILATE:
        raise EngineError(f"dilate_iterations must be in 0 .. {OVERLAY_MAX_DILATE}, got {dilate_iterations}")
    out = {o: torch.empty((n, h, w, 3) if o in ("contour", "mesh") else (n, h, w), dtype=torch.uint8, device=dev) for o in outputs}
    check(_lib.load().mp_overlay(images.data_ptr(), _ptr(render), _ptr(labels), colors.data_ptr(), colors.shape[0], n, h, w, k,
                                 _ptr(out.get("contour")), _ptr(out.get("canny")), _ptr(out.get("mask")), _ptr(out.get("mesh")), _stream()))
    return out


def draw_boxes(images: torch.Tensor, boxes: torch.Tensor, image_ids: torch.Tensor, colors=((255, 0, 0),), thickness: int = 2) -> torch.Tensor:
    images = _overlay_images("images", images)
    dev = images.device
    n, h, w = (int(v) for v in images.shape[:3])
    boxes, image_ids = _dev_f32(boxes), _dev_i32(image_ids)
    if boxes.dim() != 2 or boxes.shape[1] != 4 or image_ids.shape != boxes.shape[:1]:
        raise EngineError(f"boxes must be [n_boxes,4] and image_ids [n_boxes], got {tuple(boxes.shape)}, {tuple(image_ids.shape)}")
    colors = _overlay_colors(colors, dev)
    t = int(thickness)
    if not 1 <= t <= OVERLAY_MAX_THICKNESS:
        raise EngineError(f"thickness must be in 1 .. {OVERLAY_MAX_THICKNESS}, got {thickness}")
    out = torch.empty_like(images)
    check(_lib.load().mp_draw_boxes(images.data_ptr(), boxes.data_ptr(), image_ids.data_ptr(), boxes.shape[0], colors.data_ptr(), colors.shape[0],
                                    n, h, w, t, out.data_ptr(), _stream()))
    return out


SURFACE_BLOCK_STEP = 64
SURFACE_MAX_BLOCK = 2048
SURFACE_MAX_FACES = 1 << 22


def surface_sample(vertices: torch.Tensor, faces: torch.Tensor, vert_off, face_off, u: torch.Tensor, block: int = 0) -> Tuple[torch.Tensor, torch.Tensor]:
    vertices, faces, u = _dev_f32(vertices), _dev_i32(faces), _dev_f32(u)
    if vertices.dim() != 2 or vertices.shape[1] != 3 or faces.dim() != 2 or faces.shape[1] != 3:
        raise EngineError(f"vertices must be [V_total,3] and faces [F_total,3], got {tuple(vertices.shape)} and {tuple(faces.shape)}")
    if u.dim() != 3 or u.shape[2] != 3 or u.shape[0] < 1 or u.shape[1] < 1:
        raise EngineError(f"u must be [n_obj,count,3] with n_obj, count >= 1, got {tuple(u.shape)}")
    n_obj, count = int(u.shape[0]), int(u.shape[1])
    h_vo, h_fo = (np.ascontiguousarray(o.cpu().numpy() if isinstance(o, torch.Tensor) else o).astype(np.int64) for o in (vert_off, face_off))
    if h_vo.shape != (n_obj + 1,) or h_fo.shape != (n_obj + 1,) or h_vo[0] != 0 or h_fo[0] != 0 or h_vo[-1] != vertices.shape[0] or h_fo[-1] != faces.shape[0]:
        raise EngineError(f"vert_off and face_off must be [n_obj + 1 = {n_obj + 1}], start at 0 and end at {vertices.shape[0]} vertices and {faces.shape[0]} faces")
    if (np.diff(h_vo) < 0).any() or (np.diff(h_fo) < 1).any() or (np.diff(h_fo) > SURFACE_MAX_FACES).any():
        raise EngineError(f"vert_off must not descend, and every object must have 1 .. {SURFACE_MAX_FACES} faces")
    h_vo, h_fo = h_vo.astype(np.int32), h_fo.astype(np.int32)
    dev = vertices.device
    lib = _lib.load()
    n_bytes = lib.mp_surface_sample_scratch_bytes(n_obj, h_fo.ctypes.data, count, int(block))
    if n_bytes == 0:
        raise EngineError(f"surface_sample: block {block} is not 0 or a multiple of {SURFACE_BLOCK_STEP} up to {SURFACE_MAX_BLOCK}, or it cuts an object "
                          f"into more than {SURFACE_MAX_BLOCK} blocks, or too many objects")
    d_vo, d_fo = torch.from_numpy(h_vo).to(dev), torch.from_numpy(h_fo).to(dev)
    ws = _workspace(n_bytes, dev)
    points = torch.empty(n_obj, count, 3, dtype=torch.float32, device=dev)
    face = torch.empty(n_obj, count, dtype=torch.int32, device=dev)
    check(lib.mp_surface_sample(vertices.data_ptr(), faces.data_ptr(), d_vo.data_ptr(), d_fo.data_ptr(), h_vo.ctypes.data, h_fo.ctypes.data, n_obj,
                                u.data_ptr(), count, int(block), ws.data_ptr(), points.data_ptr(), face.data_ptr(), _stream()))
    return points, face


def icp_refine(depth_meas: torch.Tensor, im_ids: torch.Tensor, depth_rend: torch.Tensor, K_images: torch.Tensor, K_rows: torch.Tensor,
               TCO: torch.Tensor, n_iterations: int = 100, n_levels: int = 4, tolerance: float = 0.05, n_min_points: int = 1000,
               user_masks: bool = False, association: str = "nn", return_iters: bool = False, masks: Optional[torch.Tensor] = None):
    lib = _lib.load()
    depth_meas, depth_rend = _dev_f32(depth_meas), _dev_f32(depth_rend)
    K_images, K_rows, TCO = _dev_f32(K_images), _dev_f32(K_rows), _dev_f32(TCO)
    n_im, H, W = depth_meas.shape
    N = TCO.shape[0]
    assert depth_rend.shape == (N, H, W)
    dev = TCO.device
    out = torch.empty_like(TCO)
    retval = torch.empty(N, dtype=torch.int32, device=dev)
    residual = torch.empty(N, dtype=torch.float32, device=dev)
    if association == "nn":
        if user_masks:
            raise ValueError('association="nn" takes the caller\'s masks through `masks`, not pre-multiplied into the depth')
        if masks is not None:
            masks = (masks.to(dev) > 0).to(torch.uint8).contiguous()
            assert masks.shape == depth_meas.shape
        ws = torch.empty(lib.mp_icp_nn_workspace_bytes(n_im, N, H, W), dtype=torch.uint8, device=dev)
        iters = torch.zeros(N, 8, dtype=torch.int32, device=dev) if return_iters else None
        check(lib.mp_icp_refine_nn(depth_meas.data_ptr(), n_im, _dev_i32(im_ids).data_ptr(), depth_rend.data_ptr(), K_images.data_ptr(),
                                   K_rows.data_ptr(), TCO.data_ptr(), N, H, W, n_iterations, n_levels, tolerance, n_min_points, _ptr(masks),
                                   out.data_ptr(), retval.data_ptr(), residual.data_ptr(), _ptr(iters), ws.data_ptr(), ws.numel(), _stream()))
        return (out, retval, residual, iters) if return_iters else (out, retval, residual)
    if association != "projective":
        raise ValueError(f"association must be 'nn' or 'projective', got {association!r}")
    if masks is not None:
        raise ValueError('association="projective" takes masks pre-multiplied into depth_meas (user_masks=True)')
    ws = torch.empty(lib.mp_icp_workspace_bytes(n_im, N, H, W), dtype=torch.uint8, device=dev)
    check(lib.mp_icp_refine(depth_meas.data_ptr(), n_im, _dev_i32(im_ids).data_ptr(), depth_rend.data_ptr(), K_images.data_ptr(),
                            K_rows.data_ptr(), TCO.data_ptr(), N, H, W, n_iterations, n_levels, tolerance, n_min_points, int(user_masks), out.data_ptr(),
                            retval.data_ptr(), residual.data_ptr(), ws.data_ptr(), ws.numel(), _stream()))
    return out, retval, residual


TEASER_MAX_POINTS = 1024
TEASER_MASK_TYPES = {"simple": 0, "threshold": 1}
TEASER_SELECTIONS = {"kcore": 0, "none": 1, "max_clique": 2}
TEASER_TIM_GRAPHS = {"chain": 0, "complete": 1}
TEASER_INFO = ("N", "M", "n_selected", "gnc_iterations", "num_inliers")
TEASER_CLIQUE_INFO = ("size", "upper_bound", "exact", "steps")


def _teaser_mode(name: str, table: Dict[str, int], value: str) -> int:
    if value not in table:
        raise EngineError(f"{name} must be one of {sorted(table)}, got {value!r}")
    return table[value]


def farthest_point_sample(points: torch.Tensor, counts: torch.Tensor, n_points: int, use_fps: bool = True) -> Tuple[torch.Tensor, torch.Tensor]:
    points, counts = _dev_f32(points), _dev_i32(counts)
    if points.dim() != 3 or points.shape[2] != 3 or points.shape[1] < 1 or counts.shape != (points.shape[0],) or int(n_points) < 1:
        raise EngineError(f"points must be [n,stride >= 1,3], counts [n] and n_points >= 1, got {tuple(points.shape)}, {tuple(counts.shape)}, {n_points}")
    n, stride = int(points.shape[0]), int(points.shape[1])
    lib = _lib.load()
    ws = _workspace(lib.mp_fps_workspace_bytes(n, stride), points.device)
    idx = torch.empty(n, int(n_points), dtype=torch.int32, device=points.device)
    m = torch.empty(n, dtype=torch.int32, device=points.device)
    check(lib.mp_fps(points.data_ptr(), counts.data_ptr(), n, stride, int(n_points), int(bool(use_fps)), idx.data_ptr(), m.data_ptr(), ws.data_ptr(),
                     ws.numel(), _stream()))
    return idx, m


def max_clique_step_limits() -> Tuple[int, int]:
    default = int(_lib.load().mp_max_clique_default_steps())
    return default, 16 * default


def _clique_steps(max_steps: Optional[int]) -> int:
    default, ceiling = max_clique_step_limits()
    if max_steps is None:
        return default
    if not 0 <= int(max_steps) <= ceiling:
        raise EngineError(f"the step budget of the maximum-clique search must be 0 .. {ceiling}, got {max_steps}")
    return int(max_steps)


def max_clique(adjacency: torch.Tensor, counts: Optional[torch.Tensor] = None, max_steps: Optional[int] = None) -> Tuple[torch.Tensor, torch.Tensor]:
    if adjacency.dim() != 3 or adjacency.shape[1] != adjacency.shape[2] or not 1 <= adjacency.shape[1] <= TEASER_MAX_POINTS:
        raise EngineError(f"adjacency must be [n,stride,stride] with stride 1 .. {TEASER_MAX_POINTS}, got {tuple(adjacency.shape)}")
    steps = _clique_steps(max_steps)
    adj = _dev(adjacency != 0, torch.uint8)
    n, stride, dev = int(adj.shape[0]), int(adj.shape[1]), adj.device
    if counts is not None:
        counts = _dev_i32(counts)
        if counts.shape != (n,):
            raise EngineError(f"counts must be [{n}], got {tuple(counts.shape)}")
    lib = _lib.load()
    ws = _workspace(lib.mp_max_clique_workspace_bytes(n, stride), dev)
    members = torch.empty(n, stride, dtype=torch.int32, device=dev)
    info = torch.empty(n, len(TEASER_CLIQUE_INFO), dtype=torch.int32, device=dev)
    check(lib.mp_max_clique(adj.data_ptr(), _ptr(counts), n, stride, steps, members.data_ptr(), info.data_ptr(), ws.data_ptr(), ws.numel(), _stream()))
    return members, info


def _teaser_telemetry(n: int, stride: int, device, want: bool):
    if not want:
        return None, None, None, None
    return tuple(torch.full((n, stride), -1, dtype=torch.int32, device=device) for _ in range(3)) + (torch.zeros(n, len(TEASER_INFO), dtype=torch.int32, device=device),)


def _clique_info(n: int, device, want: bool):
    return torch.zeros(n, len(TEASER_CLIQUE_INFO), dtype=torch.int32, device=device) if want else None


def teaser_solve(src: torch.Tensor, dst: torch.Tensor, counts: torch.Tensor, noise_bound: float = 0.01, min_num_inliers: int = 0,
                 inlier_selection: str = "kcore", rotation_tim_graph: str = "chain", telemetry: bool = False, max_clique_steps: Optional[int] = None):
    src, dst, counts = _dev_f32(src), _dev_f32(dst), _dev_i32(counts)
    if src.dim() != 3 or src.shape[2] != 3 or dst.shape != src.shape or not 1 <= src.shape[1] <= TEASER_MAX_POINTS or counts.shape != (src.shape[0],):
        raise EngineError(f"src and dst must be [n,1 .. {TEASER_MAX_POINTS},3] and counts [n], got {tuple(src.shape)}, {tuple(dst.shape)}, {tuple(counts.shape)}")
    sel, graph = _teaser_mode("inlier_selection", TEASER_SELECTIONS, inlier_selection), _teaser_mode("rotation_tim_graph", TEASER_TIM_GRAPHS, rotation_tim_graph)
    n, stride, dev = int(src.shape[0]), int(src.shape[1]), src.device
    lib = _lib.load()
    steps = _clique_steps(max_clique_steps)
    ws = _workspace(lib.mp_teaser_workspace_bytes_ex(n, 0, 0, stride, sel), dev)
    Rt = torch.empty(n, 3, 4, dtype=torch.float64, device=dev)
    retval = torch.empty(n, dtype=torch.int32, device=dev)
    degree, core, selected, info = _teaser_telemetry(n, stride, dev, telemetry)
    clique = _clique_info(n, dev, telemetry and inlier_selection == "max_clique")
    check(lib.mp_teaser_solve_ex(src.data_ptr(), dst.data_ptr(), counts.data_ptr(), n, stride, float(noise_bound), sel, graph, int(min_num_inliers),
                                 Rt.data_ptr(), retval.data_ptr(), _ptr(degree), _ptr(core), _ptr(selected), _ptr(info), steps, _ptr(clique), ws.data_ptr(),
                                 ws.numel(), _stream()))
    if not telemetry:
        return Rt, retval
    tel = dict(degree=degree, core=core, selected=selected, info=info)
    if clique is not None:
        tel["clique"] = clique
    return Rt, retval, tel


def teaser_refine(depth_meas: torch.Tensor, im_ids: torch.Tensor, depth_rend: torch.Tensor, K_rows: torch.Tensor, TCO: torch.Tensor,
                  mask_type: str = "simple", depth_delta_thresh: float = 0.1, n_min_points: int = 100, n_points: int = 1000,
                  noise_bound: float = 0.01, min_num_inliers: int = 50, use_farthest_point_sampling: bool = True,
                  inlier_selection: str = "kcore", rotation_tim_graph: str = "chain", telemetry: bool = False, max_clique_steps: Optional[int] = None):
    depth_meas, depth_rend, K_rows, TCO, im_ids = _dev_f32(depth_meas), _dev_f32(depth_rend), _dev_f32(K_rows), _dev_f32(TCO), _dev_i32(im_ids)
    if depth_meas.dim() != 3 or TCO.dim() != 3 or TCO.shape[1:] != (4, 4):
        raise EngineError(f"depth_meas must be [B,H,W] and TCO [N,4,4], got {tuple(depth_meas.shape)} and {tuple(TCO.shape)}")
    n_im, H, W = (int(v) for v in depth_meas.shape)
    N, dev = int(TCO.shape[0]), TCO.device
    if depth_rend.shape != (N, H, W) or K_rows.shape != (N, 3, 3) or im_ids.shape != (N,):
        raise EngineError(f"depth_rend must be [{N},{H},{W}], K_rows [{N},3,3], im_ids [{N}]")
    if not 1 <= int(n_points) <= TEASER_MAX_POINTS:
        raise EngineError(f"n_points must be 1 .. {TEASER_MAX_POINTS}, got {n_points}")
    mask = _teaser_mode("mask_type", TEASER_MASK_TYPES, mask_type)
    sel, graph = _teaser_mode("inlier_selection", TEASER_SELECTIONS, inlier_selection), _teaser_mode("rotation_tim_graph", TEASER_TIM_GRAPHS, rotation_tim_graph)
    lib = _lib.load()
    steps = _clique_steps(max_clique_steps)
    ws = _workspace(lib.mp_teaser_workspace_bytes_ex(N, H, W, int(n_points), sel), dev)
    out = torch.empty_like(TCO)
    retval = torch.empty(N, dtype=torch.int32, device=dev)
    degree, core, selected, _ = _teaser_telemetry(N, int(n_points), dev, telemetry)
    info = torch.zeros(N, len(TEASER_INFO), dtype=torch.int32, device=dev)
    Rt = torch.empty(N, 3, 4, dtype=torch.float64, device=dev) if telemetry else None
    sample_idx = torch.empty(N, int(n_points), dtype=torch.int32, device=dev) if telemetry else None
    clique = _clique_info(N, dev, telemetry and inlier_selection == "max_clique")
    check(lib.mp_teaser_refine_ex(depth_meas.data_ptr(), n_im, im_ids.data_ptr(), depth_rend.data_ptr(), K_rows.data_ptr(), TCO.data_ptr(), N, H, W, mask,
                                  float(depth_delta_thresh), int(n_min_points), int(n_points), float(noise_bound), int(min_num_inliers),
                                  int(bool(use_farthest_point_sampling)), sel, graph, out.data_ptr(), retval.data_ptr(), _ptr(Rt), _ptr(sample_idx),
                                  _ptr(degree), _ptr(core), _ptr(selected), info.data_ptr(), steps, _ptr(clique), ws.data_ptr(), ws.numel(), _stream()))
    if not telemetry:
        return out, retval, info
    tel = dict(Rt=Rt, sample_idx=sample_idx, degree=degree, core=core, selected=selected)
    if clique is not None:
        tel["clique"] = clique
    return out, retval, info, tel


class DetectorNet(_Handle):
    _destroy = "mp_detector_destroy"

    def __init__(self, state_dict: Dict[str, torch.Tensor], n_classes: int, min_size: int, max_size: int, **overrides):
        lib = _lib.load()
        self.cfg = _lib.DetectorConfig()
        check(lib.mp_detector_default_config(C.byref(self.cfg), n_classes, min_size, max_size))
        for k, v in overrides.items():
            if not hasattr(self.cfg, k):
                raise EngineError(f"unknown detector option '{k}'")
            cur = getattr(self.cfg, k)
            if hasattr(cur, "__len__"):
                cur[:] = list(v)
            else:
                setattr(self.cfg, k, v)
        arr, items = _named_tensors(state_dict)
        h = C.c_void_p()
        check(lib.mp_detector_create(C.byref(self.cfg), arr, len(items), C.byref(h)))
        self.handle = h
        self.n_classes = n_classes
        self._ws: Optional[torch.Tensor] = None

    @staticmethod
    def state_spec(n_classes: int) -> List[Tuple[str, Tuple[int, ...]]]:
        lib = _lib.load()
        out, i = [], 0
        while True:
            name = C.create_string_buffer(160)
            shp, nd = (C.c_int64 * 4)(), C.c_int32(0)
            rc = lib.mp_detector_state_spec(n_classes, i, name, 160, shp, C.byref(nd))
            if rc == 1:
                return out
            check(rc)
            out.append((name.value.decode(), tuple(int(s) for s in shp[: nd.value])))
            i += 1

    def forward(self, images: torch.Tensor, with_masks: bool = True):
        lib = _lib.load()
        images = _dev_f32(images)
        n, c, H, W = images.shape
        if c != 3:
            raise EngineError("the detector takes RGB images [n,3,H,W]")
        dev = images.device
        D = int(self.cfg.box_detections_per_img)
        need = lib.mp_detector_workspace_bytes(self.handle, n, H, W)
        if need == 0:
            raise EngineError(f"mp_detector_workspace_bytes failed for {n} x {H} x {W}: {lib.mp_last_error().decode()}")
        if self._ws is None or self._ws.numel() < need or self._ws.device != dev:
            self._ws = torch.empty(need, dtype=torch.uint8, device=dev)
        boxes = torch.empty(n, D, 4, dtype=torch.float32, device=dev)
        scores = torch.empty(n, D, dtype=torch.float32, device=dev)
        labels = torch.empty(n, D, dtype=torch.int32, device=dev)
        counts = torch.empty(n, dtype=torch.int32, device=dev)
        masks = torch.empty(n, D, H, W, dtype=torch.float32, device=dev) if with_masks else None
        check(lib.mp_detector_forward(self.handle, images.data_ptr(), n, H, W, boxes.data_ptr(), scores.data_ptr(), labels.data_ptr(),
                                      counts.data_ptr(), _ptr(masks), self._ws.data_ptr(), self._ws.numel(), _stream()))
        return boxes, scores, labels, counts, masks

    def debug_tensor(self, what: str) -> torch.Tensor:
        lib = _lib.load()
        ptr, shp, border, rs, n_el = C.c_void_p(), (C.c_int64 * 4)(), C.c_int32(0), C.c_int64(0), C.c_int64(0)
        check(lib.mp_detector_debug_tensor(self.handle, what.encode(), C.byref(ptr), shp, C.byref(border), C.byref(rs), C.byref(n_el)))
        off = ptr.value - self._ws.data_ptr()
        is_int = what in ("proposal_counts", "f_cnt")
        flat = self._ws[off : off + 4 * n_el.value].view(torch.int32 if is_int else torch.float32).clone()
        s, b = [int(v) for v in shp], border.value
        if b:
            return flat.view(s[0], s[1] + 2 * b, s[2] + 2 * b, s[3])[:, b : b + s[1], b : b + s[2]].contiguous()
        if s[2] == 4:
            return flat.view(s[0], s[1], 4)
        if rs.value > 1:
            return flat.view(s[0], rs.value)[:, : s[1]].contiguous()
        return flat.view(s[0], s[1])
```

Measured before the change: 2290.

## Pack the stem's last partial channel chunk as a compact tail plane

Adds a tail form for the xrec stem convolution. The last 16-byte channel chunk of each input pixel is re-packed in LDS into a per-row plane of one element per kernel column, and matching weight blobs are packed for it, for both the dense and the background-sparse paths. This cuts the number of MFMA K-steps when that chunk is only partly used, so less padded work runs in the stem. In exchange there is an extra LDS transpose pass, a further __syncthreads, a larger patch pitch, and more kernel template instantiations. It is on by default and can be disabled with MP_STEM_TAIL=0.

```diff
diff --git a/include/mp_engine.h b/include/mp_engine.h
--- a/include/mp_engine.h
+++ b/include/mp_engine.h
@@ -160,6 +160,13 @@
 int mp_conv_stem_pack_weights_sparse(const float* h_w_oihw, int Cout, int Cin, int KS, int n_f32, const float* h_scale, void* h_packed);
 int mp_conv_stem_xrec_sparse(const mp_conv_desc* desc, const void* d_packed, const void* d_packed_sparse, int n_f32,
                              const unsigned char* d_tile_flags, float* d_ypool, int pool_border, mp_stream stream);
+
+int mp_conv_stem_tail_forms(int KS, int n_f32, int n_u8);
+size_t mp_conv_stem_tail_packed_bytes(int KS, int n_f32, int n_u8, int Cout, int background);
+int mp_conv_stem_pack_weights_tail(const float* h_w_oihw, int Cout, int Cin, int KS, uint32_t f32_mask, int background, const float* h_scale,
+                                   void* h_packed);
+int mp_conv_stem_xrec_tail(const mp_conv_desc* desc, const void* d_packed, const void* d_packed_sparse, int n_f32,
+                           const unsigned char* d_tile_flags, float* d_ypool, int pool_border, int tail_forms, mp_stream stream);
 
 int mp_maxpool3x3s2(const float* d_x, int N, int H, int W, int C, int in_border, float* d_y,
                     int out_border, float* d_y_act, const float* d_act_scale, const float* d_act_shift,
diff --git a/megapose6d_amd/_lib.py b/megapose6d_amd/_lib.py
--- a/megapose6d_amd/_lib.py
+++ b/megapose6d_amd/_lib.py
@@ -134,6 +134,10 @@
     "mp_conv_stem_sparse_packed_bytes": (_sz, [_i, _i, _i, _i]),
     "mp_conv_stem_pack_weights_sparse": (_i, [_vp, _i, _i, _i, _i, _vp, _vp]),
     "mp_conv_stem_xrec_sparse": (_i, [C.POINTER(ConvDesc), _vp, _vp, _i, _vp, _vp, _i, _vp]),
+    "mp_conv_stem_tail_forms": (_i, [_i, _i, _i]),
+    "mp_conv_stem_tail_packed_bytes": (_sz, [_i, _i, _i, _i, _i]),
+    "mp_conv_stem_pack_weights_tail": (_i, [_vp, _i, _i, _i, _u32, _i, _vp, _vp]),
+    "mp_conv_stem_xrec_tail": (_i, [C.POINTER(ConvDesc), _vp, _vp, _i, _vp, _vp, _i, _i, _vp]),
     "mp_conv_stem_bg_stats": (_i, [C.POINTER(C.c_double), C.POINTER(C.c_double), _i]),
     "mp_conv_stem_xrec": (_i, [C.POINTER(ConvDesc), _vp, _i, _vp]),
     "mp_conv_stem_xrec_pool": (_i, [C.POINTER(ConvDesc), _vp, _i, _vp, _i, _vp]),
diff --git a/megapose6d_amd/csrc/backbone.hip b/megapose6d_amd/csrc/backbone.hip
--- a/megapose6d_amd/csrc/backbone.hip
+++ b/megapose6d_amd/csrc/backbone.hip
@@ -30,6 +30,7 @@
   int stageC[4] = {64, 128, 256, 512};
   bool wide;
   bool direct_bf16 = true;
+  bool stem_tail = true;
   ConvLayer stem;
   std::vector<Block> blocks;
   std::vector<int> stage_of_block;
@@ -39,6 +40,7 @@
   std::mutex blob_mu;
   std::map<uint32_t, void*> stem_blobs;
   std::map<uint32_t, void*> stem_blobs_sparse;
+  std::map<uint32_t, int> stem_tail_forms;
   struct WsKey { void* ptr; int batch, h, w; };
   std::vector<WsKey> ws_known;
 };
@@ -111,6 +113,7 @@
   bb->kind = kind;
   bb->wide = kind != MP_BACKBONE_VANILLA_RESNET34;
   bb->direct_bf16 = !(getenv("MP_CONV_DIRECT_BF16") && atoi(getenv("MP_CONV_DIRECT_BF16")) == 0);
+  bb->stem_tail = !(getenv("MP_STEM_TAIL") && atoi(getenv("MP_STEM_TAIL")) == 0);
   bb->c_in = c_in;
   bb->c_in_p = (c_in + 3) / 4 * 4;
   bb->head_kind = head_kind;
@@ -207,29 +210,38 @@
   if (!mp_conv_stem_supported(bb->stem.K, n_f32, n_u8) || bb->stem.Cout % 64 != 0) return 0;
   std::lock_guard<std::mutex> blob_lock(bb->blob_mu);
   if (!bb->stem_blobs.count(f32_mask)) {
-    std::vector<unsigned char> blob(mp_conv_stem_packed_bytes(bb->stem.K, n_f32, n_u8, bb->stem.Cout));
-    if (mp_conv_stem_pack_weights_mask(bb->stem_w_host.data(), bb->stem.Cout, bb->c_in, bb->stem.K, f32_mask,
-                                       bb->stem_scale_host.empty() ? nullptr : bb->stem_scale_host.data(), blob.data()) != MP_OK)
+    const bool leading = f32_mask == (n_f32 >= 32 ? 0xFFFFFFFFu : (1u << n_f32) - 1u);
+    int forms = bb->stem_tail ? mp_conv_stem_tail_forms(bb->stem.K, n_f32, n_u8) & (leading ? 3 : 1) : 0;
+    const float* h_scale = bb->stem_scale_host.empty() ? nullptr : bb->stem_scale_host.data();
+    std::vector<unsigned char> blob((forms & 1) ? mp_conv_stem_tail_packed_bytes(bb->stem.K, n_f32, n_u8, bb->stem.Cout, 0)
+                                                : mp_conv_stem_packed_bytes(bb->stem.K, n_f32, n_u8, bb->stem.Cout));
+    if (((forms & 1) ? mp_conv_stem_pack_weights_tail(bb->stem_w_host.data(), bb->stem.Cout, bb->c_in, bb->stem.K, f32_mask, 0, h_scale, blob.data())
+                     : mp_conv_stem_pack_weights_mask(bb->stem_w_host.data(), bb->stem.Cout, bb->c_in, bb->stem.K, f32_mask, h_scale, blob.data())) != MP_OK)
       return 0;
     void* d = nullptr;
     if (hipMalloc(&d, blob.size()) != hipSuccess) return 0;
     if (hipMemcpy(d, blob.data(), blob.size(), hipMemcpyHostToDevice) != hipSuccess) { (void)hipFree(d); return 0; }
     bb->allocs.push_back(d);
     bb->stem_blobs[f32_mask] = d;
-    if (f32_mask == (n_f32 >= 32 ? 0xFFFFFFFFu : (1u << n_f32) - 1u) && mp_conv_stem_sparse_chunks(bb->stem.K, n_f32, n_u8) > 0) {
-      std::vector<unsigned char> sb(mp_conv_stem_sparse_packed_bytes(bb->stem.K, n_f32, n_u8, bb->stem.Cout));
+    bool have_sparse = false;
+    if (leading && ((forms & 2) || mp_conv_stem_sparse_chunks(bb->stem.K, n_f32, n_u8) > 0)) {
+      std::vector<unsigned char> sb((forms & 2) ? mp_conv_stem_tail_packed_bytes(bb->stem.K, n_f32, n_u8, bb->stem.Cout, 1)
+                                                : mp_conv_stem_sparse_packed_bytes(bb->stem.K, n_f32, n_u8, bb->stem.Cout));
       void* ds = nullptr;
-      if (mp_conv_stem_pack_weights_sparse(bb->stem_w_host.data(), bb->stem.Cout, bb->c_in, bb->stem.K, n_f32,
-                                           bb->stem_scale_host.empty() ? nullptr : bb->stem_scale_host.data(), sb.data()) == MP_OK &&
+      if (((forms & 2) ? mp_conv_stem_pack_weights_tail(bb->stem_w_host.data(), bb->stem.Cout, bb->c_in, bb->stem.K, f32_mask, 1, h_scale, sb.data())
+                       : mp_conv_stem_pack_weights_sparse(bb->stem_w_host.data(), bb->stem.Cout, bb->c_in, bb->stem.K, n_f32, h_scale, sb.data())) == MP_OK &&
           hipMalloc(&ds, sb.size()) == hipSuccess) {
         if (hipMemcpy(ds, sb.data(), sb.size(), hipMemcpyHostToDevice) == hipSuccess) {
           bb->allocs.push_back(ds);
           bb->stem_blobs_sparse[f32_mask] = ds;
+          have_sparse = true;
         } else {
           (void)hipFree(ds);
         }
       }
     }
+    if (!have_sparse) forms &= 1;
+    bb->stem_tail_forms[f32_mask] = forms;
   }
   return mp_xrec_elements(n_f32, n_u8);
 }
@@ -269,12 +281,15 @@
   if (x_mode == 2) {
     const void* d_stem_pieces = nullptr;
     const void* d_sparse_blob = nullptr;
+    int tail_forms = 0;
     {
       std::lock_guard<std::mutex> blob_lock(bb->blob_mu);
       const auto blob_it = bb->stem_blobs.find(f32_mask);
       if (blob_it != bb->stem_blobs.end()) d_stem_pieces = blob_it->second;
       const auto sp_it = bb->stem_blobs_sparse.find(f32_mask);
       if (sp_it != bb->stem_blobs_sparse.end()) d_sparse_blob = sp_it->second;
+      const auto tf_it = bb->stem_tail_forms.find(f32_mask);
+      if (tf_it != bb->stem_tail_forms.end()) tail_forms = tf_it->second;
     }
     MP_REQUIRE(d_stem_pieces != nullptr, "mp_backbone_forward_xrec: no piece blob for the fp32-kind channel mask 0x%x of this %d-channel stem: "
                "call mp_backbone_xrec_prepare first (it returns 0 if the stem has no exact-piece form)", f32_mask, bb->c_in);
@@ -288,13 +303,15 @@
     const void* d_sparse = d_tile_flags ? d_sparse_blob : nullptr;
     if (fuse_pool) {
       d.d_y = nullptr;
-      rc = d_sparse ? mp_conv_stem_xrec_sparse(&d, d_stem_pieces, d_sparse, n_f32, d_tile_flags, A[0], 1, s)
-                    : mp_conv_stem_xrec_pool(&d, d_stem_pieces, n_f32, A[0], 1, s);
+      rc = tail_forms ? mp_conv_stem_xrec_tail(&d, d_stem_pieces, d_sparse, n_f32, d_sparse ? d_tile_flags : nullptr, A[0], 1, tail_forms, s)
+           : d_sparse ? mp_conv_stem_xrec_sparse(&d, d_stem_pieces, d_sparse, n_f32, d_tile_flags, A[0], 1, s)
+                      : mp_conv_stem_xrec_pool(&d, d_stem_pieces, n_f32, A[0], 1, s);
       if (!rc && bb->wide) rc = mp_bn_relu_nhwc(A[0], batch, g.hs[0], g.ws[0], bb->stageC[0], 1, Aact[0], bb->blocks[0].pre.d_scale, bb->blocks[0].pre.d_shift, s);
       stem_pooled = true;
     } else {
-      rc = d_sparse ? mp_conv_stem_xrec_sparse(&d, d_stem_pieces, d_sparse, n_f32, d_tile_flags, nullptr, 0, s)
-                    : mp_conv_stem_xrec(&d, d_stem_pieces, n_f32, s);
+      rc = tail_forms ? mp_conv_stem_xrec_tail(&d, d_stem_pieces, d_sparse, n_f32, d_sparse ? d_tile_flags : nullptr, nullptr, 0, tail_forms, s)
+           : d_sparse ? mp_conv_stem_xrec_sparse(&d, d_stem_pieces, d_sparse, n_f32, d_tile_flags, nullptr, 0, s)
+                      : mp_conv_stem_xrec(&d, d_stem_pieces, n_f32, s);
     }
   } else {
     rc = run_conv_layer(bb->stem, d_x, batch, h, w, bb->in_border, S, 1, nullptr, 1, s, SK, SPLITK_WS_FLOATS, nullptr, nullptr, nullptr, x_f16);
diff --git a/megapose6d_amd/csrc/conv_stem.hip b/megapose6d_amd/csrc/conv_stem.hip
--- a/megapose6d_amd/csrc/conv_stem.hip
+++ b/megapose6d_amd/csrc/conv_stem.hip
@@ -33,6 +33,7 @@
   const unsigned char* __restrict__ tile_flags;
   const unsigned char* __restrict__ w_sparse;
   int fl_tx, fl_ty, q_use, n_steps_sparse;
+  int q_dense, tail_dense, tail_sparse;
   int H, W, pad;
   int count_bg;
 };
@@ -41,12 +42,19 @@
 
 constexpr size_t LDS_PER_WG = 80 * 1024;
 
-template <int KS, int Q>
+constexpr size_t patch_bytes(int KS, int Q, bool tail) {
+  const int PH = 2 * (TH - 1) + KS, PW = 2 * (TW - 1) + KS, plane = tail ? TW : 0;
+  const bool padded = Q % 2 == 0 && (size_t)(PH + 1) * ((PW * (Q + 1) + plane) | 1) * 16 <= LDS_PER_WG;
+  return (size_t)(PH + 1) * ((PW * (padded ? Q + 1 : Q) + plane) | 1) * 16;
+}
+
+template <int KS, int Q, bool TAIL = false>
 struct Geo {
   static constexpr int PH = 2 * (TH - 1) + KS, PW = 2 * (TW - 1) + KS;
-  static constexpr int QP = (Q % 2 == 0 && (size_t)(PH + 1) * ((PW * (Q + 1)) | 1) * 16 <= LDS_PER_WG) ? Q + 1 : Q;
+  static constexpr int PLANE16 = TAIL ? TW : 0;
+  static constexpr int QP = (Q % 2 == 0 && (size_t)(PH + 1) * ((PW * (Q + 1) + PLANE16) | 1) * 16 <= LDS_PER_WG) ? Q + 1 : Q;
   static constexpr int ROW16 = PW * QP;
-  static constexpr int PITCH16 = ROW16 | 1;
+  static constexpr int PITCH16 = (ROW16 + PLANE16) | 1;
   static constexpr int PITCH = PITCH16 * 16;
   static constexpr int KWQ = KS * Q;
   static constexpr int S = KS * KWQ;
@@ -58,9 +66,10 @@
   static_assert(LDS <= LDS_PER_WG, "the patch must leave room for a second workgroup on the CU");
 };
 
-template <int KS, int Q, bool POOL, bool SP = false>
+template <int KS, int Q, bool POOL, bool SP = false, bool TAIL = false>
 __global__ __launch_bounds__(256) __attribute__((amdgpu_waves_per_eu(2, 2))) void conv_stem_bf16x3(Params p) {
-  using G = Geo<KS, Q>;
+  using G = Geo<KS, Q, TAIL>;
+  constexpr bool RT = SP || TAIL;
   extern __shared__ __attribute__((aligned(16))) unsigned char lds[];
   const int tid = threadIdx.x, lane = tid & 63;
   const int wave = __builtin_amdgcn_readfirstlane(tid >> 6);
@@ -84,7 +93,9 @@
       if (blockIdx.x == 0) atomicAdd(&g_stem_bg[1], (unsigned long long)gridDim.x);
     }
   }
-  const int QU = SP && sparse ? p.q_use : Q;
+  const bool tail = TAIL && (SP && sparse ? p.tail_sparse : p.tail_dense) != 0;
+  const int QU = SP && sparse ? p.q_use : (TAIL ? p.q_dense : Q);
+  const int QS = QU + (tail ? 1 : 0);
   const int n_steps = SP && sparse ? p.n_steps_sparse : p.n_steps;
 
   {
@@ -102,7 +113,7 @@
       for (int k = 0; k < HALF; ++k) {
         const int c = tid + 256 * (h * HALF + k);
         const int row = c / SRC16, col = c - row * SRC16;
-        const bool want = c < N_CH && (!SP || col % Q < QU);
+        const bool want = c < N_CH && (!RT || col % Q < QS);
         v[k] = want ? __builtin_amdgcn_raw_buffer_load_b128(r_x, org + row * row_bytes + col * 16, 0, 0) : u32x4{0, 0, 0, 0};
       }
 #pragma unroll
@@ -110,7 +121,7 @@
         const int c = tid + 256 * (h * HALF + k);
         const int row = c / SRC16, col = c - row * SRC16;
         const int lcol = G::QP == Q ? col : col + (col / Q) * (G::QP - Q);
-        if (c < N_CH && (!SP || col % Q < QU)) *reinterpret_cast<u32x4*>(lds + row * G::PITCH + lcol * 16) = v[k];
+        if (c < N_CH && (!RT || col % Q < QS)) *reinterpret_cast<u32x4*>(lds + row * G::PITCH + lcol * 16) = v[k];
       }
     }
     for (int c = tid; c < G::PITCH16; c += 256) *reinterpret_cast<u32x4*>(lds + G::PH * G::PITCH + c * 16) = u32x4{0, 0, 0, 0};
@@ -129,27 +140,53 @@
   const int i = lane & 15, g = lane >> 4;
   int s_r = g;
   int a_row = (2 * i) * (16 * G::QP);
-  const int kwq = SP ? KS * QU : G::KWQ;
+  const int kwq = RT ? KS * QU : G::KWQ;
   const int qu_m = 1024 / QU + 1;
   auto slice_off = [&](int sr) {
-    if constexpr (SP) {
+    if constexpr (RT) {
       const int kw = (sr * qu_m) >> 10;
       return (kw * G::QP + (sr - kw * QU)) * 16;
     } else {
       return G::QP == Q ? sr * 16 : (sr + (sr / Q) * (G::QP - Q)) * 16;
     }
   };
-  int a_off = a_row + slice_off(s_r);
+  int s_t = g - KS * kwq;
+  const int t_base = (G::ROW16 + i) * 16;
+  auto slice_addr = [&]() {
+    int off = a_row + slice_off(s_r);
+    if constexpr (TAIL) {
+      if (tail && s_t >= 0) off = t_base + min(s_t, KS) * G::PITCH;
+    }
+    return off;
+  };
+  int a_off = slice_addr();
   auto advance = [&]() {
     s_r += 4;
+    s_t += 4;
     if (s_r >= kwq) { s_r -= kwq; a_row += G::PITCH; }
-    a_off = a_row + slice_off(s_r);
+    a_off = slice_addr();
   };
   f32x4 acc[TH];
 #pragma unroll
   for (int j = 0; j < TH; ++j) acc[j] = f32x4{0.f, 0.f, 0.f, 0.f};
   u32x4 a0[TH], a1[TH];
 
+  if constexpr (TAIL) {
+    if (tail) {
+      __syncthreads();
+      for (int e = tid; e < G::PH * TW; e += 256) {
+        const int r = e / TW, pi = e - r * TW;
+        const unsigned char* src = lds + r * G::PITCH + (2 * pi * G::QP + QU) * 16;
+        unsigned short el[8];
+#pragma unroll
+        for (int k = 0; k < 8; ++k) el[k] = k < KS ? *reinterpret_cast<const unsigned short*>(src + k * (G::QP * 16)) : (unsigned short)0;
+        u32x4 v;
+#pragma unroll
+        for (int k = 0; k < 4; ++k) v[k] = (unsigned)el[2 * k] | ((unsigned)el[2 * k + 1] << 16);
+        *reinterpret_cast<u32x4*>(lds + r * G::PITCH + (G::ROW16 + pi) * 16) = v;
+      }
+    }
+  }
   __syncthreads();
 #pragma unroll
   for (int j = 0; j < TH; ++j) a0[j] = *reinterpret_cast<const u32x4*>(lds + a_off + j * 2 * G::PITCH);
@@ -267,15 +304,15 @@
       make_float4(0.f, 0.f, 0.f, 0.f);
 }
 
-template <int KS, int Q, bool POOL = false, bool SP = false>
+template <int KS, int Q, bool POOL = false, bool SP = false, bool TAIL = false>
 int launch(const Params& p, hipStream_t s, double flops, double bytes, const char* name) {
   const double executed = 2.0 * (double)p.N * p.tiles_y * p.tiles_x * (TH * TW) * p.Cout * (double)p.n_steps * 32.0 * 3.0;
-  using G = Geo<KS, Q>;
+  using G = Geo<KS, Q, TAIL>;
   static int attr_dev = -1;
   int dev = 0;
   MP_CHECK_HIP(hipGetDevice(&dev));
   if (attr_dev != dev) {
-    MP_CHECK_HIP(hipFuncSetAttribute((const void*)conv_stem_bf16x3<KS, Q, POOL, SP>, hipFuncAttributeMaxDynamicSharedMemorySize, (int)G::LDS));
+    MP_CHECK_HIP(hipFuncSetAttribute((const void*)conv_stem_bf16x3<KS, Q, POOL, SP, TAIL>, hipFuncAttributeMaxDynamicSharedMemorySize, (int)G::LDS));
     attr_dev = dev;
   }
   if (POOL) {
@@ -284,12 +321,14 @@
     hipLaunchKernelGGL(pool_zero_kernel, dim3((unsigned)((total + 255) / 256)), dim3(256), 0, s, p.ypool, p.N, p.Hq, p.Wq, p.Cout, p.pool_border);
   }
   ProfScope prof(name, flops, bytes, s, executed, 2500.0);
-  hipLaunchKernelGGL((conv_stem_bf16x3<KS, Q, POOL, SP>), dim3((unsigned)((long)p.N * p.tiles_y * p.tiles_x * p.n_cb)), dim3(256), G::LDS, s, p);
+  hipLaunchKernelGGL((conv_stem_bf16x3<KS, Q, POOL, SP, TAIL>), dim3((unsigned)((long)p.N * p.tiles_y * p.tiles_x * p.n_cb)), dim3(256), G::LDS, s, p);
   MP_CHECK_HIP(hipGetLastError());
   return MP_OK;
 }
 
-inline int n_steps(int KS, int Q) { return ((KS * KS * Q + 3) / 4 + 1) / 2 * 2; }
+inline int steps_of_slices(int S) { return ((S + 3) / 4 + 1) / 2 * 2; }
+inline int n_steps(int KS, int Q) { return steps_of_slices(KS * KS * Q); }
+inline int n_steps_tail(int KS, int q_main) { return steps_of_slices(KS * KS * q_main + KS); }
 
 }
 }
@@ -311,7 +350,8 @@
   return (size_t)(Cout / stem::NCO) * 4 * stem::n_steps(KS, Q) * 3072;
 }
 
-static int pack_weights_walk(const float* w, int Cout, int Cin, int KS, uint32_t f32_mask, const float* scale, void* packed, int q_walk);
+static int pack_weights_walk(const float* w, int Cout, int Cin, int KS, uint32_t f32_mask, const float* scale, void* packed, int q_walk,
+                             bool tail = false);
 
 extern "C" int mp_conv_stem_pack_weights_mask(const float* w, int Cout, int Cin, int KS, uint32_t f32_mask, const float* scale, void* packed) {
   return pack_weights_walk(w, Cout, Cin, KS, f32_mask, scale, packed, 0);
@@ -334,7 +374,30 @@
   return pack_weights_walk(w, Cout, Cin, KS, n_f32 >= 32 ? 0xFFFFFFFFu : (1u << n_f32) - 1u, scale, packed, q_use);
 }
 
-static int pack_weights_walk(const float* w, int Cout, int Cin, int KS, uint32_t f32_mask, const float* scale, void* packed, int q_walk) {
+extern "C" int mp_conv_stem_tail_forms(int KS, int n_f32, int n_u8) {
+  if (!mp_conv_stem_supported(KS, n_f32, n_u8)) return 0;
+  const int real = 3 * n_f32 + n_u8, Q = (real + 7) / 8, bg = 3 * n_f32;
+  if (stem::patch_bytes(KS, Q, true) > stem::LDS_PER_WG) return 0;
+  int forms = 0;
+  if (real % 8 == 1) forms |= 1;
+  if (bg % 8 == 1 && bg > 8 && n_u8 > 0) forms |= 2;
+  return forms;
+}
+static int tail_main_chunks(int n_f32, int n_u8, int background) { return background ? 3 * n_f32 / 8 : (3 * n_f32 + n_u8) / 8; }
+extern "C" size_t mp_conv_stem_tail_packed_bytes(int KS, int n_f32, int n_u8, int Cout, int background) {
+  if (!(mp_conv_stem_tail_forms(KS, n_f32, n_u8) & (background ? 2 : 1))) return 0;
+  return (size_t)(Cout / stem::NCO) * 4 * stem::n_steps_tail(KS, tail_main_chunks(n_f32, n_u8, background)) * 3072;
+}
+extern "C" int mp_conv_stem_pack_weights_tail(const float* w, int Cout, int Cin, int KS, uint32_t f32_mask, int background, const float* scale,
+                                              void* packed) {
+  const int n_f32 = __builtin_popcount(f32_mask), n_u8 = Cin - n_f32;
+  MP_REQUIRE(n_u8 >= 0 && (mp_conv_stem_tail_forms(KS, n_f32, n_u8) & (background ? 2 : 1)), "mp_conv_stem_pack_weights_tail: this record has no such tail-plane form");
+  MP_REQUIRE(!background || f32_mask == (n_f32 >= 32 ? 0xFFFFFFFFu : (1u << n_f32) - 1u),
+             "mp_conv_stem_pack_weights_tail: the background walk is defined for leading fp32-kind channels only");
+  return pack_weights_walk(w, Cout, Cin, KS, f32_mask, scale, packed, tail_main_chunks(n_f32, n_u8, background), true);
+}
+
+static int pack_weights_walk(const float* w, int Cout, int Cin, int KS, uint32_t f32_mask, const float* scale, void* packed, int q_walk, bool tail) {
   MP_REQUIRE(Cin >= 1 && Cin <= 32 && (Cin == 32 || (f32_mask >> Cin) == 0u), "mp_conv_stem_pack_weights_mask: mask names channels >= Cin (<= 32 input channels)");
   const int n_f32 = __builtin_popcount(f32_mask), n_u8 = Cin - n_f32;
   MP_REQUIRE(w && packed && n_u8 >= 0 && Cout % stem::NCO == 0 && mp_conv_stem_supported(KS, n_f32, n_u8),
@@ -344,7 +407,9 @@
     if ((f32_mask >> c) & 1u) ch_of_f32[a++] = c; else ch_of_u8[b++] = c;
   }
   const int Q = q_walk > 0 ? q_walk : mp_xrec_elements(n_f32, n_u8) / 8;
-  const int T = stem::n_steps(KS, Q), S = KS * KS * Q;
+  MP_REQUIRE(!tail || q_walk > 0, "mp_conv_stem_pack_weights: a tail walk names its main chunks");
+  const int S_main = KS * KS * Q, S = S_main + (tail ? KS : 0);
+  const int T = stem::steps_of_slices(S);
   unsigned short* out = (unsigned short*)packed;
   memset(out, 0, (size_t)(Cout / stem::NCO) * 4 * T * 3072);
   for (int co = 0; co < Cout; ++co) {
@@ -352,9 +417,12 @@
     const double sc = scale ? (double)scale[co] : 1.0;
     for (int s = 0; s < S; ++s) {
       const int t = s / 4, g = s % 4;
-      const int kh = s / (KS * Q), rr = s % (KS * Q), kw = rr / Q, q = rr % Q;
-      for (int e = 0; e < 8; ++e) {
-        const int slot = 8 * q + e;
+      const bool ts = s >= S_main;
+      const int rr = s % (KS * Q);
+      const int kh = ts ? s - S_main : s / (KS * Q), q = ts ? Q : rr % Q;
+      for (int e = 0; e < (ts ? KS : 8); ++e) {
+        const int kw = ts ? e : rr / Q;
+        const int slot = ts ? 8 * q : 8 * q + e;
         int ch;
         double f;
         if (slot < 3 * n_f32) { ch = ch_of_f32[slot / 3]; f = sc; }
@@ -372,7 +440,7 @@
 }
 
 static int stem_xrec_impl(const mp_conv_desc* d, const void* d_packed, int n_f32, float* d_ypool, int pool_border, mp_stream stream,
-                          const void* d_packed_sparse = nullptr, const unsigned char* d_tile_flags = nullptr) {
+                          const void* d_packed_sparse = nullptr, const unsigned char* d_tile_flags = nullptr, int tail_forms = 0) {
   MP_REQUIRE(d && d->d_x && d_packed && (d->d_y || d_ypool), "mp_conv_stem_xrec: null pointer");
   MP_REQUIRE(!d_ypool || (d->relu && pool_border >= 0), "mp_conv_stem_xrec_pool: the fused max pool needs the ReLU (its atomicMax orders non-negative floats)");
   const int n_u8 = d->c_real - n_f32;
@@ -387,7 +455,10 @@
   p.Hp = d->H + 2 * d->in_border; p.Wp = d->W + 2 * d->in_border; p.in_off = d->in_border - d->pad;
   p.Cout = d->Cout; p.Hop = p.Ho + 2 * d->out_border; p.Wop = p.Wo + 2 * d->out_border; p.out_border = d->out_border;
   p.tiles_x = ceil_div(p.Wo, stem::TW); p.tiles_y = ceil_div(p.Ho, stem::TH); p.n_cb = d->Cout / stem::NCO;
-  p.n_steps = stem::n_steps(d->KH, Q);
+  MP_REQUIRE((tail_forms & ~mp_conv_stem_tail_forms(d->KH, n_f32, n_u8)) == 0, "mp_conv_stem_xrec_tail: this record has no such tail-plane form (mp_conv_stem_tail_forms)");
+  p.tail_dense = tail_forms & 1; p.tail_sparse = 0;
+  p.q_dense = p.tail_dense ? Q - 1 : Q;
+  p.n_steps = p.tail_dense ? stem::n_steps_tail(d->KH, Q - 1) : stem::n_steps(d->KH, Q);
   p.relu = d->relu;
   const long img = (long)p.Hp * p.Wp * 16 * Q, outb = (long)p.Hop * p.Wop * d->Cout * 4;
   MP_REQUIRE(img < (1L << 31) && outb < (1L << 31) && (long)d->N * p.tiles_y * p.tiles_x * p.n_cb < (1L << 31), "mp_conv_stem_xrec: image too large for 32-bit offsets");
@@ -396,19 +467,32 @@
   p.Hq = (p.Ho + 2 - 3) / 2 + 1; p.Wq = (p.Wo + 2 - 3) / 2 + 1;
   p.H = d->H; p.W = d->W; p.pad = d->pad;
   p.tile_flags = nullptr; p.w_sparse = nullptr; p.fl_tx = p.fl_ty = 0; p.q_use = Q; p.n_steps_sparse = p.n_steps;
-  const int q_use = mp_conv_stem_sparse_chunks(d->KH, n_f32, n_u8);
+  const bool bg_tail = (tail_forms & 2) != 0;
+  const int q_use = bg_tail ? 3 * n_f32 / 8 : mp_conv_stem_sparse_chunks(d->KH, n_f32, n_u8);
   const bool sp = d_packed_sparse && d_tile_flags && q_use > 0;
   p.count_bg = 0;
   if (sp) {
-    p.count_bg = mp_profile_active();
+    p.count_bg = Q > 2 ? mp_profile_active() : 0;
     p.tile_flags = d_tile_flags; p.w_sparse = (const unsigned char*)d_packed_sparse;
-    p.fl_tx = ceil_div(d->W, 8); p.fl_ty = ceil_div(d->H, 8); p.q_use = q_use; p.n_steps_sparse = stem::n_steps(d->KH, q_use);
+    p.fl_tx = ceil_div(d->W, 8); p.fl_ty = ceil_div(d->H, 8); p.q_use = q_use; p.tail_sparse = bg_tail ? 1 : 0;
+    p.n_steps_sparse = bg_tail ? stem::n_steps_tail(d->KH, q_use) : stem::n_steps(d->KH, q_use);
   }
   const double M = (double)d->N * p.Ho * p.Wo;
   const double flops = 2.0 * M * d->Cout * d->KH * d->KW * d->c_real;
   const double bytes = (double)d->N * img + (d->d_y ? 4.0 * M * d->Cout : 0.0) + (d_ypool ? 4.0 * (double)d->N * p.Hq * p.Wq * d->Cout : 0.0) +
-                       (double)mp_conv_stem_packed_bytes(d->KH, n_f32, n_u8, d->Cout);
+                       (double)p.n_cb * 4 * p.n_steps * 3072;
   hipStream_t s = (hipStream_t)stream;
+#define MP_STEM_GO_TAIL(KSV, QV)                                                                                                     \
+  if (tail_forms && d->KH == KSV && Q == QV) {                                                                                     \
+    if (sp)                                                                                                                        \
+      return d_ypool ? stem::launch<KSV, QV, true, true, true>(p, s, flops, bytes, "conv_stem_bf16x3+maxpool<" #KSV "x" #KSV ",Q" #QV ">")   \
+                     : stem::launch<KSV, QV, false, true, true>(p, s, flops, bytes, "conv_stem_bf16x3<" #KSV "x" #KSV ",Q" #QV ">");       \
+    return d_ypool ? stem::launch<KSV, QV, true, false, true>(p, s, flops, bytes, "conv_stem_bf16x3+maxpool<" #KSV "x" #KSV ",Q" #QV ">")    \
+                   : stem::launch<KSV, QV, false, false, true>(p, s, flops, bytes, "conv_stem_bf16x3<" #KSV "x" #KSV ",Q" #QV ">");        \
+  }
+  MP_STEM_GO_TAIL(7, 2) MP_STEM_GO_TAIL(7, 3) MP_STEM_GO_TAIL(7, 4) MP_STEM_GO_TAIL(7, 5)
+  MP_STEM_GO_TAIL(5, 2) MP_STEM_GO_TAIL(5, 3) MP_STEM_GO_TAIL(5, 4) MP_STEM_GO_TAIL(5, 5) MP_STEM_GO_TAIL(5, 6)
+#undef MP_STEM_GO_TAIL
 #define MP_STEM_GO(KSV, QV)                                                                                                          \
   if (d->KH == KSV && Q == QV) {                                                                                                   \
     if (sp)                                                                                                                        \
@@ -438,6 +522,13 @@
                                         const unsigned char* d_tile_flags, float* d_ypool, int pool_border, mp_stream stream) {
   MP_REQUIRE(d && (d->d_y || d_ypool), "mp_conv_stem_xrec_sparse: null output");
   return stem_xrec_impl(d, d_packed, n_f32, d_ypool, pool_border, stream, d_packed_sparse, d_tile_flags);
+}
+
+extern "C" int mp_conv_stem_xrec_tail(const mp_conv_desc* d, const void* d_packed, const void* d_packed_sparse, int n_f32,
+                                      const unsigned char* d_tile_flags, float* d_ypool, int pool_border, int tail_forms, mp_stream stream) {
+  MP_REQUIRE(d && (d->d_y || d_ypool), "mp_conv_stem_xrec_tail: null output");
+  MP_REQUIRE(tail_forms >= 0 && tail_forms <= 3, "mp_conv_stem_xrec_tail: tail_forms is a mask of bits 0 and 1");
+  return stem_xrec_impl(d, d_packed, n_f32, d_ypool, pool_border, stream, d_packed_sparse, d_tile_flags, tail_forms);
 }
 
 extern "C" int mp_conv_stem_bg_stats(double* background_wgs, double* total_wgs, int reset) {
diff --git a/megapose6d_amd/engine.py b/megapose6d_amd/engine.py
--- a/megapose6d_amd/engine.py
+++ b/megapose6d_amd/engine.py
@@ -429,6 +429,22 @@
     return _pack_weights(lib.mp_conv_stem_pack_weights_sparse, w_oihw, scale, n, np.uint8, Cout, Cin, KH, n_f32)
 
 
+def conv_stem_tail_forms(K: int, n_f32: int, n_u8: int) -> int:
+    return int(_lib.load().mp_conv_stem_tail_forms(K, n_f32, n_u8))
+
+
+def conv_stem_pack_weights_tail(w_oihw: np.ndarray, n_f32: int, scale: Optional[np.ndarray] = None, background: bool = False,
+                                f32_mask: Optional[int] = None) -> Optional[np.ndarray]:
+    lib = _lib.load()
+    Cout, Cin, KH, KW = np.shape(w_oihw)
+    mask = leading_mask(n_f32) if f32_mask is None else int(f32_mask)
+    nf = bin(mask).count("1")
+    n = lib.mp_conv_stem_tail_packed_bytes(KH, nf, Cin - nf, Cout, int(background))
+    if n == 0:
+        return None
+    return _pack_weights(lib.mp_conv_stem_pack_weights_tail, w_oihw, scale, n, np.uint8, Cout, Cin, KH, mask, int(background))
+
+
 def conv_stem_bg_stats(reset: bool = True) -> Tuple[float, float]:
     a, b = C.c_double(), C.c_double()
     check(_lib.load().mp_conv_stem_bg_stats(C.byref(a), C.byref(b), int(reset)))
@@ -438,10 +454,16 @@
 def conv_stem_xrec(xrec: torch.Tensor, N: int, H: int, W: int, c_real: int, n_f32: int, in_border: int, w_pieces: torch.Tensor,
                    bias: Optional[torch.Tensor], Cout: int, K: int, pad: int, y: Optional[torch.Tensor], out_border: int, relu: bool = False,
                    y_pool: Optional[torch.Tensor] = None, pool_border: int = 1, w_sparse: Optional[torch.Tensor] = None,
-                   tile_flags: Optional[torch.Tensor] = None) -> None:
+                   tile_flags: Optional[torch.Tensor] = None, tail_forms: int = 0) -> None:
     assert xrec.dtype == torch.bfloat16 and w_pieces.dtype == torch.uint8
     d = _conv_desc(xrec.data_ptr(), N, H, W, (c_real + 3) // 4 * 4, in_border, Cout, K, 2, pad, _ptr(y), out_border, bias, relu=relu)
     d.c_real = c_real
+    if tail_forms:
+        sp = w_sparse is not None and tile_flags is not None
+        assert not sp or (tile_flags.dtype == torch.uint8 and tile_flags.is_cuda and w_sparse.dtype == torch.uint8)
+        check(_lib.load().mp_conv_stem_xrec_tail(C.byref(d), w_pieces.data_ptr(), w_sparse.data_ptr() if sp else None, n_f32,
+                                                 tile_flags.data_ptr() if sp else None, _ptr(y_pool), pool_border, int(tail_forms), _stream()))
+        return
     if w_sparse is not None and tile_flags is not None:
         assert tile_flags.dtype == torch.uint8 and tile_flags.is_cuda and w_sparse.dtype == torch.uint8
         check(_lib.load().mp_conv_stem_xrec_sparse(C.byref(d), w_pieces.data_ptr(), w_sparse.data_ptr(), n_f32, tile_flags.data_ptr(),
```

New measurement: 2325 (median of 6 runs). +1.6%, better.
